# saiprasadbarke/robustmvd

Measured on AMD Instinct MI355X. Metric: depth-maps/sec at 768x1152x4srcx256planes; warp+aggregate HBM GB/s vs roofline, higher is better.
Workload: dtype f32; 1 GPU; mvsnet (Path B) forward 768x1152, 4 source views, 256 planes, batch 1 per step (BASELINE.json configs[2]); the regulariser's two layers with 32 input channels (conv0, conv4): every fp32 operand as two range-scaled fp16 terms on fp16 MFMA, fp32 accumulation (at least as close to a float64 convolution as the fp32 matrix instruction over 1e-42..1e30: tests/test_hip_f16.py), the other nine layers and ; parallelism=1 independent replica(s), frames round-robin, no collectives

## Files before the change

### include/mvd.h

```cpp
#ifndef MVD_H_
#define MVD_H_

#include <stddef.h>

#ifdef __cplusplus
extern "C" {
#endif

#define MVD_VERSION 100
#define MVD_MAX_VIEWS 32

typedef void* mvd_stream_t;

typedef enum {
    MVD_OK = 0,
    MVD_ERR_INVALID_ARG = 1,
    MVD_ERR_WORKSPACE = 2,
    MVD_ERR_LAUNCH = 3,
    MVD_ERR_NO_DEVICE = 4
} mvd_status;

#define MVD_LAYOUT_NCDHW 0
#define MVD_LAYOUT_NDHWC 1
#define MVD_GRID_EXACT 0x100
#define MVD_FEAT_NHWC_BORDER 0x200

#define MVD_LAYOUT_NCHW 0
#define MVD_LAYOUT_NHWC 1
#define MVD_LAYOUT_NHWC_BORDER 2

int mvd_version(void);
const char* mvd_last_error(void);


size_t mvd_sweep_corr_workspace_bytes(int N, int C, int h, int w, int hs, int ws, int V);
int mvd_sweep_corr_f32(const float* feat_key, const float* const* feat_src, const float* K_key,
                       const float* const* K_src, const float* const* T_src2key, const float* invdepths,
                       int invdepth_batched, int N, int C, int h, int w, int hs, int ws, int S, int V,
                       float* const* corr_out, float* const* mask_out, void* workspace, size_t workspace_bytes,
                       mvd_stream_t stream);

#define MVD_INVDEPTH_SHARED 0
#define MVD_INVDEPTH_BATCHED 1
#define MVD_INVDEPTH_PER_PIXEL 2
int mvd_sweep_corr_ex_f32(const float* feat_key, const float* const* feat_src, const float* K_key,
                          const float* const* K_src, const float* const* T_src2key, const float* invdepths,
                          int invdepth_mode, float corr_scale, int N, int C, int h, int w, int hs, int ws, int S, int V,
                          float* const* corr_out, float* const* mask_out, void* workspace, size_t workspace_bytes,
                          mvd_stream_t stream);
int mvd_sweep_corr_nhwc_f32(const float* feat_key, const float* const* feat_src, const float* K_key, const float* const* K_src,
                            const float* const* T_src2key, const float* invdepths, int invdepth_mode, float corr_scale, int N, int C,
                            int h, int w, int hs, int ws, int S, int V, float* const* corr_out, float* const* mask_out,
                            int out_pixel_stride, float* corr_absmax, mvd_stream_t stream);

int mvd_sweep_warp_f32(const float* const* feat_src, const float* K_key, const float* const* K_src,
                       const float* const* T_src2key, const float* invdepths, int invdepth_mode, int normalize_after, int N,
                       int C, int h, int w, int hs, int ws, int S, int V, float* const* warped_out, float* const* mask_out,
                       mvd_stream_t stream);

int mvd_fuse_views_f32(const float* const* corr, const float* const* mask, const float* const* score, int N, int S,
                       int h, int w, int V, float* fused, float* fused_mask, mvd_stream_t stream);
int mvd_fuse_views_nhwc_f32(const float* const* corr, const float* const* mask, const float* const* score, int N, int S, int h,
                            int w, int V, int in_pixel_stride, float* fused, float* fused_mask, int out_pixel_stride,
                            float* fused_absmax, mvd_stream_t stream);


size_t mvd_warp_variance_workspace_bytes(int B, int C, int h, int w, int V);
int mvd_warp_variance_f32(const float* key_feat, const float* const* src_feat, const float* const* src_proj,
                          const float* key_proj_inv, const float* depth_values, int B, int C, int D, int h, int w,
                          int V, float* var_out, int out_layout, void* workspace, size_t workspace_bytes,
                          mvd_stream_t stream);
int mvd_warp_variance_absmax_f32(const float* key_feat, const float* const* src_feat, const float* const* src_proj,
                                 const float* key_proj_inv, const float* depth_values, int B, int C, int D, int h, int w,
                                 int V, float* var_out, float* absmax_out, int out_layout, void* workspace,
                                 size_t workspace_bytes, mvd_stream_t stream);

size_t mvd_warp_variance_f16_workspace_bytes(int B);
int mvd_warp_variance_f16(const void* key_feat, const void* const* src_feat, const float* const* src_proj,
                          const float* key_proj_inv, const float* depth_values, int B, int D, int h, int w, int V,
                          void* var_out, void* workspace, size_t workspace_bytes, mvd_stream_t stream);
int mvd_convert_f32_to_f16(const float* src, void* dst, long long n, mvd_stream_t stream);
int mvd_convert_f16_to_f32(const void* src, float* dst, long long n, mvd_stream_t stream);

int mvd_homo_warp_f32(const float* src_feat, const float* src_proj, const float* key_proj_inv,
                      const float* depth_values, int B, int C, int D, int h, int w, float* warped_out,
                      void* workspace, size_t workspace_bytes, mvd_stream_t stream);

#define MVD_CONV3D_STRIDE1 0
#define MVD_CONV3D_STRIDE2 1
#define MVD_DECONV3D_STRIDE2 2
size_t mvd_conv3d_packed_weight_floats(int Cin, int Cout);
int mvd_pack_conv3d_weights_f32(const float* w, int Cin, int Cout, int mode, float* packed, mvd_stream_t stream);
int mvd_conv3d_bn_relu_f32(const float* x, const float* packed_w, const float* scale, const float* shift,
                           const float* skip, float* y, int B, int Di, int hi, int wi, int Cin, int Cout, int mode,
                           int relu, mvd_stream_t stream);
int mvd_conv3d_bn_relu_absmax_f32(const float* x, const float* packed_w, const float* scale, const float* shift,
                                  const float* skip, float* y, float* absmax_out, int B, int Di, int hi, int wi, int Cin,
                                  int Cout, int mode, int relu, mvd_stream_t stream);

size_t mvd_conv3d_weight_grad_workspace_bytes(int B, int Di, int hi, int wi, int Cin, int Cout, int mode);
int mvd_conv3d_weight_grad_f32(const float* x, const float* gy, float* gw, int B, int Di, int hi, int wi, int Cin, int Cout,
                               int mode, void* workspace, size_t workspace_bytes, mvd_stream_t stream);

size_t mvd_conv3d_f16_packed_weight_bytes(int Cin, int Cout);
int mvd_pack_conv3d_weights_f16(const float* w, int Cin, int Cout, void* packed, mvd_stream_t stream);
int mvd_conv3d_bn_relu_f16in(const void* x, const void* packed_w, const float* scale, const float* shift, float* y, int B,
                             int D, int h, int w, int Cin, int Cout, int relu, mvd_stream_t stream);

size_t mvd_conv3d_split_packed_weight_bytes(int Cin, int Cout);
int mvd_pack_conv3d_weights_split(const float* w, int Cin, int Cout, void* packed, mvd_stream_t stream);
int mvd_conv3d_bn_relu_f32_split(const float* x, const float* x_absmax, const void* packed_w, const float* scale, const float* shift,
                                 float* y, int B, int D, int h, int w, int Cin, int Cout, int relu, mvd_stream_t stream);
int mvd_conv3d_bn_relu_absmax_f32_split(const float* x, const float* x_absmax, const void* packed_w, const float* scale, const float* shift,
                                        float* y, float* y_absmax, int B, int D, int h, int w, int Cin, int Cout, int relu,
                                        mvd_stream_t stream);
size_t mvd_conv3d_igemm_packed_weight_bytes(int Cin, int Cout, int mode);
int mvd_pack_conv3d_weights_igemm(const float* w, int Cin, int Cout, int mode, void* packed, mvd_stream_t stream);
size_t mvd_conv3d_igemm_workspace_bytes(int B, int Di, int Hi, int Wi, int Cin, int Cout, int mode);
int mvd_conv3d_bn_relu_igemm_f32(const float* x, const float* x_absmax, const void* packed_w, const float* scale, const float* shift,
                                 const float* skip, float* y, float* y_absmax, int B, int Di, int Hi, int Wi, int Cin, int Cout, int mode,
                                 int relu, void* workspace, size_t workspace_bytes, mvd_stream_t stream);
size_t mvd_deconv3d_split_packed_weight_bytes(int Cin, int Cout);
int mvd_pack_deconv3d_weights_split(const float* w, int Cin, int Cout, void* packed, mvd_stream_t stream);
int mvd_deconv3d_bn_relu_f32_split(const float* x, const float* x_absmax, const void* packed_w, const float* scale, const float* shift,
                                   const float* skip, float* y, float* y_absmax, int B, int Di, int hi, int wi, int Cin, int Cout, int relu,
                                   mvd_stream_t stream);
#define MVD_CONV2D 0
#define MVD_DECONV2D 1
#define MVD_CONV2D_IMAGE 2
size_t mvd_conv2d_split_packed_weight_bytes(int Cin_pad, int Cout, int KH, int KW, int stride, int mode);
int mvd_pack_conv2d_weights_split(const float* w, int Cin, int Cin_pad, int Cout, int KH, int KW, int stride, int mode, void* packed,
                                  mvd_stream_t stream);
size_t mvd_conv2d_split_workspace_bytes(int B, int Hi, int Wi, int Cin_pad, int Cout, int KH, int KW, int stride, int mode);
int mvd_conv2d_split_f32(const float* x, const float* x_absmax, const void* packed_w, const float* bias, float* y, float* y_absmax, int B,
                         int Hi, int Wi, int Cin_pad, int x_pixel_stride, int Cout, int y_pixel_stride, long long y_row_stride,
                         long long y_image_stride, long long y_channel_stride, int KH, int KW, int stride, int mode, int act, float slope,
                         void* workspace, size_t workspace_bytes, mvd_stream_t stream);
int mvd_upsample2x_nhwc_f32(const float* x, float* y, float* y_absmax, int B, int C, int h, int w, int y_pixel_stride, mvd_stream_t stream);
int mvd_absmax_f32(const float* x, long long n, float* absmax, mvd_stream_t stream);

size_t mvd_conv2d_packed_weight_floats(int Cin, int Cout, int ksize);
int mvd_pack_conv2d_weights_f32(const float* w, int Cin, int Cout, int ksize, float* packed, mvd_stream_t stream);
int mvd_conv2d_bn_relu_f32(const float* x, int in_layout, const float* packed_w, const float* scale, const float* shift,
                           float* y, int out_layout, int B, int hi, int wi, int Cin, int Cout, int ksize, int stride,
                           int relu, mvd_stream_t stream);
int mvd_conv2d_bn_relu_absmax_f32(const float* x, int in_layout, const float* packed_w, const float* scale, const float* shift,
                                  float* y, float* y_absmax, int out_layout, int B, int hi, int wi, int Cin, int Cout, int ksize,
                                  int stride, int relu, mvd_stream_t stream);

size_t mvd_conv2d_head_tile_count(int B, int H, int W);
int mvd_conv2d_head_f32(const float* image, const float* w0, const float* scale0, const float* shift0, const float* w1,
                        const float* scale1, const float* shift1, float* y, float* tile_absmax, int B, int H, int W,
                        mvd_stream_t stream);
size_t mvd_conv2d_head_split_packed_bytes(void);
int mvd_pack_conv2d_head_split_weights(const float* w1, void* packed, mvd_stream_t stream);
int mvd_conv2d_head_split_f32(const float* image, const float* w0, const float* scale0, const float* shift0, const void* w1_packed,
                              const float* scale1, const float* shift1, float* y, float* tile_absmax, int B, int H, int W,
                              mvd_stream_t stream);

int mvd_softmax_regress_f32(const float* cost, const float* depth_values, int B, int D, int h, int w,
                            float* depth_out, float* conf_out, mvd_stream_t stream);

int mvd_softmax_regress_stats_f32(const float* cost, const float* depth_values, int B, int D, int h, int w,
                                  float* depth_out, float* conf_out, float* stats_out, mvd_stream_t stream);
int mvd_softmax_regress_backward_f32(const float* cost, const float* depth_values, const float* depth, const float* stats,
                                     const float* g_depth, int B, int D, int h, int w, float* g_cost, mvd_stream_t stream);

int mvd_stream_fill_f32(float* dst, long long n, float value, mvd_stream_t stream);

int mvd_arm_kernel_timing(void* start_event, void* stop_event);

int mvd_bias_leaky_relu_f32(float* x, const float* bias, int N, int C, long long HW, float slope, mvd_stream_t stream);

#define MVD_REDUCE_VARIANCE 0
#define MVD_REDUCE_VARIANCE_KEYSQ 1
#define MVD_REDUCE_GROUPCORR 2
size_t mvd_sweep_reduce_workspace_bytes(int B, int C, int h, int w, int V);
int mvd_sweep_reduce_f32(const float* key_feat, const float* const* src_feat, const float* const* M, const float* depth,
                         int depth_per_pixel, float pix_offset, float scale_x, float scale_y, float bias, int mode, int groups,
                         int B, int C, int D, int h, int w, int V, float* const* out, void* workspace, size_t workspace_bytes,
                         mvd_stream_t stream);

int mvd_sweep_reduce_nhwc_f32(const float* key_feat, const float* const* src_feat, const float* const* M, const float* depth,
                              int depth_per_pixel, float pix_offset, float scale_x, float scale_y, float bias, int mode, int B, int C,
                              int D, int h, int w, int V, float* out, mvd_stream_t stream);

int mvd_softmax_regress_pp_f32(const float* cost, const float* depth_hypos, int B, int D, int h, int w, float* depth_out,
                               float* conf_out, mvd_stream_t stream);

int mvd_sweep_groupcorr_nhwc_f32(const float* key_feat, const float* const* src_feat, const float* const* M, const float* depth,
                                 int depth_per_pixel, float pix_offset, float scale_x, float scale_y, float bias, float grid_clamp,
                                 int groups, int B, int C, int D, int h, int w, int V, float* const* out, mvd_stream_t stream);

int mvd_soft_argmin_f32(const float* score, const float* depth_start, int start_per_pixel, const float* depth_interval, float window,
                        int B, int D, int h, int w, float* depth_out, float* entropy_out, float* prob_map_out, mvd_stream_t stream);

int mvd_vis_fuse_f32(const float* const* x, const float* const* u, int B, int D, int h, int w, int C, int V, float* out,
                     mvd_stream_t stream);


size_t mvd_warp_variance_backward_workspace_bytes(int B);
int mvd_warp_variance_backward_f32(const float* key_feat, const float* const* src_feat, const float* const* src_proj,
                                   const float* key_proj_inv, const float* depth_values, const float* grad_var, int B, int C,
                                   int D, int h, int w, int V, float* grad_key, float* const* grad_src, void* workspace,
                                   size_t workspace_bytes, mvd_stream_t stream);

#define MVD_K3_GATHER_RADIUS 3
size_t mvd_warp_variance_backward_gather_workspace_bytes(int B, int C, int D, int h, int w, int V);
int mvd_warp_variance_backward_gather_f32(const float* key_feat, const float* const* src_feat, const float* const* src_proj,
                                          const float* key_proj_inv, const float* depth_values, const float* grad_var, int B, int C,
                                          int D, int h, int w, int V, float* grad_key, float* const* grad_src, int* fallback_count,
                                          void* workspace, size_t workspace_bytes, mvd_stream_t stream);

int mvd_sweep_corr_backward_f32(const float* feat_key, const float* const* feat_src, const float* K_key,
                                const float* const* K_src, const float* const* T_src2key, const float* invdepths,
                                int invdepth_mode, float corr_scale, const float* const* grad_corr, int N, int C, int h, int w,
                                int hs, int ws, int S, int V, float* grad_key, float* const* grad_src, mvd_stream_t stream);

int mvd_sweep_warp_backward_f32(const float* K_key, const float* const* K_src, const float* const* T_src2key, const float* invdepths,
                                int invdepth_mode, const float* const* grad_warped, int N, int C, int h, int w, int hs, int ws, int S,
                                int V, float* const* grad_src, mvd_stream_t stream);

size_t mvd_sweep_reduce_backward_workspace_bytes(int B, int C, int h, int w, int V);
int mvd_sweep_reduce_backward_f32(const float* key_feat, const float* const* src_feat, const float* const* M, const float* depth,
                                  int depth_per_pixel, float pix_offset, float scale_x, float scale_y, float bias, int mode,
                                  int groups, const float* const* grad_out, int B, int C, int D, int h, int w, int V, float* grad_key,
                                  float* const* grad_src, void* workspace, size_t workspace_bytes, mvd_stream_t stream);

int mvd_fuse_views_backward_f32(const float* const* corr, const float* const* mask, const float* const* score,
                                const float* grad_fused, int N, int S, int h, int w, int V, float* const* grad_corr,
                                float* const* grad_score, mvd_stream_t stream);

int mvd_resize_order1_f32(const float* src, float* dst, long long planes, int hi, int wi, int ho, int wo,
                          mvd_stream_t stream);

int mvd_dispnet_head_f32(const float* x, float* pred, float* ent, int N, long long HW, mvd_stream_t stream);

#define MVD_ALIGN_NONE 0
#define MVD_ALIGN_MEDIAN 1
#define MVD_ALIGN_LSQ 2
size_t mvd_depth_eval_workspace_bytes(int H, int W);

int mvd_depth_align_stats_f32(const float* gt, const float* pred, const float* uncertainty, const int* row, const int* col, int H,
                              int W, int h, int w, int mode, int sparse_pred, float* params, double* sums, void* workspace,
                              size_t workspace_bytes, mvd_stream_t stream);

int mvd_depth_score_f32(const float* gt, const float* pred, const float* uncertainty, const int* row, const int* col, int H, int W,
                        int h, int w, int mode, int sparse_pred, int clip, float clip_lo, float clip_hi, float thresh,
                        float thresh_plus_one, const float* params, void* result, float* pred_out, float* invdepth_out,
                        float* rel_ae_out, float* uncertainty_out, void* workspace, size_t workspace_bytes, mvd_stream_t stream);

int mvd_rank_keys_f32(const float* u, const float* u_min, const float* gt, const float* pred_aligned, int sparse_pred, long long n,
                      float* keys, mvd_stream_t stream);

int mvd_ranked_step_sums_f64(const float* ranked, long long n, const long long* count, double* step_sums, void* workspace,
                             size_t workspace_bytes, mvd_stream_t stream);

int mvd_geo_consistency_f32(const float* key_depth, const float* const* src_depth, const float* matrices, const float* uncertainty,
                            int V, int H, int W, float max_reproj_error, float max_rel_depth_diff, int min_consistent_views,
                            float max_uncertainty, unsigned* view_bits, float* fused, unsigned char* mask,
                            unsigned char* num_consistent, mvd_stream_t stream);

size_t mvd_compact_points_workspace_bytes(int H, int W);
int mvd_compact_points_f32(const unsigned char* mask, const float* depth, const float* image, const float* backproject, int H, int W,
                           float* xyz, float* rgb, long long* count, void* workspace, size_t workspace_bytes, mvd_stream_t stream);

int mvd_compact_points_attr_f32(const unsigned char* mask, const float* depth, const float* image, const float* attr,
                                const float* backproject, int H, int W, float* xyz, float* rgb, float* attr_out, long long* count,
// ... 104 lines not shown
```

### robustmvd_amd/_lib.py

```python
import ctypes
import os

import torch

_HERE = os.path.dirname(os.path.abspath(__file__))
LIB_PATH = os.path.join(_HERE, "lib", "libmvd_hip.so")
EXP_LIB_PATH = os.path.join(_HERE, "lib_exp", "libmvd_hip_exp.so")

MVD_MAX_VIEWS = 32
LAYOUT_NCDHW = 0
LAYOUT_NDHWC = 1
GRID_EXACT = 0x100
FEAT_NHWC_BORDER = 0x200
CONV3D_STRIDE1 = 0
CONV2D, DECONV2D, CONV2D_IMAGE = 0, 1, 2
CONV3D_STRIDE2 = 1
DECONV3D_STRIDE2 = 2
LAYOUT_NCHW = 0
LAYOUT_NHWC = 1
LAYOUT_NHWC_BORDER = 2
INVDEPTH_SHARED, INVDEPTH_BATCHED, INVDEPTH_PER_PIXEL = 0, 1, 2
REDUCE_VARIANCE = 0
REDUCE_VARIANCE_KEYSQ = 1
REDUCE_GROUPCORR = 2
ALIGN_NONE, ALIGN_MEDIAN, ALIGN_LSQ = 0, 1, 2
K3_GATHER_RADIUS = 3

_c_float_p = ctypes.c_void_p
_pp = ctypes.POINTER(ctypes.c_void_p)
_i = ctypes.c_int
_sz = ctypes.c_size_t

SIGNATURES = {
    "mvd_version": (_i, []),
    "mvd_last_error": (ctypes.c_char_p, []),
    "mvd_sweep_corr_workspace_bytes": (_sz, [_i] * 7),
    "mvd_sweep_corr_f32": (_i, [_c_float_p, _pp, _c_float_p, _pp, _pp, _c_float_p, _i] + [_i] * 8
                           + [_pp, _pp, ctypes.c_void_p, _sz, ctypes.c_void_p]),
    "mvd_sweep_corr_ex_f32": (_i, [_c_float_p, _pp, _c_float_p, _pp, _pp, _c_float_p, _i, ctypes.c_float] + [_i] * 8
                              + [_pp, _pp, ctypes.c_void_p, _sz, ctypes.c_void_p]),
    "mvd_sweep_corr_nhwc_f32": (_i, [_c_float_p, _pp, _c_float_p, _pp, _pp, _c_float_p, _i, ctypes.c_float] + [_i] * 8
                                + [_pp, _pp, _i, _c_float_p, ctypes.c_void_p]),
    "mvd_fuse_views_nhwc_f32": (_i, [_pp, _pp, _pp] + [_i] * 6 + [_c_float_p, _c_float_p, _i, _c_float_p, ctypes.c_void_p]),
    "mvd_upsample2x_nhwc_f32": (_i, [_c_float_p, _c_float_p, _c_float_p] + [_i] * 5 + [ctypes.c_void_p]),
    "mvd_sweep_warp_f32": (_i, [_pp, _c_float_p, _pp, _pp, _c_float_p] + [_i] * 10 + [_pp, _pp, ctypes.c_void_p]),
    "mvd_fuse_views_f32": (_i, [_pp, _pp, _pp, _i, _i, _i, _i, _i, _c_float_p, _c_float_p, ctypes.c_void_p]),
    "mvd_warp_variance_workspace_bytes": (_sz, [_i] * 5),
    "mvd_warp_variance_f32": (_i, [_c_float_p, _pp, _pp, _c_float_p, _c_float_p] + [_i] * 6
                              + [_c_float_p, _i, ctypes.c_void_p, _sz, ctypes.c_void_p]),
    "mvd_warp_variance_absmax_f32": (_i, [_c_float_p, _pp, _pp, _c_float_p, _c_float_p] + [_i] * 6
                                     + [_c_float_p, _c_float_p, _i, ctypes.c_void_p, _sz, ctypes.c_void_p]),
    "mvd_absmax_f32": (_i, [_c_float_p, ctypes.c_longlong, _c_float_p, ctypes.c_void_p]),
    "mvd_warp_variance_f16_workspace_bytes": (_sz, [_i]),
    "mvd_warp_variance_f16": (_i, [ctypes.c_void_p, _pp, _pp, _c_float_p, _c_float_p] + [_i] * 5
                              + [ctypes.c_void_p, ctypes.c_void_p, _sz, ctypes.c_void_p]),
    "mvd_convert_f32_to_f16": (_i, [_c_float_p, ctypes.c_void_p, ctypes.c_longlong, ctypes.c_void_p]),
    "mvd_convert_f16_to_f32": (_i, [ctypes.c_void_p, _c_float_p, ctypes.c_longlong, ctypes.c_void_p]),
    "mvd_homo_warp_f32": (_i, [_c_float_p] * 4 + [_i] * 5 + [_c_float_p, ctypes.c_void_p, _sz, ctypes.c_void_p]),
    "mvd_conv3d_packed_weight_floats": (_sz, [_i, _i]),
    "mvd_pack_conv3d_weights_f32": (_i, [_c_float_p, _i, _i, _i, _c_float_p, ctypes.c_void_p]),
    "mvd_conv3d_bn_relu_f32": (_i, [_c_float_p] * 6 + [_i] * 8 + [ctypes.c_void_p]),
    "mvd_conv3d_bn_relu_absmax_f32": (_i, [_c_float_p] * 7 + [_i] * 8 + [ctypes.c_void_p]),
    "mvd_conv3d_weight_grad_workspace_bytes": (_sz, [_i] * 7),
    "mvd_conv3d_weight_grad_f32": (_i, [_c_float_p] * 3 + [_i] * 7 + [ctypes.c_void_p, _sz, ctypes.c_void_p]),
    "mvd_conv3d_f16_packed_weight_bytes": (_sz, [_i, _i]),
    "mvd_pack_conv3d_weights_f16": (_i, [_c_float_p, _i, _i, ctypes.c_void_p, ctypes.c_void_p]),
    "mvd_conv3d_bn_relu_f16in": (_i, [ctypes.c_void_p, ctypes.c_void_p, _c_float_p, _c_float_p, _c_float_p] + [_i] * 7
                                 + [ctypes.c_void_p]),
    "mvd_conv3d_split_packed_weight_bytes": (_sz, [_i, _i]),
    "mvd_conv3d_bn_relu_absmax_f32_split": (_i, [_c_float_p, _c_float_p, ctypes.c_void_p, _c_float_p, _c_float_p, _c_float_p, _c_float_p]
                                            + [_i] * 7 + [ctypes.c_void_p]),
    "mvd_conv3d_igemm_packed_weight_bytes": (_sz, [_i] * 3),
    "mvd_pack_conv3d_weights_igemm": (_i, [_c_float_p, _i, _i, _i, ctypes.c_void_p, ctypes.c_void_p]),
    "mvd_conv3d_igemm_workspace_bytes": (_sz, [_i] * 7),
    "mvd_conv3d_bn_relu_igemm_f32": (_i, [_c_float_p, _c_float_p, ctypes.c_void_p] + [_c_float_p] * 5 + [_i] * 8
                                     + [ctypes.c_void_p, ctypes.c_size_t, ctypes.c_void_p]),
    "mvd_conv2d_split_packed_weight_bytes": (_sz, [_i] * 6),
    "mvd_pack_conv2d_weights_split": (_i, [_c_float_p] + [_i] * 7 + [ctypes.c_void_p, ctypes.c_void_p]),
    "mvd_conv2d_split_workspace_bytes": (_sz, [_i] * 9),
    "mvd_conv2d_split_f32": (_i, [_c_float_p, _c_float_p, ctypes.c_void_p, _c_float_p, _c_float_p, _c_float_p] + [_i] * 7
                             + [ctypes.c_longlong] * 3 + [_i] * 5 + [ctypes.c_float, ctypes.c_void_p, ctypes.c_size_t, ctypes.c_void_p]),
    "mvd_pack_conv3d_weights_split": (_i, [_c_float_p, _i, _i, ctypes.c_void_p, ctypes.c_void_p]),
    "mvd_conv3d_bn_relu_f32_split": (_i, [_c_float_p, _c_float_p, ctypes.c_void_p, _c_float_p, _c_float_p, _c_float_p] + [_i] * 7
                                     + [ctypes.c_void_p]),
    "mvd_deconv3d_split_packed_weight_bytes": (_sz, [_i, _i]),
    "mvd_pack_deconv3d_weights_split": (_i, [_c_float_p, _i, _i, ctypes.c_void_p, ctypes.c_void_p]),
    "mvd_deconv3d_bn_relu_f32_split": (_i, [_c_float_p, _c_float_p, ctypes.c_void_p] + [_c_float_p] * 5 + [_i] * 7 + [ctypes.c_void_p]),
    "mvd_conv2d_packed_weight_floats": (_sz, [_i, _i, _i]),
    "mvd_pack_conv2d_weights_f32": (_i, [_c_float_p, _i, _i, _i, _c_float_p, ctypes.c_void_p]),
    "mvd_conv2d_bn_relu_f32": (_i, [_c_float_p, _i, _c_float_p, _c_float_p, _c_float_p, _c_float_p, _i] + [_i] * 8
                               + [ctypes.c_void_p]),
    "mvd_conv2d_head_tile_count": (_sz, [_i] * 3),
    "mvd_conv2d_head_f32": (_i, [_c_float_p] * 9 + [_i] * 3 + [ctypes.c_void_p]),
    "mvd_conv2d_head_split_packed_bytes": (_sz, []),
    "mvd_pack_conv2d_head_split_weights": (_i, [_c_float_p, ctypes.c_void_p, ctypes.c_void_p]),
    "mvd_conv2d_head_split_f32": (_i, [_c_float_p] * 4 + [ctypes.c_void_p] + [_c_float_p] * 4 + [_i] * 3 + [ctypes.c_void_p]),
    "mvd_conv2d_bn_relu_absmax_f32": (_i, [_c_float_p, _i, _c_float_p, _c_float_p, _c_float_p, _c_float_p, _c_float_p, _i] + [_i] * 8
                                      + [ctypes.c_void_p]),
    "mvd_softmax_regress_f32": (_i, [_c_float_p, _c_float_p, _i, _i, _i, _i, _c_float_p, _c_float_p, ctypes.c_void_p]),
    "mvd_softmax_regress_stats_f32": (_i, [_c_float_p, _c_float_p, _i, _i, _i, _i, _c_float_p, _c_float_p, _c_float_p,
                                           ctypes.c_void_p]),
    "mvd_softmax_regress_backward_f32": (_i, [_c_float_p] * 5 + [_i] * 4 + [_c_float_p, ctypes.c_void_p]),
    "mvd_bias_leaky_relu_f32": (_i, [_c_float_p, _c_float_p, _i, _i, ctypes.c_longlong, ctypes.c_float, ctypes.c_void_p]),
    "mvd_dispnet_head_f32": (_i, [_c_float_p, _c_float_p, _c_float_p, _i, ctypes.c_longlong, ctypes.c_void_p]),
    "mvd_arm_kernel_timing": (_i, [ctypes.c_void_p, ctypes.c_void_p]),
    "mvd_stream_fill_f32": (_i, [_c_float_p, ctypes.c_longlong, ctypes.c_float, ctypes.c_void_p]),
    "mvd_warp_variance_backward_workspace_bytes": (_sz, [_i]),
    "mvd_warp_variance_backward_f32": (_i, [_c_float_p, _pp, _pp, _c_float_p, _c_float_p, _c_float_p] + [_i] * 6
                                       + [_c_float_p, _pp, ctypes.c_void_p, _sz, ctypes.c_void_p]),
    "mvd_warp_variance_backward_gather_workspace_bytes": (_sz, [_i] * 6),
    "mvd_warp_variance_backward_gather_f32": (_i, [_c_float_p, _pp, _pp, _c_float_p, _c_float_p, _c_float_p] + [_i] * 6
                                              + [_c_float_p, _pp, ctypes.c_void_p, ctypes.c_void_p, _sz, ctypes.c_void_p]),
    "mvd_sweep_corr_backward_f32": (_i, [_c_float_p, _pp, _c_float_p, _pp, _pp, _c_float_p, _i, ctypes.c_float, _pp] + [_i] * 8
                                    + [_c_float_p, _pp, ctypes.c_void_p]),
    "mvd_fuse_views_backward_f32": (_i, [_pp, _pp, _pp, _c_float_p] + [_i] * 5 + [_pp, _pp, ctypes.c_void_p]),
    "mvd_sweep_reduce_workspace_bytes": (_sz, [_i] * 5),
    "mvd_sweep_reduce_f32": (_i, [_c_float_p, _pp, _pp, _c_float_p, _i] + [ctypes.c_float] * 4 + [_i] * 8
                             + [_pp, ctypes.c_void_p, _sz, ctypes.c_void_p]),
    "mvd_sweep_reduce_nhwc_f32": (_i, [_c_float_p, _pp, _pp, _c_float_p, _i] + [ctypes.c_float] * 4 + [_i] * 7
                                  + [_c_float_p, ctypes.c_void_p]),
    "mvd_softmax_regress_pp_f32": (_i, [_c_float_p, _c_float_p, _i, _i, _i, _i, _c_float_p, _c_float_p, ctypes.c_void_p]),
    "mvd_sweep_groupcorr_nhwc_f32": (_i, [_c_float_p, _pp, _pp, _c_float_p, _i] + [ctypes.c_float] * 5 + [_i] * 7 + [_pp, ctypes.c_void_p]),
    "mvd_soft_argmin_f32": (_i, [_c_float_p, _c_float_p, _i, _c_float_p, ctypes.c_float] + [_i] * 4 + [_c_float_p] * 3 + [ctypes.c_void_p]),
    "mvd_vis_fuse_f32": (_i, [_pp, _pp] + [_i] * 6 + [_c_float_p, ctypes.c_void_p]),
    "mvd_sweep_reduce_backward_workspace_bytes": (_sz, [_i] * 5),
    "mvd_sweep_reduce_backward_f32": (_i, [_c_float_p, _pp, _pp, _c_float_p, _i] + [ctypes.c_float] * 4 + [_i, _i, _pp] + [_i] * 6
                                      + [_c_float_p, _pp, ctypes.c_void_p, _sz, ctypes.c_void_p]),
    "mvd_sweep_warp_backward_f32": (_i, [_c_float_p, _pp, _pp, _c_float_p, _i, _pp] + [_i] * 8 + [_pp, ctypes.c_void_p]),
    "mvd_resize_order1_f32": (_i, [_c_float_p, _c_float_p, ctypes.c_longlong, _i, _i, _i, _i, ctypes.c_void_p]),
    "mvd_nchw_to_nhwc_f32": (_i, [_c_float_p, _c_float_p, _i, _i, ctypes.c_longlong, ctypes.c_void_p]),
    "mvd_nhwc_to_nchw_f32": (_i, [_c_float_p, _c_float_p, _i, _i, ctypes.c_longlong, ctypes.c_void_p]),
    "mvd_zero_border_nhwc_f32": (_i, [_c_float_p, _i, _i, _i, _i, ctypes.c_void_p]),
    "mvd_depth_eval_workspace_bytes": (_sz, [_i, _i]),
    "mvd_depth_align_stats_f32": (_i, [_c_float_p] * 3 + [ctypes.c_void_p] * 2 + [_i] * 6 + [_c_float_p, ctypes.c_void_p,
                                                                                            ctypes.c_void_p, _sz, ctypes.c_void_p]),
    "mvd_depth_score_f32": (_i, [_c_float_p] * 3 + [ctypes.c_void_p] * 2 + [_i] * 7 + [ctypes.c_float] * 4
                            + [_c_float_p, ctypes.c_void_p] + [_c_float_p] * 4 + [ctypes.c_void_p, _sz, ctypes.c_void_p]),
    "mvd_rank_keys_f32": (_i, [_c_float_p] * 4 + [_i, ctypes.c_longlong, _c_float_p, ctypes.c_void_p]),
    "mvd_ranked_step_sums_f64": (_i, [_c_float_p, ctypes.c_longlong, ctypes.c_void_p, ctypes.c_void_p, ctypes.c_void_p, _sz,
                                      ctypes.c_void_p]),
    "mvd_geo_consistency_f32": (_i, [_c_float_p, _pp, _c_float_p, _c_float_p, _i, _i, _i, ctypes.c_float, ctypes.c_float, _i,
                                     ctypes.c_float] + [ctypes.c_void_p] * 5),
    "mvd_compact_points_workspace_bytes": (_sz, [_i, _i]),
    "mvd_compact_points_f32": (_i, [ctypes.c_void_p] + [_c_float_p] * 3 + [_i, _i, _c_float_p, _c_float_p, ctypes.c_void_p,
                                                                          ctypes.c_void_p, _sz, ctypes.c_void_p]),
    "mvd_compact_points_attr_f32": (_i, [ctypes.c_void_p] + [_c_float_p] * 4 + [_i, _i] + [_c_float_p] * 3
                                    + [ctypes.c_void_p, ctypes.c_void_p, _sz, ctypes.c_void_p]),
    "mvd_depth_normals_f32": (_i, [_c_float_p, _c_float_p, _i, _i, _c_float_p, ctypes.c_void_p]),
    "mvd_geo_merge_f32": (_i, [_c_float_p, _pp, _c_float_p, _c_float_p, _i, _i, _i, ctypes.c_float, ctypes.c_float, _i, ctypes.c_float,
                               ctypes.c_void_p, _pp, _c_float_p, _pp, _c_float_p, _pp] + [ctypes.c_void_p] * 7),
    "mvd_cloud_cell_keys_f32": (_i, [_c_float_p, ctypes.c_longlong] + [ctypes.c_double] * 4 + [ctypes.c_void_p] * 2),
    "mvd_cloud_grid_build_f32": (_i, [_c_float_p, ctypes.c_void_p, ctypes.c_longlong, _c_float_p, ctypes.c_void_p]),
    "mvd_cloud_nearest_f32": (_i, [_c_float_p, ctypes.c_longlong, _c_float_p, ctypes.c_void_p, ctypes.c_longlong]
                              + [ctypes.c_double] * 4 + [ctypes.c_float, _c_float_p, ctypes.c_void_p, ctypes.c_void_p]),
    "mvd_cloud_scores_workspace_bytes": (_sz, [ctypes.c_longlong]),
    "mvd_cloud_scores_f32": (_i, [_c_float_p, ctypes.c_void_p, _c_float_p, ctypes.c_longlong, _c_float_p, _i, ctypes.c_void_p,
                                  ctypes.c_void_p, _sz, ctypes.c_void_p]),
    "mvd_voxel_reduce_workspace_bytes": (_sz, [ctypes.c_longlong]),
    "mvd_voxel_reduce_f32": (_i, [ctypes.c_void_p] * 2 + [_c_float_p] * 2 + [ctypes.c_longlong, _c_float_p, _c_float_p]
                             + [ctypes.c_void_p] * 3 + [_sz, ctypes.c_void_p]),
    "mvd_cloud_transform_f32": (_i, [_c_float_p, _c_float_p, ctypes.c_longlong, ctypes.c_void_p, _c_float_p, _c_float_p, ctypes.c_void_p]),
    "mvd_cloud_transform_records_f32": (_i, [_c_float_p, ctypes.c_void_p, ctypes.c_longlong, ctypes.c_void_p, _c_float_p, ctypes.c_void_p]),
    "mvd_cloud_pair_sums_workspace_bytes": (_sz, [ctypes.c_longlong]),
    "mvd_cloud_pair_sums_f32": (_i, [_c_float_p, ctypes.c_longlong, ctypes.c_void_p, ctypes.c_void_p, _c_float_p, _c_float_p,
                                     ctypes.c_longlong] + [ctypes.c_double] * 3 + [ctypes.c_void_p, ctypes.c_void_p, _sz, ctypes.c_void_p]),
    "mvd_tsdf_integrate_f32": (_i, [_c_float_p] * 3 + [_i] * 3 + [_pp] * 3 + [_c_float_p, _i, _i, _i, ctypes.c_float, ctypes.c_float,
                                                                            ctypes.c_void_p]),
    "mvd_tsdf_extract_workspace_bytes": (_sz, [_i] * 3),
    "mvd_tsdf_extract_f32": (_i, [_c_float_p] * 3 + [_i] * 3 + [ctypes.c_float] * 5 + [_i, _c_float_p, _c_float_p, ctypes.c_void_p,
                                                                                      ctypes.c_longlong, ctypes.c_longlong,
                                                                                      ctypes.c_void_p, ctypes.c_void_p, _sz,
                                                                                      ctypes.c_void_p]),
    "mvd_mesh_render_workspace_bytes": (_sz, [ctypes.c_longlong, ctypes.c_longlong, _i, _i, _i]),
    "mvd_mesh_render_f32": (_i, [_c_float_p, ctypes.c_longlong, ctypes.c_void_p, ctypes.c_longlong, _c_float_p, _c_float_p, _i, _i, _i,
                                 ctypes.c_float, _i, _i, _i, _c_float_p, ctypes.c_void_p, _c_float_p, _c_float_p, _c_float_p,
                                 ctypes.c_void_p, _sz, ctypes.c_void_p]),
    "mvd_mesh_hook_round": (_i, [ctypes.c_void_p, ctypes.c_longlong, ctypes.c_longlong, _i] + [ctypes.c_void_p] * 4),
    "mvd_mesh_component_rank_workspace_bytes": (_sz, [ctypes.c_longlong]),
    "mvd_mesh_component_rank": (_i, [ctypes.c_void_p, ctypes.c_void_p, ctypes.c_longlong, ctypes.c_void_p, ctypes.c_void_p,
                                     ctypes.c_void_p, _sz, ctypes.c_void_p]),
    "mvd_mesh_component_table": (_i, [ctypes.c_void_p, ctypes.c_void_p] + [ctypes.c_longlong] * 3 + [ctypes.c_void_p] * 3),
    "mvd_mesh_component_sums_workspace_bytes": (_sz, [ctypes.c_longlong, ctypes.c_longlong]),
    "mvd_mesh_component_sums_f64": (_i, [_c_float_p, ctypes.c_longlong, ctypes.c_void_p, ctypes.c_longlong, ctypes.c_void_p,
                                         ctypes.c_void_p, ctypes.c_longlong, ctypes.c_void_p, ctypes.c_void_p, ctypes.c_void_p, _sz,
                                         ctypes.c_void_p]),
    "mvd_mesh_filter_workspace_bytes": (_sz, [ctypes.c_longlong, ctypes.c_longlong]),
    "mvd_mesh_filter": (_i, [ctypes.c_void_p, ctypes.c_longlong, ctypes.c_longlong, ctypes.c_void_p, ctypes.c_void_p,
                             ctypes.c_longlong, _i, _i] + [ctypes.c_void_p] * 3 + [ctypes.c_longlong, ctypes.c_void_p, ctypes.c_void_p,
                                                                                   _sz, ctypes.c_void_p]),
    "mvd_mesh_gather_rows_f32": (_i, [_c_float_p, ctypes.c_void_p, ctypes.c_longlong, _i, ctypes.c_longlong, _c_float_p,
                                      ctypes.c_void_p]),
    "mvd_mesh_vertex_normals_f32": (_i, [_c_float_p, ctypes.c_longlong, ctypes.c_void_p, ctypes.c_longlong, ctypes.c_void_p,
                                         ctypes.c_void_p, _c_float_p, ctypes.c_void_p]),
}
CULL_NONE, CULL_BACK, CULL_FRONT = 0, 1, 2
RENDER_LOAD_FIRST, RENDER_KEEP_PROJECT, RENDER_KEEP_KEYS, RENDER_NO_RESOLVE = 1, 16, 32, 64
MESH_RENDER_MAX_SMALL = 64
MESH_ROUND_FIRST, MESH_ROUND_NO_HOOK, MESH_ROUND_NO_SHORTCUT = 1, 2, 4
MVD_CLOUD_MAX_THRESHOLDS = 8
MVD_CLOUD_PAIR_SUMS_PER_WORKGROUP = 2048

PRODUCT_ONLY = ("mvd_sweep_reduce_backward_workspace_bytes", "mvd_sweep_reduce_backward_f32")

_lib = None
_override = None


def _bind(path, skip=()):
    lib = ctypes.CDLL(path)
    for name, (res, args) in SIGNATURES.items():
        if name in skip:
            continue
        fn = getattr(lib, name)
        fn.restype = res
        fn.argtypes = args
    return lib


def load():
    global _lib
    if _override is not None:
        return _override
    if _lib is not None:
        return _lib
    if not os.path.exists(LIB_PATH):
        raise RuntimeError(
            f"{LIB_PATH} not found: the HIP engine is not built. Run `python -c 'import __graft_entry__ as g; "
            "g.build()'` or `make -C robustmvd_amd/csrc`. There is no CPU fallback for this path.")
    _lib = _bind(LIB_PATH)
    return _lib


class use_experiments_library:

    def __init__(self, path=None):
        self.path = path or EXP_LIB_PATH

# ... 60 lines not shown
```

### robustmvd_amd/blocks.py

```python
from typing import NamedTuple

import numpy as np
import torch
import torch.nn as nn
import torch.nn.functional as F

from . import _lib as L
from . import ops
from .utils import to_torch

homo_warp = ops.homo_warp


def compute_sampling_invdepths(min_depth, max_depth, num_samples, sampling_type="linear_invdepth"):
    def col(v):
        if isinstance(v, (float, int, np.floating)):
            v = torch.tensor([float(v)])
        return to_torch(v).float()[..., None]

    lo, hi = col(min_depth), col(max_depth)
    steps = torch.arange(0, num_samples, dtype=lo.dtype, device=lo.device)[None]
    if sampling_type == "linear_invdepth":
        return 1 / hi + steps * (1 / lo - 1 / hi) / (num_samples - 1)
    if sampling_type == "linear_depth":
# ... 230 lines not shown
        self.split_layers = bool(split_layers)
        self.fused_head = True
        self.head_split = True
        for i, s in enumerate(self.SPEC):
            setattr(self, f"conv{i}", ConvBnReLU(*s))
        self.feature = nn.Conv2d(32, 32, 3, 1, 1)

    def _pack(self):
        pk = FeatureNetWeights()
        for i, (cin, cout, k, stride, _) in enumerate(self.SPEC):
            m = getattr(self, f"conv{i}")
            w, _, _, _ = ops.pack_conv2d_weights(m.conv.weight.detach())
            pk.layers.append(Conv2dLayer(w, cin, cout, k, stride, *fold_bn(m.bn), True))
        w, _, _, _ = ops.pack_conv2d_weights(self.feature.weight.detach())
        pk.layers.append(Conv2dLayer(w, 32, 32, 3, 1, torch.ones(32, device=w.device), self.feature.bias.detach().contiguous(), False))
        if self.split_layers:
            for i in range(2, 8):
                conv = getattr(self, f"conv{i}").conv if i < 7 else self.feature
                lay = pk.layers[i]
                pk.split.append((ops.pack_conv2d_weights_split(conv.weight.detach() * lay.scale.view(-1, 1, 1, 1), lay.shift,
                                                               stride=lay.stride), lay.relu))
            for conv, lay in ((self.conv0.conv, pk.layers[0]), (self.conv1.conv, pk.layers[1])):
                pk.head += (conv.weight.detach().permute(2, 3, 1, 0).contiguous(), lay.scale, lay.shift)
            pk.head_w1 = ops.pack_conv2d_head_weights_split(self.conv1.conv.weight.detach())
        return pk

    @ops.inference_only
    def forward_layout(self, x, out_layout, return_absmax=False, out=None):
        pk = self._prepare()
        if out is not None and not (self.split_layers and out_layout == L.LAYOUT_NHWC_BORDER):
            raise ValueError("out: only the split layers' LAYOUT_NHWC_BORDER output can be written into a caller's buffer")
        if not self.split_layers:
            for layer in pk.layers[:-1]:
                x = layer(x)
            x = pk.layers[-1](x, out_layout)
            return (x, ops.absmax(x)) if return_absmax else x
        slots = Slots(8, x.device)
        if self.fused_head:
            if self.head_split:
                x, a_in = ops.conv2d_head_split(x, *pk.head[:3], pk.head_w1, *pk.head[4:], return_absmax=True)
            else:
                x, a_in = ops.conv2d_head(x, *pk.head, return_absmax=True)
        else:
            x = pk.layers[1](pk.layers[0](x))
            a_in = ops.absmax(x)
        for wts, relu in pk.split[:-1]:
            a_out = slots.take()
            x = ops.conv2d_split(x, a_in, wts, act=2 if relu else 0, out_absmax=a_out)
            a_in = a_out
        wts, a_out = pk.split[-1][0], slots.take()
        if out_layout == L.LAYOUT_NCHW:
            x = ops.conv2d_split(x, a_in, wts, act=0, planar_out=True)
            if return_absmax:
                a_out.copy_(ops.absmax(x))
        elif out_layout == L.LAYOUT_NHWC_BORDER:
            B, h, w_, _ = x.shape
            if out is None:
                out = torch.empty((B, h + 3, w_ + 3, wts.cout), dtype=torch.float32, device=x.device)
            elif tuple(out.shape) != (B, h + 3, w_ + 3, wts.cout):
                raise ValueError(f"out: shape {tuple(out.shape)}, expected {(B, h + 3, w_ + 3, wts.cout)}")
            buf = ops.zero_border_nhwc(out)
            ops.conv2d_split(x, a_in, wts, act=0, out=buf[:, 1:h + 1, 1:w_ + 1, :], out_absmax=a_out)
            x = buf
        else:
            x = ops.conv2d_split(x, a_in, wts, act=0, out_absmax=a_out)
        return (x, a_out) if return_absmax else x

    def forward(self, x):
        return self.forward_layout(x, L.LAYOUT_NCHW)

    def forward_autograd(self, x):
        x = self.conv1(self.conv0(x))
        x = self.conv4(self.conv3(self.conv2(x)))
        return self.feature(self.conv6(self.conv5(x)))


class ConvBnReLU3D(nn.Module):
    def __init__(self, cin, cout, kernel_size=3, stride=1, pad=1):
        super().__init__()
        self.conv = nn.Conv3d(cin, cout, kernel_size, stride=stride, padding=pad, bias=False)
        self.bn = nn.BatchNorm3d(cout)

    def forward(self, x):
        return F.relu(self.bn(self.conv(x)), inplace=True)


def _deconv_block(cin, cout):
    return nn.Sequential(nn.ConvTranspose3d(cin, cout, kernel_size=3, padding=1, output_padding=1, stride=2, bias=False),
                         nn.BatchNorm3d(cout), nn.ReLU(inplace=True))


class CostRegWeights:

    def __init__(self):
        self.layers, self.igemm, self.dsplit = {}, {}, {}
        self.conv0_f16 = self.conv0_split = self.conv0_bound = None

    def get(self, key):
        name, _, form = key.rpartition("_")
        if form in ("igemm", "dsplit"):
            return getattr(self, form).get(name)
        return self.layers.get(key, getattr(self, key, None) if name == "conv0" else None)

    def __getitem__(self, key):
        found = self.get(key)
        if found is None:
            raise KeyError(key)
        return found

    def __contains__(self, key):
        return self.get(key) is not None


class CostRegNet(PackedWeights, nn.Module):

    FOLDS_BN = "CostRegNet"
    LAYERS = [("conv0", 32, 8, 1), ("conv1", 8, 16, 2), ("conv2", 16, 16, 1), ("conv3", 16, 32, 2), ("conv4", 32, 32, 1),
              ("conv5", 32, 64, 2), ("conv6", 64, 64, 1)]
    UPS = [("conv7", 64, 32), ("conv9", 32, 16), ("conv11", 16, 8)]

    def __init__(self, conv0_split=True):
        super().__init__()
        self.conv0_split = bool(conv0_split)
        for name, cin, cout, stride in self.LAYERS:
            setattr(self, name, ConvBnReLU3D(cin, cout, stride=stride))
        for name, cin, cout in self.UPS:
            setattr(self, name, _deconv_block(cin, cout))
        self.prob = nn.Conv3d(8, 1, 3, stride=1, padding=1)

    def _pack(self):
        pk = CostRegWeights()
        for name, _, _, stride in self.LAYERS:
            m = getattr(self, name)
            pk.layers[name] = Conv3dLayer.pack(m.conv.weight, L.CONV3D_STRIDE1 if stride == 1 else L.CONV3D_STRIDE2, bn=m.bn)
        for name, _, _ in self.UPS:
            m = getattr(self, name)
            pk.layers[name] = Conv3dLayer.pack(m[0].weight, L.DECONV3D_STRIDE2, bn=m[1])
        pk.layers["prob"] = Conv3dLayer.pack(self.prob.weight, L.CONV3D_STRIDE1, bias=self.prob.bias)
        pk.conv0_f16 = ops.pack_conv3d_weights_f16(self.conv0.conv.weight.detach())
        if self.conv0_split:
            w0, conv0 = self.conv0.conv.weight.detach(), pk.layers["conv0"]
            pk.conv0_split = ops.pack_conv3d_weights_split(w0)
            pk.conv0_bound = ((w0.abs().sum(dim=(1, 2, 3, 4)) * conv0.scale.abs()).contiguous(), conv0.shift.abs().contiguous())
            for name, _, _, _ in self.LAYERS[1:]:
                pk.igemm[name] = ops.pack_conv3d_weights_igemm(getattr(self, name).conv.weight.detach(), pk.layers[name].mode)
            for name, _, _ in self.UPS:
                pk.dsplit[name] = ops.pack_deconv3d_weights_split(getattr(self, name)[0].weight.detach())
        return pk

    @ops.inference_only
    def forward_channels_last(self, x, x_absmax=None):
        if x.shape[1] % 8 or x.shape[2] % 8 or x.shape[3] % 8:
            raise ValueError(f"CostRegNet needs D,h,w divisible by 8, got {tuple(x.shape[1:4])}")
        pk = self._prepare()
        first = pk["conv0"]
        split_decoder = self.conv0_split and x.dtype == torch.float32

        if x.dtype == torch.float16:
            conv0 = ops.conv3d_bn_relu_f16in(x, pk.conv0_f16, first.scale, first.shift, relu=True)
        elif self.conv0_split:
            if x_absmax is None:
                x_absmax = ops.absmax(x)
            conv0 = ops.conv3d_bn_relu_split(x, pk.conv0_split, first.scale, first.shift, relu=True, x_absmax=x_absmax)
            gain0, off0 = pk.conv0_bound
            a0 = (gain0 * x_absmax + off0).amax().reshape(1)
        else:
            conv0 = first(x)

        if self.conv0_split:
            slots = Slots(8, x.device)

            def igemm(name, t, a, leave_absmax=True):
                lay = pk[name]
                y = ops.conv3d_bn_relu_igemm(t, a, pk.igemm[name], lay.cin, lay.cout, lay.scale, lay.shift, lay.mode, relu=True,
                                             return_absmax=leave_absmax, out_absmax=slots.take() if leave_absmax else None)
                return y if leave_absmax else (y, None)

            if x.dtype == torch.float16:
                a0 = ops.absmax(conv0)
            t, a = igemm("conv1", conv0, a0)
            conv2, a = igemm("conv2", t, a)
            t, a = igemm("conv3", conv2, a)
            conv4, a = igemm("conv4", t, a)
            t, a = igemm("conv5", conv4, a)
            y, a = igemm("conv6", t, a, leave_absmax=split_decoder)
        else:
            conv2 = pk["conv2"](pk["conv1"](conv0))
            conv4 = pk["conv4"](pk["conv3"](conv2))
            y, a = pk["conv6"](pk["conv5"](conv4)), None

        def deconv(name, t, a, skip, leave_absmax=True):
            lay = pk[name]
            if not split_decoder:
                return lay(t, skip=skip), None
            y = ops.deconv3d_bn_relu_split(t, a, pk.dsplit[name], lay.cin, lay.cout, lay.scale, lay.shift, relu=True, skip=skip,
                                           return_absmax=leave_absmax, out_absmax=slots.take() if leave_absmax else None)
            return y if leave_absmax else (y, None)

        y, a = deconv("conv7", y, a, conv4)
        del conv4
        y, a = deconv("conv9", y, a, conv2)
        del conv2
        y, _ = deconv("conv11", y, a, conv0, leave_absmax=False)
        del conv0

        return pk["prob"](y, relu=False).squeeze(-1)

    @ops.inference_only
    def forward(self, x):
        return self.forward_channels_last(ops.to_channels_last_3d(x)).unsqueeze(1)

    def forward_autograd(self, x):
        conv0 = self.conv0(x)
        conv2 = self.conv2(self.conv1(conv0))
        conv4 = self.conv4(self.conv3(conv2))
        x = self.conv6(self.conv5(conv4))
        x = conv4 + self.conv7(x)
        x = conv2 + self.conv9(x)
        x = conv0 + self.conv11(x)
        return self.prob(x)

    def forward_autograd_engine(self, x):
        if x.dim() != 5 or x.shape[1] % 8 or x.shape[2] % 8 or x.shape[3] % 8:
            raise ValueError(f"CostRegNet needs (B,D,h,w,32) with D,h,w divisible by 8, got {tuple(x.shape)}")

        def layer(name, t):
            m = getattr(self, name)
            stride = m.conv.stride[0]
            y = ops.conv3d_autograd(t, m.conv.weight, L.CONV3D_STRIDE1 if stride == 1 else L.CONV3D_STRIDE2)
            return F.relu(_batch_norm_channels_last(m.bn, y), inplace=True)

        def up(name, t):
            m = getattr(self, name)
            y = ops.conv3d_autograd(t, m[0].weight, L.DECONV3D_STRIDE2)
            return F.relu(_batch_norm_channels_last(m[1], y), inplace=True)

        conv0 = layer("conv0", x)
        conv2 = layer("conv2", layer("conv1", conv0))
        conv4 = layer("conv4", layer("conv3", conv2))
        x = layer("conv6", layer("conv5", conv4))
        x = conv4 + up("conv7", x)
        x = conv2 + up("conv9", x)
        x = conv0 + up("conv11", x)
        return (ops.conv3d_autograd(x, self.prob.weight, L.CONV3D_STRIDE1) + self.prob.bias).squeeze(-1)


def _batch_norm_channels_last(bn, y):
    factor = 0.0 if bn.momentum is None else bn.momentum
    if bn.training and bn.track_running_stats and bn.num_batches_tracked is not None:
        bn.num_batches_tracked.add_(1)
        if bn.momentum is None:
            factor = 1.0 / float(bn.num_batches_tracked)
    batch_stats = bn.training or (bn.running_mean is None and bn.running_var is None)
    keep = not bn.training or bn.track_running_stats
    out = F.batch_norm(y.reshape(-1, y.shape[-1]), bn.running_mean if keep else None, bn.running_var if keep else None,
                       bn.weight, bn.bias, batch_stats, factor, bn.eps)
    return out.view(y.shape)


class _ConvLeaky(nn.Sequential):

    def forward(self, x):
        c = self[0]
        if torch.is_grad_enabled() or not x.is_cuda or c.bias is None:
            return super().forward(x)
        if isinstance(c, nn.ConvTranspose2d):
            y = F.conv_transpose2d(x, c.weight, None, c.stride, c.padding, c.output_padding, c.groups, c.dilation)
        else:
            y = F.conv2d(x, c.weight, None, c.stride, c.padding, c.dilation, c.groups)
        if y.dtype != torch.float32 or not y.is_contiguous() or y.shape[0] * y.shape[1] > 65535:
            return F.leaky_relu(y + c.bias.to(y.dtype).view(1, -1, 1, 1), self[1].negative_slope, inplace=True)
        return ops.bias_leaky_relu_(y, c.bias, self[1].negative_slope)


def conv(cin, cout, kernel_size=3, stride=1):
    return _ConvLeaky(nn.Conv2d(cin, cout, kernel_size=kernel_size, stride=stride, padding=(kernel_size - 1) // 2, bias=True),
                      nn.LeakyReLU(0.2, inplace=True))


class ReLUAndSigmoid(nn.Module):

    def __init__(self, inplace=False, min=0.0, max=1.0):
        super().__init__()
        self.min, self.max, self.range = min, max, max - min

    def forward(self, x):
        return torch.cat([F.relu(x[:, :1]), torch.sigmoid(x[:, 1:] * (4 / self.range)) * self.range + self.min], 1)


class DispnetEncoder(nn.Module):
    def __init__(self):
        super().__init__()
        self.conv1 = conv(3, 64, kernel_size=7, stride=2)
        self.conv2 = conv(64, 128, kernel_size=5, stride=2)
        self.conv3 = conv(128, 256, kernel_size=3, stride=2)

    def forward(self, image):
        c1 = self.conv1(image)
        c2 = self.conv2(c1)
        c3 = self.conv3(c2)
        return {"conv1": c1, "conv2": c2, "conv3a": c3}, c3


class DispnetContextEncoder(nn.Module):
    def __init__(self):
        super().__init__()
        self.conv_redir = conv(256, 32, kernel_size=1, stride=1)

    def forward(self, conv3):
        return self.conv_redir(conv3)


class DispnetCostvolumeEncoder(nn.Module):
    def __init__(self):
        super().__init__()
        self.conv3_1 = conv(256 + 32, 256)
        self.conv4 = conv(256, 512, stride=2)
        self.conv4_1 = conv(512, 512)
        self.conv5 = conv(512, 512, stride=2)
        self.conv5_1 = conv(512, 512)
        self.conv6 = conv(512, 1024, stride=2)
        self.conv6_1 = conv(1024, 1024)

    def forward(self, corr, ctx):
        out = {"merged": torch.cat([ctx, corr], 1)}
        x = out["merged"]
        for name in ("conv3_1", "conv4", "conv4_1", "conv5", "conv5_1", "conv6", "conv6_1"):
            x = getattr(self, name)(x)
            out[name] = x
        return out, x

# ... 61 lines not shown
```

### robustmvd_amd/csrc/conv3d_split.hip

```cpp
#include "mvd_common.h"
#include "split_operand.h"

#ifndef SPLIT_KO
#define SPLIT_KO 0
#endif
#ifndef SPLIT_DEPTH
#define SPLIT_DEPTH 4
#endif

namespace mvd {

typedef _Float16 h16x8 __attribute__((ext_vector_type(8)));
typedef float sf32x4 __attribute__((ext_vector_type(4)));
typedef unsigned int su32x4 __attribute__((ext_vector_type(4)));
typedef unsigned int su32x2 __attribute__((ext_vector_type(2)));
typedef _Float16 h16x2 __attribute__((ext_vector_type(2)));

constexpr int S_TH = 4, S_TW = 32, S_ROWS = S_TH + 2;
constexpr float S_LO_FACTOR = 2048.0f;
template <int CIN>
struct SplitGeom {
    static constexpr int CH8 = CIN / 8;
    static constexpr int VB = CIN * 2;
    static constexpr int KWG = CIN == 32 ? 3 : 2;
    static constexpr int NT = 9 * KWG;
    static constexpr int COLS = CIN == 32 ? S_TW + 2 : S_TW + 3;
    static constexpr int HALF_BYTES = S_ROWS * COLS * VB;
    static constexpr int PLANE_BYTES = 2 * HALF_BYTES;
    static constexpr int ITEMS = S_ROWS * COLS * CH8;
    static constexpr int NLOAD = (ITEMS + 255) / 256;
    static constexpr int NF = 4 * KWG * 2;
    static_assert(NF - 8 == 4 * NLOAD, "pass B interleaves 8 epilogue groups and 4 staging groups per item");
};

template <int CIN>
__global__ void pack_conv0_split_kernel(const float* __restrict__ w, const float* __restrict__ wscale, _Float16* __restrict__ packed, int ncb) {
    using G = SplitGeom<CIN>;
    const int e = blockIdx.x * 256 + threadIdx.x;
    if (e >= ncb * G::NT * 64 * 8) return;
    const int j = e & 7, lane = (e >> 3) & 63, t = (e >> 9) % G::NT, cb = (e >> 9) / G::NT;
    const int col = lane & 15, k = 8 * (lane >> 4) + j, cout = cb * 8 + (col & 7);
    int tap, cin;
    if constexpr (CIN == 32) { tap = t; cin = k; }
    else { const int kw = 2 * (t % 2) + k / 16; tap = kw < 3 ? (t / 2) * 3 + kw : -1; cin = k % 16; }
    const float v = tap >= 0 ? w[((size_t)cout * CIN + cin) * 27 + tap] / wscale[cout] : 0.0f;
    _Float16 hi, lo;
    split_weight(v, S_LO_FACTOR, hi, lo);
    packed[e] = col < 8 ? hi : lo;
}

struct SplitParams {
    const float* x;
    const char* wpk;
    const float* scale;
    const float* shift;
    const float* absmax;
    float* y;
    float* yamax;
    int B, D, h, w, relu;
    int cout, ncb;
    int tiles_x, tiles_y, dgroups, td, tiles_per_xcd;
};

__device__ __forceinline__ unsigned pack_h2(_Float16 a, _Float16 b) {
    const h16x2 v = {a, b};
    return __builtin_bit_cast(unsigned, v);
}

template <int CIN, bool YAMAX = false>
__global__ void __launch_bounds__(256, 2) conv0_split_kernel(SplitParams p) {
    using G = SplitGeom<CIN>;
    constexpr int S_COLS = G::COLS, S_HALF_BYTES = G::HALF_BYTES, S_PLANE_BYTES = G::PLANE_BYTES, S_ITEMS = G::ITEMS, S_NLOAD = G::NLOAD;
    constexpr int KWG = G::KWG, NT = G::NT;
    extern __shared__ __attribute__((aligned(16))) char ring[];
    const int tid = threadIdx.x, lane = tid & 63, wv = tid >> 6;
    const int D = p.D, h = p.h, w = p.w;

    const int xcd = blockIdx.x & 7;
    int j = blockIdx.x >> 3;
    const int cb = j % p.ncb; j /= p.ncb;
    const int t_in = j % p.tiles_per_xcd; j /= p.tiles_per_xcd;
    const int dg = j % p.dgroups;
    const int b = j / p.dgroups;
    const int tile = xcd * p.tiles_per_xcd + t_in;
    if (tile >= p.tiles_x * p.tiles_y) return;
    const int ty = tile / p.tiles_x, tx = tile - ty * p.tiles_x;
    const int x0 = tx * S_TW, y0 = ty * S_TH;
    const int dz0 = dg * p.td, dz1 = min(dz0 + p.td, D);

    h16x8 wf[NT];
#pragma unroll
    for (int t = 0; t < NT; ++t) wf[t] = *reinterpret_cast<const h16x8*>(p.wpk + (((size_t)cb * NT + t) * 64 + lane) * 16);

    constexpr unsigned OOB = 0x80000000u;
    unsigned gob[S_NLOAD];
    int loff[S_NLOAD];
#pragma unroll
    for (int k = 0; k < S_NLOAD; ++k) {
        const int e = tid + 256 * k;
        const int vox = e / G::CH8, ch = e % G::CH8;
        const int r = vox / S_COLS, c = vox - r * S_COLS;
        const int gy = y0 - 1 + r, gx = x0 - 1 + c;
        const bool in = e < S_ITEMS && c < S_TW + 2 && gy >= 0 && gy < h && gx >= 0 && gx < w;
        gob[k] = in ? (unsigned)(((gy * w + gx) * CIN + ch * 8) * 4) : OOB;
        if constexpr (CIN == 32) loff[k] = e < S_ITEMS ? (vox * 64 + ((ch ^ ((c >> 1) & 3)) * 16)) : -1;
        else loff[k] = e < S_ITEMS ? e * 16 : -1;
    }
    const size_t plane_f = (size_t)h * w * CIN;
    const float* xb = p.x + (size_t)b * D * plane_f;
    su32x4 pre[S_NLOAD][2];
    auto fetch = [&](int d) {
        const bool din = d >= 0 && d < D && d <= dz1;
        const __amdgpu_buffer_rsrc_t rs = __builtin_amdgcn_make_buffer_rsrc(
            const_cast<float*>(xb + (din ? (size_t)d * plane_f : 0)), 0, din ? (int)(plane_f * 4) : 0, 0x00020000);
#pragma unroll
        for (int k = 0; k < S_NLOAD; ++k) {
            pre[k][0] = __builtin_amdgcn_raw_buffer_load_b128(rs, gob[k], 0, 0);
            pre[k][1] = __builtin_amdgcn_raw_buffer_load_b128(rs, gob[k] + 16u, 0, 0);
        }
    };
    char* const dump = ring + 2 * S_PLANE_BYTES + tid * 16;
    float xs, xs_inv;
    split_xscale(p.absmax, xs, xs_inv);
    auto split2 = [xs](float a0, float a1, unsigned& hi, unsigned& lo) { mvd::split2(xs, a0, a1, hi, lo, S_LO_FACTOR); };
    auto stash = [&](int d) {
        char* slot = ring + (d & 1) * S_PLANE_BYTES;
#pragma unroll
        for (int k = 0; k < S_NLOAD; ++k) {
            su32x4 hv, lv;
#pragma unroll
            for (int q = 0; q < 4; ++q) {
                const sf32x4 v = __builtin_bit_cast(sf32x4, pre[k][q >> 1]);
                unsigned hi, lo;
                split2(v[(q & 1) * 2], v[(q & 1) * 2 + 1], hi, lo);
                hv[q] = hi; lv[q] = lo;
            }
            char* dst = loff[k] >= 0 ? slot + loff[k] : dump;
            *reinterpret_cast<su32x4*>(dst) = hv;
            *reinterpret_cast<su32x4*>(loff[k] >= 0 ? dst + S_HALF_BYTES : dst) = lv;
        }
    };

    const int col = lane & 15;
    float esc_ = p.scale[cb * 8 + (col & 7)], esh_ = p.shift[cb * 8 + (col & 7)];
    float eun_ = reinterpret_cast<const float*>(p.wpk + (size_t)p.ncb * NT * 64 * 16)[cb * 8 + (col & 7)] * xs_inv;
    const float floor_ = p.relu ? 0.f : -__builtin_inff();
    const int xh = wv & 1, rp = wv >> 1;

    int fragk[KWG];
#pragma unroll
    for (int kw = 0; kw < KWG; ++kw) {
        if constexpr (CIN == 32) {
            const int c = 16 * xh + (lane & 15) + kw;
            fragk[kw] = (2 * rp * S_COLS + c) * 64 + (((lane >> 4) ^ ((c >> 1) & 3)) * 16);
        } else {
            const int c = 16 * xh + (lane & 15) + 2 * kw;
            fragk[kw] = (2 * rp * S_COLS + c) * 32 + (lane >> 4) * 16;
        }
    }

    sf32x4 acc[3][2][2];
#pragma unroll
    for (int s = 0; s < 3; ++s)
#pragma unroll
        for (int r = 0; r < 2; ++r) { acc[s][r][0] = sf32x4{0, 0, 0, 0}; acc[s][r][1] = sf32x4{0, 0, 0, 0}; }

    unsigned yoff[2];
#pragma unroll
    for (int row = 0; row < 2; ++row) {
        const int oy = y0 + 2 * rp + row;
        yoff[row] = (col < 8 && oy < h) ? (unsigned)((((size_t)oy * w + x0 + 16 * xh + 4 * (lane >> 4)) * p.cout + cb * 8 + col) * 4) : OOB;
    }
    const int oxb = x0 + 16 * xh + 4 * (lane >> 4);
    const size_t yplane_f = (size_t)h * w * p.cout;
    const unsigned vox_b = (unsigned)p.cout * 4u;

    fetch(dz0 - 1);
    asm volatile("" : "+v"(esc_), "+v"(esh_), "+v"(eun_));
    stash(dz0 - 1);
    fetch(dz0);

    [[maybe_unused]] float amax_ = 0.f;
    for (int z = dz0 - 1; z <= dz1; ++z) {
        if (!(SPLIT_KO & 8)) __syncthreads();
        const char* slot = ring + (z & 1) * S_PLANE_BYTES;
        char* wslot = ring + ((z + 1) & 1) * S_PLANE_BYTES;
        const int din = z + 2, dout = z - 1;
        const bool in_ok = din >= 0 && din < D && din <= dz1, out_ok = dout >= dz0 && dout < dz1;
        const __amdgpu_buffer_rsrc_t rs_in = __builtin_amdgcn_make_buffer_rsrc(
            const_cast<float*>(xb + (in_ok ? (size_t)din * plane_f : 0)), 0, in_ok ? (int)(plane_f * 4) : 0, 0x00020000);
        const __amdgpu_buffer_rsrc_t rs_out = __builtin_amdgcn_make_buffer_rsrc(
            p.y + ((size_t)b * D + (out_ok ? dout : 0)) * yplane_f, 0, out_ok ? (int)(yplane_f * 4) : 0, 0x00020000);
        int ox = oxb;
        asm volatile("" : "+v"(ox));

        constexpr int NF = G::NF, NR = 2 * NF, DEPTH = SPLIT_DEPTH;
        h16x8 fr[DEPTH];
        auto rr_of = [](int ro) { return ro == 0 ? 1 : ro == 1 ? 2 : ro == 2 ? 0 : 3; };
        auto frag = [&](int i) {
            const int g = i % NF, term = g & 1, kw = (g >> 1) % KWG, rr = rr_of(g / (2 * KWG));
            if (SPLIT_KO & 32) return wf[i % NT];
            return *reinterpret_cast<const h16x8*>(slot + term * S_HALF_BYTES + fragk[kw] + rr * S_COLS * G::VB);
        };
#pragma unroll
        for (int i = 0; i < DEPTH; ++i) fr[i] = frag(i);
#pragma unroll
        for (int g = 0; g < NF; ++g) {
            const int term = g & 1, kw = (g >> 1) % KWG, rr = rr_of(g / (2 * KWG));
            const h16x8 f = fr[g % DEPTH];
#pragma unroll
            for (int row = 0; row < 2; ++row) {
                const int kh = rr - row;
                if (kh < 0 || kh > 2) continue;
                if (SPLIT_KO & 16) acc[0][row][term][0] += f[0] * wf[(6 + kh) * KWG + kw][0];
                else acc[0][row][term] = __builtin_amdgcn_mfma_f32_16x16x32_f16(f, wf[(6 + kh) * KWG + kw], acc[0][row][term], 0, 0, 0);
            }
            fr[g % DEPTH] = frag(g + DEPTH);
            __builtin_amdgcn_sched_barrier(0);
        }
        float hl = __shfl_down(acc[0][0][0][0], 8, 16);
        unsigned hq0 = 0, lq0 = 0;
#pragma unroll
        for (int g = 0; g < NF; ++g) {
            const int term = g & 1, kw = (g >> 1) % KWG, rr = rr_of(g / (2 * KWG));
            const h16x8 f = fr[(NF + g) % DEPTH];
#pragma unroll
            for (int row = 0; row < 2; ++row) {
                const int kh = rr - row;
                if (kh < 0 || kh > 2) continue;
#pragma unroll
                for (int s = 1; s < 3; ++s)
                    if (SPLIT_KO & 16) acc[s][row][term][0] += f[0] * wf[((2 - s) * 3 + kh) * KWG + kw][0];
                    else acc[s][row][term] = __builtin_amdgcn_mfma_f32_16x16x32_f16(f, wf[((2 - s) * 3 + kh) * KWG + kw], acc[s][row][term], 0, 0, 0);
            }
            if (NF + g + DEPTH < NR) fr[(NF + g) % DEPTH] = frag(NF + g + DEPTH);
            if (g < 8) {
                const int row = g >> 2, i = g & 3;
                const float cur = hl;
                if (g + 1 < 8) hl = __shfl_down(acc[0][(g + 1) >> 2][0][(g + 1) & 3], 8, 16);
                float r = __builtin_fmaf(cur + acc[0][row][1][i], 1.0f / 2048.0f, acc[0][row][0][i]);
                r = fmaxf(__builtin_fmaf(r * eun_, esc_, esh_), floor_);
                if constexpr (YAMAX)
                    if (out_ok && yoff[row] != OOB && ox + i < w) amax_ = fmaxf(amax_, finite_abs_or_zero(r));
                if (!(SPLIT_KO & 2) || r == 12345.678f)
                    __builtin_amdgcn_raw_buffer_store_b32(__float_as_uint(r), rs_out, ox + i < w ? yoff[row] + vox_b * i : OOB, 0, 0);
            } else if (!(SPLIT_KO & 4)) {
                const int k = (g - 8) >> 2, q = (g - 8) & 3;
                const sf32x4 v = __builtin_bit_cast(sf32x4, pre[k][q >> 1]);
                unsigned hq1, lq1;
                split2(v[(q & 1) * 2], v[(q & 1) * 2 + 1], hq1, lq1);
                if (q & 1) {
                    char* dst = (loff[k] >= 0 ? wslot + loff[k] : dump) + 8 * (q >> 1);
                    *reinterpret_cast<su32x2*>(dst) = su32x2{hq0, hq1};
                    *reinterpret_cast<su32x2*>(loff[k] >= 0 ? dst + S_HALF_BYTES : dst) = su32x2{lq0, lq1};
                } else {
                    hq0 = hq1; lq0 = lq1;
                }
                if (q == 3 && !(SPLIT_KO & 1)) {
                    pre[k][0] = __builtin_amdgcn_raw_buffer_load_b128(rs_in, gob[k], 0, 0);
                    pre[k][1] = __builtin_amdgcn_raw_buffer_load_b128(rs_in, gob[k] + 16u, 0, 0);
                }
            }
            __builtin_amdgcn_sched_barrier(0);
        }
#pragma unroll
        for (int r = 0; r < 2; ++r)
#pragma unroll
            for (int t = 0; t < 2; ++t) {
                acc[0][r][t] = acc[1][r][t];
                acc[1][r][t] = acc[2][r][t];
                acc[2][r][t] = sf32x4{0, 0, 0, 0};
            }
    }
    if constexpr (YAMAX) {
        for (int o = 32; o > 0; o >>= 1) amax_ = fmaxf(amax_, __shfl_xor(amax_, o));
        __syncthreads();
        float* wm = reinterpret_cast<float*>(ring);
        if (lane == 0) wm[wv] = amax_;
        __syncthreads();
        if (tid == 0) {
            amax_ = fmaxf(fmaxf(wm[0], wm[1]), fmaxf(wm[2], wm[3]));
            raise_absmax(p.yamax, amax_);
        }
    }
}

}

static bool split_shape_ok(int Cin, int Cout) { return (Cin == 32 || Cin == 16) && Cout >= 8 && Cout <= 64 && Cout % 8 == 0; }
static size_t split_frag_bytes(int Cin, int Cout) { return (size_t)(Cout / 8) * (Cin == 32 ? 27 : 18) * 64 * 16; }

template <int CIN, bool YAMAX>
static int launch_split_v(const mvd::SplitParams& p, long long nblk, hipStream_t st) {
    const size_t lds = 2 * (size_t)mvd::SplitGeom<CIN>::PLANE_BYTES + 256 * 16;
    (void)hipFuncSetAttribute((const void*)mvd::conv0_split_kernel<CIN, YAMAX>, hipFuncAttributeMaxDynamicSharedMemorySize, (int)lds);
    hipLaunchKernelGGL((mvd::conv0_split_kernel<CIN, YAMAX>), dim3((unsigned)nblk), dim3(256), lds, st, p);
    return mvd::launch_status("conv3d_split");
}
template <int CIN>
static int launch_split(const mvd::SplitParams& p, long long nblk, hipStream_t st) {
    return p.yamax ? launch_split_v<CIN, true>(p, nblk, st) : launch_split_v<CIN, false>(p, nblk, st);
}

extern "C" {

size_t mvd_conv3d_split_packed_weight_bytes(int Cin, int Cout) {
    return split_shape_ok(Cin, Cout) ? split_frag_bytes(Cin, Cout) + (size_t)Cout * sizeof(float) : 0;
}

int mvd_pack_conv3d_weights_split(const float* w, int Cin, int Cout, void* packed, mvd_stream_t stream) {
    MVD_REQUIRE(w && packed, "pack_conv3d_weights_split: NULL argument");
    MVD_REQUIRE(split_shape_ok(Cin, Cout), "pack_conv3d_weights_split: 16 or 32 input channels and 8, 16, ... 64 output channels are built (got %d -> %d)", Cin, Cout);
    const int ncb = Cout / 8;
    float* wscale = reinterpret_cast<float*>(static_cast<char*>(packed) + split_frag_bytes(Cin, Cout));
    mvd::split_wscale_launch(w, wscale, Cin, Cout, 27, false, Cout, Cout, (hipStream_t)stream);
    const unsigned nb = (unsigned)((split_frag_bytes(Cin, Cout) / 2 + 255) / 256);
    if (Cin == 32) hipLaunchKernelGGL(mvd::pack_conv0_split_kernel<32>, dim3(nb), dim3(256), 0, (hipStream_t)stream, w, wscale, (_Float16*)packed, ncb);
    else hipLaunchKernelGGL(mvd::pack_conv0_split_kernel<16>, dim3(nb), dim3(256), 0, (hipStream_t)stream, w, wscale, (_Float16*)packed, ncb);
    return mvd::launch_status("pack_conv3d_weights_split");
}

static int conv3d_split_entry(const float* x, const float* x_absmax, const void* packed_w, const float* scale, const float* shift, float* y,
                              float* y_absmax, int B, int D, int h, int w, int Cin, int Cout, int relu, mvd_stream_t stream);

int mvd_conv3d_bn_relu_f32_split(const float* x, const float* x_absmax, const void* packed_w, const float* scale, const float* shift,
                                 float* y, int B, int D, int h, int w, int Cin, int Cout, int relu, mvd_stream_t stream) {
    return conv3d_split_entry(x, x_absmax, packed_w, scale, shift, y, nullptr, B, D, h, w, Cin, Cout, relu, stream);
}

int mvd_conv3d_bn_relu_absmax_f32_split(const float* x, const float* x_absmax, const void* packed_w, const float* scale, const float* shift,
                                        float* y, float* y_absmax, int B, int D, int h, int w, int Cin, int Cout, int relu,
                                        mvd_stream_t stream) {
    MVD_REQUIRE(y_absmax, "conv3d_split_absmax: NULL argument");
    return conv3d_split_entry(x, x_absmax, packed_w, scale, shift, y, y_absmax, B, D, h, w, Cin, Cout, relu, stream);
}

static int conv3d_split_entry(const float* x, const float* x_absmax, const void* packed_w, const float* scale, const float* shift, float* y,
                              float* y_absmax, int B, int D, int h, int w, int Cin, int Cout, int relu, mvd_stream_t stream) {
    MVD_REQUIRE(x && x_absmax && packed_w && scale && shift && y, "conv3d_split: NULL argument");
    MVD_REQUIRE(split_shape_ok(Cin, Cout), "conv3d_split: 16 or 32 input channels and 8, 16, ... 64 output channels are built (got %d -> %d)", Cin, Cout);
    MVD_REQUIRE(B > 0 && D > 0 && h > 0 && w > 0, "conv3d_split: non-positive dimension");
    MVD_REQUIRE((long long)h * w * Cin * 4 < 0x7fffffffLL && (long long)h * w * Cout * 4 < 0x7fffffffLL,
                "conv3d_split: one plane exceeds the 31-bit byte-offset range");
    mvd::SplitParams p{};
    p.x = x; p.absmax = x_absmax; p.wpk = (const char*)packed_w; p.scale = scale; p.shift = shift; p.y = y; p.yamax = y_absmax;
    if (y_absmax && hipMemsetAsync(y_absmax, 0, sizeof(float), (hipStream_t)stream) != hipSuccess) return mvd::launch_status("conv3d_split: memset");
    p.B = B; p.D = D; p.h = h; p.w = w; p.relu = relu;
    p.cout = Cout; p.ncb = Cout / 8;
    p.tiles_x = (w + mvd::S_TW - 1) / mvd::S_TW;
    p.tiles_y = (h + mvd::S_TH - 1) / mvd::S_TH;
    const long long tiles = (long long)p.tiles_x * p.tiles_y;
    p.tiles_per_xcd = (int)((tiles + 7) / 8);
    int td = 32;
    while (td > 8 && tiles * B * p.ncb * ((D + td - 1) / td) < 2048) td /= 2;
    p.td = td;
    p.dgroups = (D + td - 1) / td;
    const long long nblk = 8LL * p.ncb * p.tiles_per_xcd * p.dgroups * B;
    MVD_REQUIRE(nblk <= 0x7fffffffLL, "conv3d_split: %lld workgroups exceed the grid limit", nblk);
    return Cin == 32 ? launch_split<32>(p, nblk, (hipStream_t)stream) : launch_split<16>(p, nblk, (hipStream_t)stream);
}
}
```

### robustmvd_amd/csrc/split_operand.h

```cpp
#pragma once
#include "mvd_common.h"

namespace mvd {

__device__ __forceinline__ void split_xscale_of(unsigned max_bits, float& xsc, float& xsc_inv) {
    const int ex = (int)((max_bits >> 23) & 0xffu) - 127;
    const int e = max(-125, min(125, ex - 14));
    xsc = __uint_as_float((unsigned)(127 - e) << 23);
    xsc_inv = __uint_as_float((unsigned)(127 + e) << 23);
}
__device__ __forceinline__ void split_xscale(const float* xamax, float& xsc, float& xsc_inv) {
    split_xscale_of(__builtin_amdgcn_readfirstlane((int)__float_as_uint(*xamax)), xsc, xsc_inv);
}
__device__ __forceinline__ void split2(float xsc, float a0, float a1, unsigned& hi, unsigned& lo, float lo_factor = 1.0f) {
    unsigned hp, lp;
    float t0, t1;
    asm("v_fma_mixlo_f16 %0, %1, %2, 0 op_sel:[0,0,0] op_sel_hi:[0,0,0]" : "=v"(hp) : "v"(a0), "s"(xsc));
    asm("v_fma_mixhi_f16 %0, %1, %2, 0 op_sel:[0,0,0] op_sel_hi:[0,0,0]" : "+v"(hp) : "v"(a1), "s"(xsc));
    asm("v_fma_mix_f32 %0, %1, %2, -%3 op_sel:[0,0,0] op_sel_hi:[0,0,1]" : "=v"(t0) : "v"(a0), "s"(xsc), "v"(hp));
    asm("v_fma_mix_f32 %0, %1, %2, -%3 op_sel:[0,0,1] op_sel_hi:[0,0,1]" : "=v"(t1) : "v"(a1), "s"(xsc), "v"(hp));
    asm("v_fma_mixlo_f16 %0, %1, %2, 0 op_sel:[0,0,0] op_sel_hi:[0,0,0]" : "=v"(lp) : "v"(t0), "s"(lo_factor));
    asm("v_fma_mixhi_f16 %0, %1, %2, 0 op_sel:[0,0,0] op_sel_hi:[0,0,0]" : "+v"(lp) : "v"(t1), "s"(lo_factor));
    hi = hp;
    lo = lp;
}

__device__ __forceinline__ void split_weight(float v, float lo_factor, _Float16& hi, _Float16& lo) {
    hi = (_Float16)v;
    lo = (_Float16)((v - (float)hi) * lo_factor);
}

static __global__ void split_wscale_kernel(const float* __restrict__ w, float* __restrict__ wscale, int Cin, int Cout, int taps, int transposed,
                                           int rows) {
    __shared__ float red[256];
    const int r = blockIdx.x, c = r % Cout;
    float m = 0.f;
    if (r < rows)
        for (int e = threadIdx.x; e < Cin * taps; e += 256) {
            const int ci = e / taps, t = e % taps;
            const float v = fabsf(transposed ? w[((size_t)ci * Cout + c) * taps + t] : w[((size_t)c * Cin + ci) * taps + t]);
            m = (finite_f32(v) && v > m) ? v : m;
        }
    red[threadIdx.x] = m;
    __syncthreads();
    for (int o = 128; o > 0; o >>= 1) {
        if (threadIdx.x < o) red[threadIdx.x] = fmaxf(red[threadIdx.x], red[threadIdx.x + o]);
        __syncthreads();
    }
    if (threadIdx.x == 0) {
        const int ex = (int)((__float_as_uint(red[0]) >> 23) & 0xffu) - 127;
        const int k = red[0] > 0.f ? max(-100, min(100, ex - 10)) : 0;
        wscale[r] = ldexpf(1.0f, k);
    }
}
static inline void split_wscale_launch(const float* w, float* wscale, int Cin, int Cout, int taps, bool transposed, int rows, int rows_padded,
                                       hipStream_t st) {
    hipLaunchKernelGGL(split_wscale_kernel, dim3(rows_padded), dim3(256), 0, st, w, wscale, Cin, Cout, taps, transposed ? 1 : 0, rows);
}

}
```

### robustmvd_amd/csrc/warp_variance.hip

```cpp
#include "mvd_common.h"
#include "warp_variance_common.h"

namespace mvd {


__global__ void compose_transforms_kernel(ViewPtrs proj, const float* __restrict__ key_proj_inv, int B, int V,
                                          float* __restrict__ M) {
    const int e = blockIdx.x * blockDim.x + threadIdx.x;
    if (e >= V * B * 12) return;
    const int j = e % 4, i = (e / 4) % 3, b = (e / 12) % B, v = e / (12 * B);
    const float* P = proj.p[v] + b * 16;
    const float* Q = key_proj_inv + b * 16;
    float acc = P[i * 4 + 0] * Q[0 * 4 + j];
    acc = fmaf(P[i * 4 + 1], Q[1 * 4 + j], acc);
    acc = fmaf(P[i * 4 + 2], Q[2 * 4 + j], acc);
    acc = fmaf(P[i * 4 + 3], Q[3 * 4 + j], acc);
    M[e] = acc;
}
void launch_compose_transforms(const ViewPtrs& proj, const float* key_proj_inv, int B, int V, float* M, hipStream_t st) {
    hipLaunchKernelGGL(compose_transforms_kernel, dim3((unsigned)((V * B * 12 + 255) / 256)), dim3(256), 0, st, proj, key_proj_inv,
                       B, V, M);
}

__global__ void __launch_bounds__(256) repack_padded_kernel(const float* __restrict__ src, float* __restrict__ dst, int C,
// ... 283 lines not shown
                }
        } else {
#pragma unroll
            for (int i = 0; i < DPB; ++i) {
                f[i][0] = __builtin_amdgcn_raw_buffer_load_b128(rsrc, off[i], 0, 0);
                f[i][1] = __builtin_amdgcn_raw_buffer_load_b128(rsrc, off[i] + PIX, 0, 0);
                f[i][2] = __builtin_amdgcn_raw_buffer_load_b128(rsrc, off[i] + rowb, 0, 0);
                f[i][3] = __builtin_amdgcn_raw_buffer_load_b128(rsrc, off[i] + rowb + PIX, 0, 0);
            }
        }
#pragma unroll
        for (int i = 0; i < DPB; ++i) {
            float4 acc = make_float4(0, 0, 0, 0);
#pragma unroll
            for (int k = 0; k < 4; ++k) {
                acc.x = fmaf(__uint_as_float(f[i][k].x), wt[i][k], acc.x);
                acc.y = fmaf(__uint_as_float(f[i][k].y), wt[i][k], acc.y);
                acc.z = fmaf(__uint_as_float(f[i][k].z), wt[i][k], acc.z);
                acc.w = fmaf(__uint_as_float(f[i][k].w), wt[i][k], acc.w);
            }
            s1[i].x += acc.x; s1[i].y += acc.y; s1[i].z += acc.z; s1[i].w += acc.w;
            s2[i].x = fmaf(acc.x, acc.x, s2[i].x); s2[i].y = fmaf(acc.y, acc.y, s2[i].y);
            s2[i].z = fmaf(acc.z, acc.z, s2[i].z); s2[i].w = fmaf(acc.w, acc.w, s2[i].w);
        }
    }

    const float inv_nv = 1.0f / (float)(p.V + 1);
    const size_t plane = (size_t)h * w;
#pragma unroll
    for (int i = 0; i < DPB; ++i) {
        const int d = d0 + i;
        if (d >= D) break;
        float4 r;
        if constexpr (WARP_ONLY) {
            r = s1[i];
        } else {
            const float mx = s1[i].x * inv_nv, my = s1[i].y * inv_nv, mz = s1[i].z * inv_nv, mw = s1[i].w * inv_nv;
            r = make_float4(fmaf(s2[i].x, inv_nv, -mx * mx), fmaf(s2[i].y, inv_nv, -my * my),
                            fmaf(s2[i].z, inv_nv, -mz * mz), fmaf(s2[i].w, inv_nv, -mw * mw));
        }
        if (p.layout == MVD_LAYOUT_NDHWC) {
            if (active)
                *reinterpret_cast<float4*>(p.out + ((((size_t)b * D + d) * h + y) * w + x) * C + q * 4) = r;
            continue;
        }
        __syncthreads();
        stage[(q * 4 + 0) * (PPB + 1) + px] = r.x;
        stage[(q * 4 + 1) * (PPB + 1) + px] = r.y;
        stage[(q * 4 + 2) * (PPB + 1) + px] = r.z;
        stage[(q * 4 + 3) * (PPB + 1) + px] = r.w;
        __syncthreads();
#pragma unroll
        for (int e0 = 0; e0 < C * PPB / 256; ++e0) {
            const int e = tid + e0 * 256;
            const int c = e / PPB, xx = e % PPB;
            if (x0 + xx < w)
                p.out[(((size_t)b * C + c) * D + d) * plane + (size_t)y * w + x0 + xx] = stage[c * (PPB + 1) + xx];
        }
    }
}

static size_t padded_image_floats(int C, int h, int w) { return (size_t)(h + 3) * (w + 3) * C; }
static size_t padded_slot_bytes(int B, int C, int h, int w) {
    return align_up((size_t)B * padded_image_floats(C, h, w) * sizeof(float), 256);
}

static int repack_padded(const float* src, float* dst, int B, int C, int h, int w, hipStream_t st) {
    if (hipMemsetAsync(dst, 0, padded_slot_bytes(B, C, h, w), st) != hipSuccess) return launch_status("repack: memset");
    const long long hw = (long long)h * w;
    dim3 grid((unsigned)((hw + 31) / 32), (unsigned)((C + 31) / 32), (unsigned)B);
    hipLaunchKernelGGL(repack_padded_kernel, grid, dim3(256), 0, st, src, dst, C, h, w);
    return launch_status("repack_padded");
}

int repack_padded_launch(const float* src, float* dst, int B, int C, int h, int w, hipStream_t st) {
    return repack_padded(src, dst, B, C, h, w, st);
}
size_t padded_slot_bytes_public(int B, int C, int h, int w) { return padded_slot_bytes(B, C, h, w); }

int launch_gather(const WarpParams& p0, int lpp, int dpb, WarpKernel kernel, hipStream_t st) {
    WarpParams p = p0;
    const int ppb = 256 / lpp;
    p.tiles_x = (p.w + ppb - 1) / ppb;
    const long long tiles = (long long)p.tiles_x * p.h;
    p.tiles_per_xcd = (int)((tiles + 7) / 8);
    const long long nblk = 8LL * p.tiles_per_xcd * ((p.D + dpb - 1) / dpb) * p.B;
    if (nblk > 0x7fffffffLL) {
        set_error("warp_variance: %lld workgroups exceed the grid limit", nblk);
        return MVD_ERR_INVALID_ARG;
    }
    timing_begin(st);
    hipLaunchKernelGGL(kernel, dim3((unsigned)nblk), dim3(256), 0, st, p);
    timing_end(st);
    return launch_status("warp_variance");
}

template <bool WARP_ONLY, bool EXACT>
static WarpKernel gather_kernel(int lpp) {
    switch (lpp) {
        case 1: return warp_variance_kernel<1, WARP_ONLY, 4, 3, 0, EXACT>;
        case 2: return warp_variance_kernel<2, WARP_ONLY, 4, 3, 0, EXACT>;
        case 4: return warp_variance_kernel<4, WARP_ONLY, 4, 3, 0, EXACT>;
        case 8: return warp_variance_kernel<8, WARP_ONLY, 4, 3, EXACT ? 0 : 2, EXACT>;
        default: return warp_variance_kernel<16, WARP_ONLY, 4, 3, 0, EXACT>;
    }
}

int launch_warp_gather(const WarpParams& p, int C, bool warp_only, hipStream_t st) {
    const int lpp = C / 4;
    const WarpKernel k = p.exact_grid ? (warp_only ? gather_kernel<true, true>(lpp) : gather_kernel<false, true>(lpp))
                                      : (warp_only ? gather_kernel<true, false>(lpp) : gather_kernel<false, false>(lpp));
    return launch_gather(p, lpp, 4, k, st);
}

__global__ void __launch_bounds__(256) absmax_kernel(const float* __restrict__ x, long long n, unsigned* __restrict__ out) {
    __shared__ float wmax[4];
    const long long n4 = n / 4;
    float m = 0.f;
    auto take = [&m](const float4 v) {
        m = fmaxf(fmaxf(m, fmaxf(finite_abs_or_zero(v.x), finite_abs_or_zero(v.y))), fmaxf(finite_abs_or_zero(v.z), finite_abs_or_zero(v.w)));
    };
    const long long per_blk = ((n4 + gridDim.x - 1) / gridDim.x + 255) / 256 * 256;
    const float4* __restrict__ x4 = reinterpret_cast<const float4*>(x);
    long long i = (long long)blockIdx.x * per_blk + threadIdx.x;
    const long long end = min(n4, ((long long)blockIdx.x + 1) * per_blk);
    for (; i + 7 * 256 < end; i += 8 * 256) {
        float4 v[8];
#pragma unroll
        for (int k = 0; k < 8; ++k) v[k] = x4[i + k * 256];
#pragma unroll
        for (int k = 0; k < 8; ++k) take(v[k]);
    }
    for (; i < end; i += 256) take(x4[i]);
    if (blockIdx.x == 0 && threadIdx.x < (int)(n - n4 * 4)) m = fmaxf(m, finite_abs_or_zero(x[n4 * 4 + threadIdx.x]));
    for (int o = 32; o > 0; o >>= 1) m = fmaxf(m, __shfl_xor(m, o));
    if ((threadIdx.x & 63) == 0) wmax[threadIdx.x >> 6] = m;
    __syncthreads();
    if (threadIdx.x == 0) {
        m = fmaxf(fmaxf(wmax[0], wmax[1]), fmaxf(wmax[2], wmax[3]));
        raise_absmax(reinterpret_cast<float*>(out), m);
    }
}

int absmax_launch(const float* x, long long n, float* absmax, hipStream_t st) {
    if (hipMemsetAsync(absmax, 0, sizeof(float), st) != hipSuccess) return launch_status("absmax: memset");
    if (n <= 0) return MVD_OK;
    const long long want = (n / 4 + 4095) / 4096;
    const unsigned nblk = (unsigned)(want < 1 ? 1 : (want > 2048 ? 2048 : want));
    hipLaunchKernelGGL(absmax_kernel, dim3(nblk), dim3(256), 0, st, x, n, reinterpret_cast<unsigned*>(absmax));
    return launch_status("absmax");
}

static int launch_k3(const WarpParams& p0, int C, bool warp_only, bool f16, hipStream_t st, float* absmax = nullptr,
                     bool* absmax_done = nullptr) {
    WarpParams p = p0;
#ifdef MVD_EXPERIMENTS
    if (const char* e = exp_env("MVD_K3_CFG")) {
#define MVD_G(R, DPB, MW) {R, DPB, MW, warp_only ? warp_variance_kernel<8, true, DPB, MW, R> : warp_variance_kernel<8, false, DPB, MW, R>}
        const GatherForm forms[] = {MVD_G(0, 1, 8), MVD_G(0, 2, 4), MVD_G(0, 2, 6), MVD_G(0, 2, 8), MVD_G(0, 4, 2), MVD_G(0, 4, 3),
                                    MVD_G(0, 4, 4), MVD_G(0, 8, 2), MVD_G(0, 8, 3), MVD_G(1, 2, 4), MVD_G(1, 2, 6), MVD_G(1, 4, 2),
                                    MVD_G(1, 4, 3), MVD_G(1, 4, 4), MVD_G(1, 8, 2), MVD_G(2, 4, 2), MVD_G(2, 4, 3), MVD_G(2, 4, 4),
                                    MVD_G(4, 4, 2), MVD_G(4, 4, 3), MVD_G(4, 4, 4)};
#undef MVD_G
        return warp_variance_experiment(e, p, C, warp_only, f16, st, forms, (int)(sizeof(forms) / sizeof(forms[0])));
    }
#endif
    if (f16) return launch_warp_tile(p, st, 8, 128, 8, 1, true, false);
    if (!warp_only && C == 32 && p.layout == MVD_LAYOUT_NDHWC && warp_tile_supported(p, false)) {
        if (absmax) {
            if (hipMemsetAsync(absmax, 0, sizeof(float), st) != hipSuccess) return launch_status("warp_variance: memset");
            p.absmax = absmax;
            *absmax_done = true;
        }
        return launch_warp_tile(p, st, 8, 104, 8, 1, false, p.exact_grid != 0);
    }
    return launch_warp_gather(p, C, warp_only, st);
}

static int run_warp(const float* key_feat, const float* const* src_feat, const float* const* src_proj,
                    const float* key_proj_inv, const float* depth_values, int B, int C, int D, int h, int w, int V,
                    float* out, int layout, void* workspace, size_t workspace_bytes, hipStream_t st, bool warp_only,
                    float* absmax = nullptr, bool* absmax_done = nullptr) {
    const char* who = warp_only ? "homo_warp" : "warp_variance";
    MVD_REQUIRE(B > 0 && D > 0 && h > 1 && w > 1, "%s: non-positive dimension (h, w must be >= 2)", who);
    MVD_REQUIRE(V >= 1 && V <= MVD_MAX_VIEWS, "%s: V=%d outside 1..%d", who, V, MVD_MAX_VIEWS);
    MVD_REQUIRE(C == 4 || C == 8 || C == 16 || C == 32 || C == 64, "%s: C=%d unsupported (need 4, 8, 16, 32 or 64)", who, C);
    MVD_REQUIRE((long long)(h + 3) * (w + 3) * C * 4 < 0x7fffffffLL && h < (1 << 23) && w < (1 << 23),
                "%s: one padded feature map of %dx%dx%d floats exceeds the 2 GiB buffer-offset range", who, h, w, C);
    const bool staged = (layout & MVD_FEAT_NHWC_BORDER) != 0;
    const size_t need = staged ? align_up((size_t)MVD_MAX_VIEWS * B * 12 * sizeof(float), 256)
                               : mvd_warp_variance_workspace_bytes(B, C, h, w, warp_only ? 0 : V);
    if (!workspace || workspace_bytes < need) {
        set_error("%s: workspace %zu B < required %zu B", who, workspace_bytes, need);
        return MVD_ERR_WORKSPACE;
    }
    const size_t slot = padded_slot_bytes(B, C, h, w);
    char* ws = (char*)workspace;
    WarpParams p{};
    p.M = (float*)ws;
    ws += align_up((size_t)MVD_MAX_VIEWS * B * 12 * sizeof(float), 256);
    int rc;
    if (!warp_only) {
        if (staged) {
            p.key = key_feat;
        } else {
            rc = repack_padded(key_feat, (float*)ws, B, C, h, w, st);
            if (rc) return rc;
            p.key = (float*)ws;
            ws += slot;
        }
    }
    for (int v = 0; v < V; ++v) {
        MVD_REQUIRE(src_feat[v] && src_proj[v], "%s: NULL view %d", who, v);
        if (staged) {
            p.src.p[v] = src_feat[v];
        } else {
            rc = repack_padded(src_feat[v], (float*)ws, B, C, h, w, st);
            if (rc) return rc;
            p.src.p[v] = (float*)ws;
            ws += slot;
        }
        p.proj.p[v] = src_proj[v];
    }
    launch_compose_transforms(p.proj, key_proj_inv, B, V, const_cast<float*>(p.M), st);
    rc = launch_status("compose_transforms");
    if (rc) return rc;
    p.key_proj_inv = key_proj_inv;
    p.depth = depth_values;
    p.out = out;
    p.B = B; p.D = D; p.h = h; p.w = w; p.V = V;
    p.layout = layout & 0xff;
    p.exact_grid = (layout & MVD_GRID_EXACT) ? 1 : 0;
    return launch_k3(p, C, warp_only, false, st, absmax, absmax_done);
}

static int run_warp_f16(const void* key_feat, const void* const* src_feat, const float* const* src_proj,
                        const float* key_proj_inv, const float* depth_values, int B, int D, int h, int w, int V, void* out,
                        void* workspace, size_t workspace_bytes, hipStream_t st) {
    const char* who = "warp_variance_f16";
    MVD_REQUIRE(B > 0 && D > 0 && h > 1 && w > 1, "%s: non-positive dimension (h, w must be >= 2)", who);
    MVD_REQUIRE(V >= 1 && V <= MVD_MAX_VIEWS, "%s: V=%d outside 1..%d", who, V, MVD_MAX_VIEWS);
    MVD_REQUIRE((long long)(h + 3) * (w + 3) * 64 < 0x7fffffffLL && h < (1 << 23) && w < (1 << 23),
                "%s: one padded feature map of %dx%dx32 halves exceeds the 2 GiB buffer-offset range", who, h, w);
    const size_t need = align_up((size_t)MVD_MAX_VIEWS * B * 12 * sizeof(float), 256);
    if (!workspace || workspace_bytes < need) {
        set_error("%s: workspace %zu B < required %zu B", who, workspace_bytes, need);
        return MVD_ERR_WORKSPACE;
    }
    WarpParams p{};
    p.M = (float*)workspace;
    p.key = (const float*)key_feat;
    for (int v = 0; v < V; ++v) {
        MVD_REQUIRE(src_feat[v] && src_proj[v], "%s: NULL view %d", who, v);
        p.src.p[v] = (const float*)src_feat[v];
        p.proj.p[v] = src_proj[v];
    }
    p.key_proj_inv = key_proj_inv;
    p.depth = depth_values;
    p.out = (float*)out;
    p.B = B; p.D = D; p.h = h; p.w = w; p.V = V;
    p.layout = MVD_LAYOUT_NDHWC;
    MVD_REQUIRE(warp_tile_supported(p, true), "%s: maps of %dx%d are outside the fp16 kernel's range (h, w <= 65532 and h*w*64 < 2^31)",
                who, h, w);
    launch_compose_transforms(p.proj, key_proj_inv, B, V, const_cast<float*>(p.M), st);
    const int rc = launch_status("compose_transforms");
    if (rc) return rc;
    return launch_k3(p, 32, false, true, st);
}

template <bool TO_HALF>
__global__ void __launch_bounds__(256) convert_kernel(const void* __restrict__ src, void* __restrict__ dst, long long n4) {
    const long long i = (long long)blockIdx.x * 256 + threadIdx.x;
    if (i >= n4) return;
    if constexpr (TO_HALF) {
        const float4 v = reinterpret_cast<const float4*>(src)[i];
        const f16x2 lo = {(_Float16)v.x, (_Float16)v.y}, hi = {(_Float16)v.z, (_Float16)v.w};
        reinterpret_cast<u32x2*>(dst)[i] = u32x2{as_u32(lo), as_u32(hi)};
    } else {
        const u32x2 v = reinterpret_cast<const u32x2*>(src)[i];
        const f16x2 lo = as_h2(v.x), hi = as_h2(v.y);
        reinterpret_cast<float4*>(dst)[i] = make_float4((float)lo.x, (float)lo.y, (float)hi.x, (float)hi.y);
    }
}

template <bool TO_HALF>
static int convert(const void* src, void* dst, long long n, hipStream_t st) {
    MVD_REQUIRE(src && dst && n > 0 && n % 4 == 0, "convert: NULL argument or element count not a positive multiple of 4");
    const long long n4 = n / 4, nblk = (n4 + 255) / 256;
    MVD_REQUIRE(nblk <= 0x7fffffffLL, "convert: too many elements");
    hipLaunchKernelGGL(convert_kernel<TO_HALF>, dim3((unsigned)nblk), dim3(256), 0, st, src, dst, n4);
    return launch_status("convert");
}

}

extern "C" {

size_t mvd_warp_variance_f16_workspace_bytes(int B) {
    return B > 0 ? mvd::align_up((size_t)MVD_MAX_VIEWS * B * 12 * sizeof(float), 256) : 0;
}

int mvd_warp_variance_f16(const void* key_feat, const void* const* src_feat, const float* const* src_proj,
                          const float* key_proj_inv, const float* depth_values, int B, int D, int h, int w, int V,
                          void* var_out, void* workspace, size_t workspace_bytes, mvd_stream_t stream) {
    MVD_REQUIRE(key_feat && src_feat && src_proj && key_proj_inv && depth_values && var_out, "warp_variance_f16: NULL argument");
    return mvd::run_warp_f16(key_feat, src_feat, src_proj, key_proj_inv, depth_values, B, D, h, w, V, var_out, workspace,
                             workspace_bytes, (hipStream_t)stream);
}

int mvd_convert_f32_to_f16(const float* src, void* dst, long long n, mvd_stream_t stream) {
    return mvd::convert<true>(src, dst, n, (hipStream_t)stream);
}
int mvd_convert_f16_to_f32(const void* src, float* dst, long long n, mvd_stream_t stream) {
    return mvd::convert<false>(src, dst, n, (hipStream_t)stream);
}

size_t mvd_warp_variance_workspace_bytes(int B, int C, int h, int w, int V) {
    if (B <= 0 || C <= 0 || h <= 0 || w <= 0 || V < 0) return 0;
    return mvd::align_up((size_t)MVD_MAX_VIEWS * B * 12 * sizeof(float), 256) +
           (size_t)(V + 1) * mvd::padded_slot_bytes(B, C, h, w);
}

int mvd_warp_variance_f32(const float* key_feat, const float* const* src_feat, const float* const* src_proj,
                          const float* key_proj_inv, const float* depth_values, int B, int C, int D, int h, int w,
                          int V, float* var_out, int out_layout, void* workspace, size_t workspace_bytes,
                          mvd_stream_t stream) {
    MVD_REQUIRE(key_feat && src_feat && src_proj && key_proj_inv && depth_values && var_out,
                "warp_variance: NULL argument");
    MVD_REQUIRE((out_layout & 0xff) == MVD_LAYOUT_NCDHW || (out_layout & 0xff) == MVD_LAYOUT_NDHWC, "warp_variance: bad layout");
    return mvd::run_warp(key_feat, src_feat, src_proj, key_proj_inv, depth_values, B, C, D, h, w, V, var_out, out_layout,
                         workspace, workspace_bytes, (hipStream_t)stream, false);
}

int mvd_warp_variance_absmax_f32(const float* key_feat, const float* const* src_feat, const float* const* src_proj,
                                 const float* key_proj_inv, const float* depth_values, int B, int C, int D, int h, int w,
                                 int V, float* var_out, float* absmax_out, int out_layout, void* workspace, size_t workspace_bytes,
                                 mvd_stream_t stream) {
    MVD_REQUIRE(key_feat && src_feat && src_proj && key_proj_inv && depth_values && var_out && absmax_out,
                "warp_variance_absmax: NULL argument");
    MVD_REQUIRE((out_layout & 0xff) == MVD_LAYOUT_NCDHW || (out_layout & 0xff) == MVD_LAYOUT_NDHWC, "warp_variance: bad layout");
    bool done = false;
    int rc = mvd::run_warp(key_feat, src_feat, src_proj, key_proj_inv, depth_values, B, C, D, h, w, V, var_out, out_layout,
                           workspace, workspace_bytes, (hipStream_t)stream, false, absmax_out, &done);
    if (rc == MVD_OK && !done) rc = mvd::absmax_launch(var_out, (long long)B * C * D * h * w, absmax_out, (hipStream_t)stream);
    return rc;
}

int mvd_absmax_f32(const float* x, long long n, float* absmax, mvd_stream_t stream) {
    MVD_REQUIRE(x && absmax && n >= 0, "absmax: NULL argument or negative count");
    return mvd::absmax_launch(x, n, absmax, (hipStream_t)stream);
}

int mvd_homo_warp_f32(const float* src_feat, const float* src_proj, const float* key_proj_inv,
                      const float* depth_values, int B, int C, int D, int h, int w, float* warped_out,
                      void* workspace, size_t workspace_bytes, mvd_stream_t stream) {
    MVD_REQUIRE(src_feat && src_proj && key_proj_inv && depth_values && warped_out, "homo_warp: NULL argument");
    const float* srcs[1] = {src_feat};
    const float* projs[1] = {src_proj};
    return mvd::run_warp(nullptr, srcs, projs, key_proj_inv, depth_values, B, C, D, h, w, 1, warped_out,
                         MVD_LAYOUT_NCDHW, workspace, workspace_bytes, (hipStream_t)stream, true);
}
}
```

### robustmvd_amd/csrc/warp_variance_common.h

```cpp
#pragma once
#include "mvd_common.h"

namespace mvd {

struct WarpParams {
    ViewPtrs src;
    ViewPtrs proj;
    const float* key;
    const float* M;
    const float* key_proj_inv;
    const float* depth;
    float* out;
    int B, D, h, w, V;
    int layout;
    int tiles_x, tiles_y, tiles_per_xcd;
    int exact_grid;
    float* absmax;
};

typedef unsigned int u32x4 __attribute__((ext_vector_type(4)));

__device__ __forceinline__ void accumulate_cell(float4& a1, float4& a2, const float (&w)[4], const u32x4 (&t)[4]) {
    float4 acc = make_float4(0, 0, 0, 0);
#pragma unroll
    for (int k = 0; k < 4; ++k) {
        acc.x = fmaf(__uint_as_float(t[k].x), w[k], acc.x);
        acc.y = fmaf(__uint_as_float(t[k].y), w[k], acc.y);
        acc.z = fmaf(__uint_as_float(t[k].z), w[k], acc.z);
        acc.w = fmaf(__uint_as_float(t[k].w), w[k], acc.w);
    }
    a1.x += acc.x; a1.y += acc.y; a1.z += acc.z; a1.w += acc.w;
    a2.x = fmaf(acc.x, acc.x, a2.x); a2.y = fmaf(acc.y, acc.y, a2.y);
    a2.z = fmaf(acc.z, acc.z, a2.z); a2.w = fmaf(acc.w, acc.w, a2.w);
}

typedef unsigned int u32x2 __attribute__((ext_vector_type(2)));
typedef _Float16 f16x2 __attribute__((ext_vector_type(2)));
__device__ __forceinline__ f16x2 as_h2(unsigned v) { return __builtin_bit_cast(f16x2, v); }
__device__ __forceinline__ unsigned as_u32(f16x2 v) { return __builtin_bit_cast(unsigned, v); }

__device__ __forceinline__ void accumulate_cell(float4& a1, float4& a2, const float (&w)[4], const u32x2 (&t)[4]) {
    float4 acc = make_float4(0, 0, 0, 0);
#pragma unroll
    for (int k = 0; k < 4; ++k) {
        const f16x2 lo = as_h2(t[k].x), hi = as_h2(t[k].y);
        acc.x = fmaf((float)lo.x, w[k], acc.x);
        acc.y = fmaf((float)lo.y, w[k], acc.y);
        acc.z = fmaf((float)hi.x, w[k], acc.z);
        acc.w = fmaf((float)hi.y, w[k], acc.w);
    }
    a1.x += acc.x; a1.y += acc.y; a1.z += acc.z; a1.w += acc.w;
    a2.x = fmaf(acc.x, acc.x, a2.x); a2.y = fmaf(acc.y, acc.y, a2.y);
    a2.z = fmaf(acc.z, acc.z, a2.z); a2.w = fmaf(acc.w, acc.w, a2.w);
}

typedef unsigned int u32x2n __attribute__((vector_size(8)));
__device__ __forceinline__ u32x2 load_b64(__amdgpu_buffer_rsrc_t rsrc, unsigned voff, unsigned soff) {
    const u32x2n r = __builtin_amdgcn_raw_buffer_load_b64(rsrc, voff, soff, 0);
    return u32x2{r[0], r[1]};
}
__device__ __forceinline__ void store_b64(u32x2 v, __amdgpu_buffer_rsrc_t rsrc, unsigned voff) {
    const u32x2n r = {v.x, v.y};
    __builtin_amdgcn_raw_buffer_store_b64(r, rsrc, voff, 0, 0);
}

bool warp_tile_supported(const WarpParams& p, bool f16);
int launch_warp_tile(const WarpParams& p0, hipStream_t st, int tw, int win, int nch, int sets, bool f16, bool exact);

typedef void (*WarpKernel)(WarpParams);
int launch_gather(const WarpParams& p0, int lpp, int dpb, WarpKernel kernel, hipStream_t st);
int launch_warp_gather(const WarpParams& p, int C, bool warp_only, hipStream_t st);

#ifdef MVD_EXPERIMENTS
struct GatherForm {
    int reuse, dpb, minw;
    WarpKernel kernel;
};
int warp_variance_experiment(const char* cfg, const WarpParams& p, int C, bool warp_only, bool f16, hipStream_t st,
                             const GatherForm* forms, int nforms);
#endif

}
```

### robustmvd_amd/csrc/warp_variance_tile.hip

```cpp
#include "mvd_common.h"
#include <type_traits>
#include "warp_variance_common.h"

namespace mvd {

typedef unsigned short u16x2 __attribute__((ext_vector_type(2)));

__device__ __forceinline__ unsigned pk_min_u16(unsigned a, unsigned b) {
    return __builtin_bit_cast(unsigned, __builtin_elementwise_min(__builtin_bit_cast(u16x2, a), __builtin_bit_cast(u16x2, b)));
}
__device__ __forceinline__ unsigned pk_max_u16(unsigned a, unsigned b) {
    return __builtin_bit_cast(unsigned, __builtin_elementwise_max(__builtin_bit_cast(u16x2, a), __builtin_bit_cast(u16x2, b)));
}
template <int K>
__device__ __forceinline__ unsigned row_shr(unsigned v) {
    return (unsigned)__builtin_amdgcn_update_dpp((int)v, (int)v, 0x110 + K, 0xf, 0xf, false);
}

typedef float f32x2 __attribute__((ext_vector_type(2)));
struct Sums { f32x2 a1[2], a2[2]; };
__device__ __forceinline__ void tap_pairs(const u32x4& t, f32x2& lo, f32x2& hi) {
    lo = f32x2{__uint_as_float(t.x), __uint_as_float(t.y)};
    hi = f32x2{__uint_as_float(t.z), __uint_as_float(t.w)};
}
__device__ __forceinline__ void tap_pairs(const u32x2& t, f32x2& lo, f32x2& hi) {
    const f16x2 l = as_h2(t.x), h = as_h2(t.y);
    lo = f32x2{(float)l.x, (float)l.y};
    hi = f32x2{(float)h.x, (float)h.y};
}
template <class TAP>
__device__ __forceinline__ void accumulate_cell_pk(Sums& s, const float4 w, const TAP (&t)[4]) {
    const float wk[4] = {w.x, w.y, w.z, w.w};
    f32x2 lo = {0.0f, 0.0f}, hi = {0.0f, 0.0f};
#pragma unroll
    for (int k = 0; k < 4; ++k) {
        f32x2 tl, th;
        tap_pairs(t[k], tl, th);
        const f32x2 ws = {wk[k], wk[k]};
        lo = __builtin_elementwise_fma(tl, ws, lo);
        hi = __builtin_elementwise_fma(th, ws, hi);
    }
    s.a1[0] += lo; s.a1[1] += hi;
    s.a2[0] = __builtin_elementwise_fma(lo, lo, s.a2[0]);
    s.a2[1] = __builtin_elementwise_fma(hi, hi, s.a2[1]);
}

__device__ __forceinline__ void lds_dma_b128(u32x4 rsrc, unsigned voff, unsigned lds_dst) {
    asm volatile("s_mov_b32 m0, %2\n\ts_nop 0\n\tbuffer_load_dwordx4 %0, %1, 0 offen lds" : : "v"(voff), "s"(rsrc), "s"(lds_dst) : "memory");
}

#ifndef MVD_K3T_KO
#define MVD_K3T_KO 0
#endif

struct UnitRec {
    unsigned boxmin;
    unsigned extent;
    unsigned pitch;
    unsigned npix;
    unsigned base;
    unsigned skip;
    float inv_nc;
    unsigned pad;
};
struct ViewRec {
    float M[12];
    unsigned base_lo, base_hi;
    unsigned pad[2];
};

template <int TW, int WINPIX, bool F16, bool EXACT, int MINW, int SETS>
__global__ void __launch_bounds__(256, MINW) warp_variance_tile_kernel(WarpParams p, int nch) {
    constexpr int P = 8, NPX = 32;
    constexpr unsigned PIXB = F16 ? 64 : 128;
    constexpr unsigned QB = F16 ? 8 : 16;
    constexpr unsigned WINB = WINPIX * PIXB;
    constexpr int PPP = 1024 / PIXB;
    constexpr int LPX = PIXB / 16;
    constexpr int NPIECE = WINPIX / PPP;
    constexpr unsigned TABW0 = 2 * WINB, TABO0 = TABW0 + 2 * 4096, PROBE0 = TABO0 + 2 * 1024, FAIL0 = PROBE0 + 512, VIEW0 = FAIL0 + 128;
    using TAP = typename std::conditional<F16, u32x2, u32x4>::type;
    extern __shared__ __attribute__((aligned(16))) char lds[];

    const int tid = threadIdx.x;
    const int wv = __builtin_amdgcn_readfirstlane(tid >> 6);
    const int h = p.h, w = p.w, D = p.D, V = p.V;
    const unsigned DEP0 = VIEW0 + (unsigned)V * sizeof(ViewRec), UNIT0 = DEP0 + (unsigned)nch * 32;

    const int xcd = blockIdx.x & 7;
    int j = blockIdx.x >> 3;
    const int dchunks = (D + P - 1) / P;
    const int dgroups = (dchunks + nch - 1) / nch;
    const int dg = j % dgroups; j /= dgroups;
    const int tile_in = j % p.tiles_per_xcd;
    const int b = j / p.tiles_per_xcd;
    const int tile = xcd * p.tiles_per_xcd + tile_in;
    if (tile >= p.tiles_x * p.tiles_y) return;
    const int tyi = tile / p.tiles_x;
    const int x0 = (tile - tyi * p.tiles_x) * TW, y0 = tyi * (NPX / TW);
    const int nchunks = (dchunks - dg + dgroups - 1) / dgroups;
    auto chunk_of = [&](int jc) { return dg + jc * dgroups; };

    const int W2 = w + 3;
    const unsigned rowb = (unsigned)W2 * PIXB;
    const unsigned img_bytes = (unsigned)(h + 3) * rowb;

    auto opaque_tid = [&]() { int t = tid; asm volatile("" : "+v"(t)); return t; };
    auto blend_pixel = [&](int t, int& bx, int& by) {
        const int px = t >> 3;
        bx = min(x0 + px % TW, w - 1);
        by = min(y0 + px / TW, h - 1);
    };

    float4 key;
    {
        int bx, by;
        blend_pixel(tid, bx, by);
        const char* kp = reinterpret_cast<const char*>(p.key) + (size_t)b * img_bytes + (unsigned)(by + 1) * rowb +
                         (unsigned)(bx + 1) * PIXB + (unsigned)(tid & 7) * QB;
        if constexpr (F16) {
            const u32x2 kh = *reinterpret_cast<const u32x2*>(kp);
            const f16x2 lo = as_h2(kh.x), hi = as_h2(kh.y);
            key = make_float4((float)lo.x, (float)lo.y, (float)hi.x, (float)hi.y);
        } else {
            key = *reinterpret_cast<const float4*>(kp);
        }
    }
    const float inv_nv = 1.0f / (float)(V + 1);
    const size_t plane_bytes = (size_t)h * w * PIXB;

    auto src_rsrc = [&](int v) {
        return __builtin_amdgcn_make_buffer_rsrc(const_cast<char*>(reinterpret_cast<const char*>(p.src.p[v]) + (size_t)b * img_bytes),
                                                 0, (int)img_bytes, 0x00020000);
    };

    const float sx = __int_as_float(__builtin_amdgcn_readfirstlane(__float_as_int((float)w / (float)(w - 1))));
    const float sy = __int_as_float(__builtin_amdgcn_readfirstlane(__float_as_int((float)h / (float)(h - 1))));
    auto position = [&](const float (&M)[12], float fx, float fy, float depth, float& ix, float& iy) -> float {
        float Z;
        if constexpr (EXACT) {
            const float half_w = (float)(w - 1) / 2.0f, half_h = (float)(h - 1) / 2.0f;
            const float gx = fx * depth, gy = fy * depth;
            const float X = ((M[0] * gx + M[1] * gy) + M[2] * depth) + M[3];
            const float Y = ((M[4] * gx + M[5] * gy) + M[6] * depth) + M[7];
            Z = ((M[8] * gx + M[9] * gy) + M[10] * depth) + M[11];
            ix = unnormalize_coord((X / Z) / half_w - 1.0f, (float)w);
            iy = unnormalize_coord((Y / Z) / half_h - 1.0f, (float)h);
        } else {
            const float ax = fmaf(M[0], fx, fmaf(M[1], fy, M[2]));
            const float ay = fmaf(M[4], fx, fmaf(M[5], fy, M[6]));
            const float az = fmaf(M[8], fx, fmaf(M[9], fy, M[10]));
            const float X = fmaf(ax, depth, M[3]), Y = fmaf(ay, depth, M[7]);
            Z = fmaf(az, depth, M[11]);
            const float rz = __builtin_amdgcn_rcpf(Z);
            ix = fmaf(X * rz, sx, -0.5f);
            iy = fmaf(Y * rz, sy, -0.5f);
        }
        ix = __builtin_amdgcn_fmed3f(ix, -1.0f, (float)w);
        iy = __builtin_amdgcn_fmed3f(iy, -1.0f, (float)h);
        return Z;
    };

    unsigned lds_chunks;
    {
        const int pv = tid >> 3, co = tid & 7;
        const float cfx = (float)((co & 1) ? min(x0 + TW - 1, w - 1) : x0);
        const float cfy = (float)((co & 2) ? min(y0 + NPX / TW - 1, h - 1) : y0);
        float M[12];
        {
            const float* Mg = p.M + ((size_t)min(pv, V - 1) * p.B + b) * 12;
#pragma unroll
            for (int k = 0; k < 12; ++k) M[k] = Mg[k];
        }
        if (co == 0 && pv < V) {
            ViewRec* vr = reinterpret_cast<ViewRec*>(lds + VIEW0) + pv;
#pragma unroll
            for (int k = 0; k < 12; ++k) vr->M[k] = M[k];
            const unsigned long long sb = (unsigned long long)(reinterpret_cast<const char*>(p.src.p[pv]) + (size_t)b * img_bytes);
            vr->base_lo = (unsigned)sb; vr->base_hi = (unsigned)(sb >> 32);
        }
        if (tid < 32) *reinterpret_cast<unsigned*>(lds + FAIL0 + tid * 4) = 0u;
        const float* dg_ = p.depth + (size_t)b * D;
        for (int e = tid; e < nchunks * P; e += 256) *reinterpret_cast<float*>(lds + DEP0 + e * 4) = dg_[min(chunk_of(e / P) * P + e % P, D - 1)];
        __syncthreads();
        for (int jc = 0; jc < nchunks; ++jc) {
            const float depth = *reinterpret_cast<const float*>(lds + DEP0 + (jc * P + ((co & 4) ? P - 1 : 0)) * 4);
            float ix, iy;
            const float Z = position(M, cfx, cfy, depth, ix, iy);
            const unsigned cell = ((unsigned)((int)floorf(iy) + 1) << 16) | (unsigned)((int)floorf(ix) + 1);
            const bool ok = Z > 0.0f;
            unsigned mn = ok ? cell : 0u, mx = ok ? cell : 0xffffffffu;
            mn = pk_min_u16(mn, row_shr<1>(mn)); mx = pk_max_u16(mx, row_shr<1>(mx));
            mn = pk_min_u16(mn, row_shr<2>(mn)); mx = pk_max_u16(mx, row_shr<2>(mx));
            mn = pk_min_u16(mn, row_shr<4>(mn)); mx = pk_max_u16(mx, row_shr<4>(mx));
            const int xmin = max((int)(mn & 0xffffu) - 1, 0), ymin = max((int)(mn >> 16) - 1, 0);
            const int xmax = min((int)(mx & 0xffffu) + 1, w + 1), ymax = min((int)(mx >> 16) + 1, h + 1);
            const int nc = xmax - xmin + 2, nr = ymax - ymin + 2;
            const bool mine = (co == 7) && (pv < V);
            if (mine) {
                UnitRec r;
                r.boxmin = (unsigned)xmin | ((unsigned)ymin << 16);
                r.extent = (unsigned)(xmax - xmin) | ((unsigned)(ymax - ymin) << 16);
                r.pitch = (unsigned)nc * PIXB;
                r.npix = (unsigned)(nc * nr);
                r.base = (unsigned)(ymin * W2 + xmin) * PIXB;
                r.skip = rowb - (unsigned)nc * PIXB;
                r.inv_nc = 1.0f / (float)nc;
                r.pad = 0;
                *(reinterpret_cast<UnitRec*>(lds + UNIT0) + jc * V + pv) = r;
            }
            const bool any_bad = __builtin_amdgcn_ballot_w64(mine && nc * nr > WINPIX) != 0;
            if ((tid & 63) == 0) *reinterpret_cast<unsigned*>(lds + PROBE0 + (jc * 4 + wv) * 4) = any_bad ? 1u : 0u;
        }
        __syncthreads();
        unsigned m = 0;
        for (int jc = 0; jc < nchunks; ++jc) {
            const u32x4 f = *reinterpret_cast<const u32x4*>(lds + PROBE0 + jc * 16);
            if ((f.x | f.y | f.z | f.w) == 0) m |= 1u << jc;
        }
        lds_chunks = (unsigned)__builtin_amdgcn_readfirstlane((int)m);
        if constexpr ((MVD_K3T_KO & 16) != 0) lds_chunks = 0;
    }

    auto locate = [&](int jc, int v, int slot, int wb) {
        if constexpr ((MVD_K3T_KO & 8) != 0) return;
        const int t = opaque_tid(), lpx = t & 31, li = t >> 5;
        const float lfx = (float)min(x0 + lpx % TW, w - 1), lfy = (float)min(y0 + lpx / TW, h - 1);
        const float depth = *reinterpret_cast<const float*>(lds + DEP0 + (jc * P + li) * 4);
        const ViewRec* vr = reinterpret_cast<const ViewRec*>(lds + VIEW0) + v;
        const float4 m0 = *reinterpret_cast<const float4*>(vr->M), m1 = *reinterpret_cast<const float4*>(vr->M + 4),
                     m2 = *reinterpret_cast<const float4*>(vr->M + 8);
        const float M[12] = {m0.x, m0.y, m0.z, m0.w, m1.x, m1.y, m1.z, m1.w, m2.x, m2.y, m2.z, m2.w};
        float ix, iy;
        position(M, lfx, lfy, depth, ix, iy);
        const float xf = floorf(ix), yf = floorf(iy);
        const float wx = ix - xf, wy = iy - yf;
        const float ux = 1.0f - wx, uy = 1.0f - wy;
        *reinterpret_cast<float4*>(lds + TABW0 + slot * 4096 + t * 16) = make_float4(ux * uy, wx * uy, ux * wy, wx * wy);
        unsigned* const ent = reinterpret_cast<unsigned*>(lds + TABO0 + slot * 1024 + (lpx * P + li) * 4);
        const int cx = (int)xf + 1, cy = (int)yf + 1;
        if (wb < 0) {
            *ent = (unsigned)(cy * W2 + cx) * PIXB;
        } else {
            const u32x4 rec = *reinterpret_cast<const u32x4*>(lds + UNIT0 + (jc * V + v) * sizeof(UnitRec));
            const unsigned dx = (unsigned)cx - (rec.x & 0xffffu), dy = (unsigned)cy - (rec.x >> 16);
            *ent = (unsigned)wb * WINB + dy * rec.z + dx * PIXB;
            const bool outside = dx > (rec.y & 0xffffu) || dy > (rec.y >> 16);
            if (__builtin_amdgcn_ballot_w64(outside) != 0) {
                if ((t & 63) == 0) *reinterpret_cast<unsigned*>(lds + FAIL0 + jc * 4) = 1u;
            }
        }
    };

    auto copy_window = [&](int jc, int v, int wb) {
        if constexpr ((MVD_K3T_KO & 1) != 0) return;
        const char* rp = lds + UNIT0 + (jc * V + v) * sizeof(UnitRec);
        const u32x4 ra = *reinterpret_cast<const u32x4*>(rp), rb = *reinterpret_cast<const u32x4*>(rp + 16);
        const u32x2 sb = *reinterpret_cast<const u32x2*>(lds + VIEW0 + v * sizeof(ViewRec) + 48);
        const u32x4 rsrc = {(unsigned)__builtin_amdgcn_readfirstlane((int)sb.x), (unsigned)__builtin_amdgcn_readfirstlane((int)sb.y) & 0xffffu,
                            img_bytes, 0x00020000u};
        const int npix = __builtin_amdgcn_readfirstlane((int)ra.w);
        const int ln = opaque_tid() & 63;
        const float inv_nc = __uint_as_float(rb.z);
        const unsigned base = rb.x + (unsigned)(ln % LPX) * 16u + (unsigned)(ln / LPX) * PIXB;
        const float nf0 = (float)(ln / LPX) + 0.5f;
#pragma unroll
        for (int k = 0; k < (NPIECE + 3) / 4; ++k) {
            const int piece = wv + 4 * k;
            if (piece * PPP < npix) {
                const int r = (int)((nf0 + (float)(piece * PPP)) * inv_nc);
                lds_dma_b128(rsrc, base + (unsigned)(piece * 1024) + (unsigned)r * rb.y, (unsigned)(wb * WINB + piece * 1024));
            }
        }
    };

    auto blend = [&](Sums (&sm)[P], int jc, int v, int slot, auto lds_tag) {
        constexpr bool LDSTAPS = decltype(lds_tag)::value;
        const int t = opaque_tid();
        const unsigned q_b = (unsigned)(t & 7) * QB;
        const char* tw = lds + TABW0 + slot * 4096 + (t >> 3) * 16;
        const char* to = lds + TABO0 + slot * 1024 + (t >> 3) * 32;
        const u32x4 oa = *reinterpret_cast<const u32x4*>(to), ob = *reinterpret_cast<const u32x4*>(to + 16);
        const unsigned ofs[P] = {oa.x, oa.y, oa.z, oa.w, ob.x, ob.y, ob.z, ob.w};
        unsigned pitch = 0;
        __amdgpu_buffer_rsrc_t rsrc;
        if constexpr (LDSTAPS) pitch = *reinterpret_cast<const unsigned*>(lds + UNIT0 + (jc * V + v) * sizeof(UnitRec) + 8);
        else rsrc = src_rsrc(v);
        auto weights = [&](int i) { return *reinterpret_cast<const float4*>(tw + i * (NPX * 16)); };
        auto taps = [&](int i, TAP (&f)[4]) {
            const unsigned o = ofs[i] + q_b;
            if constexpr ((MVD_K3T_KO & 2) != 0) {
                if constexpr (F16) { f[0] = u32x2{o, o + 1}; f[1] = u32x2{o + 2, o + 3}; f[2] = u32x2{o + pitch, o + 5}; f[3] = u32x2{o + 6, o + 7}; }
                else { f[0] = u32x4{o, o + 1, o + 2, o + 3}; f[1] = u32x4{o + 4, o + 5, o + 6, o + 7};
                       f[2] = u32x4{o + pitch, o + 9, o + 10, o + 11}; f[3] = u32x4{o + 12, o + 13, o + 14, o + 15}; }
            } else if constexpr (LDSTAPS) {
                f[0] = *reinterpret_cast<const TAP*>(lds + o);
                f[1] = *reinterpret_cast<const TAP*>(lds + o + PIXB);
                f[2] = *reinterpret_cast<const TAP*>(lds + o + pitch);
                f[3] = *reinterpret_cast<const TAP*>(lds + o + pitch + PIXB);
            } else if constexpr (F16) {
                f[0] = load_b64(rsrc, o, 0); f[1] = load_b64(rsrc, o + PIXB, 0);
                f[2] = load_b64(rsrc, o, rowb); f[3] = load_b64(rsrc, o + PIXB, rowb);
            } else {
                f[0] = __builtin_amdgcn_raw_buffer_load_b128(rsrc, o, 0, 0);
                f[1] = __builtin_amdgcn_raw_buffer_load_b128(rsrc, o + PIXB, 0, 0);
                f[2] = __builtin_amdgcn_raw_buffer_load_b128(rsrc, o, rowb, 0);
                f[3] = __builtin_amdgcn_raw_buffer_load_b128(rsrc, o + PIXB, rowb, 0);
            }
        };
        auto next = [&](int i, float4& wq, TAP (&f)[4], Sums& done) {
            wq = weights(i);
            unsigned oi = ofs[i];
            asm volatile("" : "+v"(done.a1[0]), "+v"(done.a1[1]), "+v"(done.a2[0]), "+v"(done.a2[1]), "+v"(oi));
            if (__builtin_amdgcn_ballot_w64(oi != ofs[i - SETS]) != 0) {
                const unsigned o = oi + q_b;
                if constexpr ((MVD_K3T_KO & 2) != 0) { taps(i, f); }
                else if constexpr (LDSTAPS) {
                    f[0] = *reinterpret_cast<const TAP*>(lds + o);
                    f[1] = *reinterpret_cast<const TAP*>(lds + o + PIXB);
                    f[2] = *reinterpret_cast<const TAP*>(lds + o + pitch);
                    f[3] = *reinterpret_cast<const TAP*>(lds + o + pitch + PIXB);
                } else if constexpr (F16) {
                    f[0] = load_b64(rsrc, o, 0); f[1] = load_b64(rsrc, o + PIXB, 0);
                    f[2] = load_b64(rsrc, o, rowb); f[3] = load_b64(rsrc, o + PIXB, rowb);
                } else {
                    f[0] = __builtin_amdgcn_raw_buffer_load_b128(rsrc, o, 0, 0);
                    f[1] = __builtin_amdgcn_raw_buffer_load_b128(rsrc, o + PIXB, 0, 0);
                    f[2] = __builtin_amdgcn_raw_buffer_load_b128(rsrc, o, rowb, 0);
                    f[3] = __builtin_amdgcn_raw_buffer_load_b128(rsrc, o + PIXB, rowb, 0);
                }
            }
        };
        if constexpr (SETS == 2) {
            float4 wA = weights(0), wB = weights(1);
            TAP fA[4], fB[4];
            taps(0, fA);
            taps(1, fB);
            __builtin_amdgcn_sched_barrier(0);
#pragma unroll
            for (int i = 0; i < P; i += 2) {
                accumulate_cell_pk(sm[i], wA, fA);
                __builtin_amdgcn_sched_barrier(0);
                if (i + 2 < P) next(i + 2, wA, fA, sm[i]);
                __builtin_amdgcn_sched_barrier(0);
                accumulate_cell_pk(sm[i + 1], wB, fB);
                __builtin_amdgcn_sched_barrier(0);
                if (i + 3 < P) next(i + 3, wB, fB, sm[i + 1]);
                __builtin_amdgcn_sched_barrier(0);
            }
        } else {
            float4 wA = weights(0);
            TAP fA[4];
            taps(0, fA);
            __builtin_amdgcn_sched_barrier(0);
#pragma unroll
            for (int i = 0; i < P; ++i) {
                accumulate_cell_pk(sm[i], wA, fA);
                __builtin_amdgcn_sched_barrier(0);
                if (i + 1 < P) next(i + 1, wA, fA, sm[i]);
                __builtin_amdgcn_sched_barrier(0);
            }
        }
    };

    auto reset_sums = [&](Sums (&sm)[P]) {
        const f32x2 klo = {key.x, key.y}, khi = {key.z, key.w};
#pragma unroll
        for (int i = 0; i < P; ++i) { sm[i].a1[0] = klo; sm[i].a1[1] = khi; sm[i].a2[0] = klo * klo; sm[i].a2[1] = khi * khi; }
    };

    float amax = 0.f;
    const bool want_absmax = p.absmax != nullptr;
    auto store_chunk = [&](const Sums (&sm)[P], int c, bool drop) {
        int bx, by;
        const int t = opaque_tid();
        blend_pixel(t, bx, by);
        const unsigned out_off = ((unsigned)by * (unsigned)w + (unsigned)bx) * PIXB + (unsigned)(t & 7) * QB;
        const unsigned long long plane0 = (unsigned long long)(reinterpret_cast<char*>(p.out) + ((size_t)b * D + (size_t)c * P) * plane_bytes);
        const int nvalid = drop ? 0 : min(P, D - c * P);
#pragma unroll
        for (int i = 0; i < P; ++i) {
            const float mx = sm[i].a1[0].x * inv_nv, my = sm[i].a1[0].y * inv_nv, mz = sm[i].a1[1].x * inv_nv, mw = sm[i].a1[1].y * inv_nv;
            const float4 r = make_float4(fmaf(sm[i].a2[0].x, inv_nv, -mx * mx), fmaf(sm[i].a2[0].y, inv_nv, -my * my),
                                         fmaf(sm[i].a2[1].x, inv_nv, -mz * mz), fmaf(sm[i].a2[1].y, inv_nv, -mw * mw));
            const unsigned long long pb = plane0 + (i < nvalid ? (unsigned long long)i * plane_bytes : 0ull);
            const __amdgpu_buffer_rsrc_t orsrc = __builtin_amdgcn_make_buffer_rsrc(reinterpret_cast<char*>(pb), 0, i < nvalid ? (int)plane_bytes : 0, 0x00020000);
            if constexpr ((MVD_K3T_KO & 4) != 0) { if (r.x != 123.456f) continue; }
            if (want_absmax && i < nvalid) {
                const float qm = fmaxf(fmaxf(fabsf(r.x), fabsf(r.y)), fmaxf(fabsf(r.z), fabsf(r.w)));
                const bool fin = fabsf(r.x) + fabsf(r.y) + fabsf(r.z) + fabsf(r.w) <= 3.402823466e38f;
                amax = fin ? fmaxf(amax, qm) : amax;
            }
            if constexpr (F16) {
                const f16x2 lo = {(_Float16)r.x, (_Float16)r.y}, hi = {(_Float16)r.z, (_Float16)r.w};
                store_b64(u32x2{as_u32(lo), as_u32(hi)}, orsrc, out_off);
            } else {
                __builtin_amdgcn_raw_buffer_store_b128(u32x4{__float_as_uint(r.x), __float_as_uint(r.y), __float_as_uint(r.z), __float_as_uint(r.w)},
                                                       orsrc, out_off, 0, 0);
            }
        }
    };

#define MVD_UNIT_BARRIER(NST) asm volatile("s_waitcnt vmcnt(" #NST ") lgkmcnt(0)\n\ts_barrier" ::: "memory")
    auto first_chunk = [](unsigned mask) { return mask ? (int)__builtin_ctz(mask) : -1; };
    auto advance = [&](unsigned mask, int& jc, int& v) {
        if (++v < V) return;
        v = 0;
        const unsigned rest = jc >= 31 ? 0u : (mask >> (jc + 1));
        jc = rest ? jc + 1 + (int)__builtin_ctz(rest) : -1;
    };
    std::integral_constant<bool, true> yes;
    std::integral_constant<bool, false> no;

    if (lds_chunks) {
        const unsigned mask = lds_chunks;
        int jb = first_chunk(mask);
        copy_window(jb, 0, 0);
        locate(jb, 0, 0, 0);
        MVD_UNIT_BARRIER(0);
        int slot = 0;
        while (jb >= 0) {
            const unsigned rest = jb >= 31 ? 0u : (mask >> (jb + 1));
            const int jn = rest ? jb + 1 + (int)__builtin_ctz(rest) : -1;
            Sums sm[P];
            reset_sums(sm);
            for (int v = 0; v + 1 < V; ++v) {
                copy_window(jb, v + 1, slot ^ 1);
                blend(sm, jb, v, slot, yes);
                locate(jb, v + 1, slot ^ 1, slot ^ 1);
                MVD_UNIT_BARRIER(0);
                slot ^= 1;
            }
            if (jn >= 0) copy_window(jn, 0, slot ^ 1);
            blend(sm, jb, V - 1, slot, yes);
            {
                const bool drop = __builtin_amdgcn_readfirstlane((int)*reinterpret_cast<const unsigned*>(lds + FAIL0 + jb * 4)) != 0;
                store_chunk(sm, chunk_of(jb), drop);
            }
            if (jn >= 0) locate(jn, 0, slot ^ 1, slot ^ 1);
            MVD_UNIT_BARRIER(8);
            slot ^= 1;
            jb = jn;
        }
    }

    unsigned failed = 0;
    for (int jc = 0; jc < nchunks; ++jc)
        if (*reinterpret_cast<const unsigned*>(lds + FAIL0 + jc * 4) != 0) failed |= 1u << jc;
    failed = (unsigned)__builtin_amdgcn_readfirstlane((int)failed);
    const unsigned all = nchunks >= 32 ? 0xffffffffu : ((1u << nchunks) - 1u);
    const unsigned gmask = (all & ~lds_chunks) | failed;
    if (gmask) {
        int jl = first_chunk(gmask), vl = 0;
        locate(jl, vl, 0, -1); advance(gmask, jl, vl);
        int jb = first_chunk(gmask), vb = 0, slot = 0;
        Sums sm[P];
        reset_sums(sm);
        while (jb >= 0) {
            MVD_UNIT_BARRIER(8);
            if (jl >= 0) { locate(jl, vl, slot ^ 1, -1); advance(gmask, jl, vl); }
            blend(sm, jb, vb, slot, no);
            if (vb + 1 == V) {
                store_chunk(sm, chunk_of(jb), false);
                reset_sums(sm);
            }
            slot ^= 1;
            advance(gmask, jb, vb);
        }
    }
#undef MVD_UNIT_BARRIER
    if (want_absmax) {
        unsigned m = __float_as_uint(amax);
        m = max(m, row_shr<1>(m)); m = max(m, row_shr<2>(m)); m = max(m, row_shr<4>(m)); m = max(m, row_shr<8>(m));
        m = max(m, (unsigned)__builtin_amdgcn_update_dpp((int)m, (int)m, 0x142, 0xa, 0xf, false));
        m = max(m, (unsigned)__builtin_amdgcn_update_dpp((int)m, (int)m, 0x143, 0xc, 0xf, false));
        unsigned* wm = reinterpret_cast<unsigned*>(lds + PROBE0);
        __syncthreads();
        if ((tid & 63) == 63) wm[wv] = m;
        __syncthreads();
        if (tid == 0) raise_absmax(p.absmax, __uint_as_float(max(max(wm[0], wm[1]), max(wm[2], wm[3]))));
    }
}

static size_t tile_lds_bytes(int win, bool f16, int V, int nch) {
    return 2 * (size_t)win * (f16 ? 64 : 128) + 2 * 4096 + 2 * 1024 + 512 + 128 + (size_t)V * sizeof(ViewRec) + (size_t)nch * 32 +
           (size_t)nch * V * sizeof(UnitRec);
}

template <int TW, int WINPIX, bool F16, bool EXACT, int MINW, int SETS>
static int launch_tile_variant(const WarpParams& p, const dim3& grid, hipStream_t st, int nch) {
    const size_t lds = tile_lds_bytes(WINPIX, F16, p.V, nch);
    auto* fn = warp_variance_tile_kernel<TW, WINPIX, F16, EXACT, MINW, SETS>;
    if (lds > 48 * 1024) {
        if (hipFuncSetAttribute(reinterpret_cast<const void*>(fn), hipFuncAttributeMaxDynamicSharedMemorySize, (int)lds) != hipSuccess)
            return launch_status("warp_variance_tile: hipFuncSetAttribute");
    }
    hipLaunchKernelGGL(fn, grid, dim3(256), lds, st, p, nch);
    return MVD_OK;
}

bool warp_tile_supported(const WarpParams& p, bool f16) {
    return p.h + 3 < 65536 && p.w + 3 < 65536 && (long long)p.h * p.w * (f16 ? 64 : 128) < 0x7fffffffLL && p.V <= 32;
}

int launch_warp_tile(const WarpParams& p0, hipStream_t st, int tw, int win, int nch, int sets, bool f16, bool exact) {
    WarpParams p = p0;
    const int th = 32 / tw;
    p.tiles_x = (p.w + tw - 1) / tw;
    p.tiles_y = (p.h + th - 1) / th;
    const long long tiles = (long long)p.tiles_x * p.tiles_y;
    p.tiles_per_xcd = (int)((tiles + 7) / 8);
    const int dchunks = (p.D + 7) / 8;
    nch = nch < 1 ? 1 : (nch > 32 ? 32 : nch);
    const size_t budget = (size_t)160 * 1024 / (sets == 1 ? 4 : 3);
    while (nch > 1 && tile_lds_bytes(win, f16, p.V, nch) > budget) --nch;
    const int dgroups = (dchunks + nch - 1) / nch;
    const long long nblk = 8LL * p.tiles_per_xcd * dgroups * p.B;
    if (nblk > 0x7fffffffLL) {
        set_error("warp_variance: %lld workgroups exceed the grid limit", nblk);
        return MVD_ERR_INVALID_ARG;
    }
    const dim3 grid((unsigned)nblk);
    int rc = MVD_ERR_INVALID_ARG;
    timing_begin(st);
#define MVD_T(TW_, WIN_, MW_, SETS_)                                                                                   \
    if (tw == TW_ && win == WIN_ && sets == SETS_) {                                                                  \
        rc = f16 ? (exact ? launch_tile_variant<TW_, WIN_, true, true, MW_, SETS_>(p, grid, st, nch)                  \
                          : launch_tile_variant<TW_, WIN_, true, false, MW_, SETS_>(p, grid, st, nch))                \
                 : (exact ? launch_tile_variant<TW_, WIN_, false, true, MW_, SETS_>(p, grid, st, nch)                 \
                          : launch_tile_variant<TW_, WIN_, false, false, MW_, SETS_>(p, grid, st, nch));              \
    }
    MVD_T(8, 104, 4, 1) MVD_T(8, 128, 4, 1)
#ifdef MVD_EXPERIMENTS
    MVD_T(8, 128, 3, 2) MVD_T(8, 96, 4, 1) MVD_T(16, 128, 3, 2) MVD_T(16, 104, 4, 1) MVD_T(16, 96, 4, 1) MVD_T(32, 128, 3, 2) MVD_T(32, 104, 4, 1)
#endif
#undef MVD_T
    timing_end(st);
    if (rc == MVD_ERR_INVALID_ARG) {
        set_error("warp_variance: tile variant tw=%d win=%d sets=%d is not compiled", tw, win, sets);
        return rc;
    }
    if (rc) return rc;
    return launch_status("warp_variance_tile");
}

}
```

### robustmvd_amd/models.py

```python
import math

import numpy as np
import torch
import torch.nn as nn

from . import _lib as L
from . import ops
from .blocks import (CostRegNet, DispnetContextEncoder, DispnetCostvolumeEncoder, DispnetDecoder, DispnetEncoder,
                     FeatureNet, LearnedFusion, PlanesweepCorrelation)
from .registry import build_model_with_cfg, register_model
from .utils import exclude_index, get_torch_model_device, select_by_index, to_numpy, to_torch


def _key_positions(keyview_idx, n):
    if isinstance(keyview_idx, torch.Tensor):
        keyview_idx = keyview_idx.detach().cpu().numpy()
    k = np.asarray(keyview_idx).reshape(-1)
    if k.size == 1:
        return [int(k[0])] * n
    if k.size != n:
        raise ValueError(f"keyview_idx has {k.size} entries for a batch of {n}")
    return [int(v) for v in k]


def _upscale_to_multiple(images, intrinsics, m, device):
    orig_ht, orig_wd = images[0].shape[-2:]
    ht, wd = int(math.ceil(orig_ht / m) * m), int(math.ceil(orig_wd / m) * m)
    images = [im.float() for im in to_torch(list(images), device=device)]
    if ht != orig_ht or wd != orig_wd:
        if any(tuple(im.shape[-2:]) != (orig_ht, orig_wd) for im in images):
            raise ValueError("all views must have the size of the first one to be resized together (transforms.py:56-66)")
        images = [ops.resize_order1(im, ht, wd) for im in images]
        if intrinsics is not None:
            scale = np.array([[wd / orig_wd] * 3, [ht / orig_ht] * 3, [1.0] * 3], dtype=np.float32)
            intrinsics = [(k.detach().cpu().numpy() if isinstance(k, torch.Tensor) else np.asarray(k)) * scale
                          for k in intrinsics]
    return images, intrinsics, ht, wd


def _stack_views(images, fn):
    if len(images) < 2 or any(im.shape != images[0].shape for im in images):
        return [fn(im).float() for im in images]
    buf = torch.empty((len(images),) + tuple(images[0].shape), dtype=torch.float32, device=images[0].device)
    for i, im in enumerate(images):
        buf[i].copy_(fn(im))
    return [buf[i] for i in range(len(images))]


def _as_batch(views):
    v0 = views[0]
    if len(views) == 1:
        return v0
    step = v0.numel() * v0.element_size()
    if all(v.shape == v0.shape and v.dtype == v0.dtype and v.is_contiguous() and v.untyped_storage().data_ptr() == v0.untyped_storage().data_ptr()
           and v.data_ptr() == v0.data_ptr() + i * step for i, v in enumerate(views)):
        return torch.as_strided(v0, (len(views) * v0.shape[0],) + tuple(v0.shape[1:]), v0.stride())
    return torch.cat(list(views), 0)


class RobustMVD(nn.Module):
    def __init__(self, half_dispnet=False, engine_dispnet=True):
        super().__init__()
        self.half_dispnet = bool(half_dispnet)
        self.engine_dispnet = bool(engine_dispnet)
        self._engine = None
        self.encoder = DispnetEncoder()
        self.context_encoder = DispnetContextEncoder()
        self.corr_block = PlanesweepCorrelation()
        self.fusion_block = LearnedFusion()
        self.fusion_enc_block = DispnetCostvolumeEncoder()
        self.decoder = DispnetDecoder()
        for m in self.modules():
            if isinstance(m, (nn.Conv2d, nn.ConvTranspose2d)):
                nn.init.kaiming_normal_(m.weight, a=0.2, nonlinearity="leaky_relu")
                if m.bias is not None:
                    nn.init.zeros_(m.bias)

    SWEEP = dict(num_sampling_points=256, min_depth=0.4, max_depth=1000.0)

    def _prepare(self):
        dev = next(self.parameters()).device
        if dev.type == "cuda":
            self.corr_block.warm(sampling_type="linear_invdepth", device=dev, **self.SWEEP)

    def forward(self, images, poses, intrinsics, keyview_idx, **_):
        half = self.half_dispnet and images[0].is_cuda and not torch.is_grad_enabled()
        with torch.autocast("cuda", dtype=torch.float16, enabled=half):
            pred, aux = self._forward(images, poses, intrinsics, keyview_idx)
        if half:
            f32 = lambda v: [x.float() for x in v] if isinstance(v, list) else v.float()
            pred = {k: f32(v) for k, v in pred.items()}
            aux = {k: f32(v) for k, v in aux.items()}
        return pred, aux

    def _forward(self, images, poses, intrinsics, keyview_idx):
        key_pos = _key_positions(keyview_idx, images[0].shape[0])
        keyview_idx = key_pos[0] if all(k == key_pos[0] for k in key_pos) else key_pos
        image_key = select_by_index(images, keyview_idx)
        images_source = exclude_index(images, keyview_idx)
        intrinsics_key = select_by_index(intrinsics, keyview_idx)
        intrinsics_source = exclude_index(intrinsics, keyview_idx)
        source_to_key = exclude_index(poses, keyview_idx)

        n = image_key.shape[0]
        same = all(im.shape == image_key.shape for im in images_source)
        if (self.engine_dispnet and same and image_key.is_cuda and image_key.dtype == torch.float32 and not torch.is_grad_enabled()
                and not torch.is_autocast_enabled() and image_key.shape[-2] % 64 == 0 and image_key.shape[-1] % 64 == 0):
            if self._engine is None:
                from .dispnet_engine import DispnetEngine
                self._engine = DispnetEngine(self)
            dec = self._engine.forward(image_key, images_source, intrinsics_key, intrinsics_source, source_to_key)
            return self._outputs(dec)
        if same:
            feats = self.encoder.conv3(self.encoder.conv2(self.encoder.conv1(_as_batch(images_source))))
            enc_sources = list(torch.split(feats, n, 0))
        else:
            enc_sources = [self.encoder(im)[1] for im in images_source]
        all_enc_key, enc_key = self.encoder(image_key)
        ctx = self.context_encoder(enc_key)

        corrs, masks, _ = self.corr_block(
            feat_key=enc_key, intrinsics_key=intrinsics_key, feat_sources=enc_sources,
            source_to_key_transforms=source_to_key, intrinsics_sources=intrinsics_source,
            **self.SWEEP)
        fused_corr, _ = self.fusion_block(corrs=corrs, masks=masks)
        all_enc_fused, enc_fused = self.fusion_enc_block(corr=fused_corr, ctx=ctx)
        dec = self.decoder(enc_fused=enc_fused, all_enc={**all_enc_key, **all_enc_fused})
        return self._outputs(dec)

    @staticmethod
    def _outputs(dec):
        inv, log_b = dec["invdepth"].float(), dec["invdepth_log_b"].float()
        pred = {"depth": 1 / (inv + 1e-9), "depth_uncertainty": torch.exp(log_b) / (inv + 1e-9)}
        aux = dec
        aux["depth"], aux["depth_uncertainty"] = pred["depth"], pred["depth_uncertainty"]
        return pred, aux

    def input_adapter(self, images, keyview_idx, poses, intrinsics, **_):
        device = get_torch_model_device(self)
        images, intrinsics, ht, wd = _upscale_to_multiple(images, intrinsics, 64, device)
        scale = np.array([[wd] * 3, [ht] * 3, [1.0] * 3], dtype=np.float32)
        intrinsics = [k / scale for k in intrinsics]
        poses, intrinsics = to_torch((poses, intrinsics), device=device)
        keyview_idx = to_torch(keyview_idx)
        c255 = torch.full((1,), 255.0, dtype=torch.float32, device=device)
        images = _stack_views(images, lambda im: im / c255 - 0.4)
        poses = [p.float() for p in poses]
        intrinsics = [k.float() for k in intrinsics]
        return {"images": images, "keyview_idx": keyview_idx, "poses": poses, "intrinsics": intrinsics}

    def output_adapter(self, model_output):
        pred, aux = model_output
        return to_numpy(pred), to_numpy(aux)


class MVSNet(nn.Module):
    def __init__(self, sample_in_inv_depth_space=False, num_sampling_steps=192, half_features=False, conv0_split=True,
                 exact_grid=False, train_regulariser="vendor", sweep_backward="atomic"):
        super().__init__()
        if train_regulariser not in ("vendor", "engine"):
            raise ValueError(f"train_regulariser must be 'vendor' or 'engine', got {train_regulariser!r}")
        self.train_regulariser = train_regulariser
        if sweep_backward not in ops.K3_BACKWARDS:
            raise ValueError(f"sweep_backward must be 'atomic' or 'gather', got {sweep_backward!r}")
        self.sweep_backward = sweep_backward
        if sweep_backward == "gather":
            self.register_buffer("sweep_backward_fallbacks", torch.zeros(1, dtype=torch.int32), persistent=False)
        self.half_features = bool(half_features)
        if sample_in_inv_depth_space:
            raise NotImplementedError("sample_in_inv_depth_space=True is a dead branch in the reference "
                                      "(tensor[::-1] raises, mvsnet.py:50,56-63)")
        self.feature = FeatureNet(split_layers=conv0_split)
        self.cost_regularization = CostRegNet(conv0_split=conv0_split)
        self.exact_grid = bool(exact_grid)
        self.num_sampling_steps = num_sampling_steps
        self.sample_in_inv_depth_space = False
        self._intrinsics_scale_host = torch.tensor([[0.25] * 3, [0.25] * 3, [1.0] * 3])
        self.register_buffer("intrinsics_scale", self._intrinsics_scale_host.clone(), persistent=False)

    def depth_samples(self, depth_range, n, device):
        D = self.num_sampling_steps
        if depth_range is None:
            return torch.linspace(0.2, 100.0, D, dtype=torch.float32, device=device).expand(n, D).contiguous()
        lo, hi = depth_range[0], depth_range[1]
        if not (isinstance(lo, torch.Tensor) and lo.is_cuda) and not (isinstance(hi, torch.Tensor) and hi.is_cuda):
            lo = float(torch.as_tensor(lo, dtype=torch.float32).reshape(-1)[0])
            hi = float(torch.as_tensor(hi, dtype=torch.float32).reshape(-1)[0])
            d = torch.linspace(lo, hi, D, dtype=torch.float32)
            return d.expand(n, D).contiguous().to(device, non_blocking=True)
        lo = torch.as_tensor(lo, dtype=torch.float32, device=device).reshape(-1)[0]
        hi = torch.as_tensor(hi, dtype=torch.float32, device=device).reshape(-1)[0]
        i = torch.arange(D, dtype=torch.float32, device=device)
        step = (hi - lo) / (D - 1)
        d = torch.where(i < D // 2, lo + step * i, hi - step * (D - 1 - i))
        return d.expand(n, D).contiguous()

    def projection_matrices(self, intrinsics, poses, key_pos, device):
        on_host = not intrinsics[0].is_cuda and not poses[0].is_cuda
        scale = self._intrinsics_scale_host if on_host else self.intrinsics_scale
        out = []
        for v, (K, T) in enumerate(zip(intrinsics, poses)):
            P = T.float().clone()
            P[:, :3, :4] = torch.matmul(K.float() * scale, P[:, :3, :4])
            if any(k == v for k in key_pos):
                inv = torch.linalg.inv(P) if on_host else torch.linalg.inv_ex(P, check_errors=False).inverse
                if all(k == v for k in key_pos):
                    P = inv
                else:
                    sel = torch.tensor([k == v for k in key_pos], device=P.device).view(-1, 1, 1)
                    P = torch.where(sel, inv, P)
            out.append(P)
        if on_host:
            packed = torch.stack(out, 0).to(device, non_blocking=True)
            out = list(packed.unbind(0))
        return out

    def _records_graph(self):
        return self.training or (torch.is_grad_enabled() and any(p.requires_grad for p in self.parameters()))

    def forward(self, images, poses, intrinsics, keyview_idx, depth_range=None, **_):
        n = images[0].shape[0]
        device = images[0].device
        key_pos = _key_positions(keyview_idx, n)
        kidx = key_pos[0] if all(k == key_pos[0] for k in key_pos) else key_pos
        depth_samples = self.depth_samples(depth_range, n, device)
        proj = self.projection_matrices(intrinsics, poses, key_pos, device)
        views = [select_by_index(images, kidx)] + exclude_index(images, kidx)
        projs = [select_by_index(proj, kidx)] + exclude_index(proj, kidx)
        if self._records_graph():
            return self._forward_autograd(views, projs, depth_samples, n)

        split = self.cost_regularization.conv0_split and not self.half_features
        feats = self.feature.forward_layout(_as_batch(views), L.LAYOUT_NHWC_BORDER, return_absmax=split)
        if split:
            feats, a_feat = feats
        if self.half_features:
            feats = ops.to_f16(feats)
        feats = list(torch.split(feats, n, 0))
        amax = None
        if self.half_features:
            var = ops.warp_variance_f16(feats[0], feats[1:], projs[1:], projs[0], depth_samples)
        else:
            var = ops.warp_variance(feats[0], feats[1:], projs[1:], projs[0], depth_samples, channels_last=True, staged=True,
                                    exact_grid=self.exact_grid)
            if split:
                amax = a_feat * a_feat
        cost = self.cost_regularization.forward_channels_last(var, x_absmax=amax)
        del var
        depth, conf = ops.softmax_regress(cost, depth_samples)
        pred = {"depth": depth.unsqueeze(1), "depth_uncertainty": (1 - conf).unsqueeze(1)}
        return pred, {}

    def _forward_autograd(self, views, projs, depth_samples, n):
        if self.half_features:
            raise ValueError("MVSNet(half_features=True) is inference-only: call .eval() and run under torch.no_grad()")
        feats = list(torch.split(self.feature.forward_autograd(_as_batch(views)), n, 0))
        if self.sweep_backward == "gather":
            var = ops.warp_variance_autograd(feats[0], feats[1:], projs[1:], projs[0], depth_samples, backward="gather",
                                             fallback_count=self.sweep_backward_fallbacks)
        else:
            var = ops.warp_variance_autograd(feats[0], feats[1:], projs[1:], projs[0], depth_samples)
        if self.train_regulariser == "engine":
            cost = self.cost_regularization.forward_autograd_engine(var.permute(0, 2, 3, 4, 1).contiguous())
        else:
            cost = self.cost_regularization.forward_autograd(var).squeeze(1)
        depth, conf = ops.softmax_regress_autograd(cost, depth_samples)
        pred = {"depth": depth.unsqueeze(1), "depth_uncertainty": (1 - conf).unsqueeze(1)}
        return pred, {}

    def input_adapter(self, images, keyview_idx, poses=None, intrinsics=None, depth_range=None, masks=None):
        device = get_torch_model_device(self)
        images, intrinsics, _, _ = _upscale_to_multiple(images, intrinsics, 32, device)
        masks = to_torch(masks, device=device)
        mean = torch.tensor([0.485, 0.456, 0.406], dtype=torch.float64, device=device).view(-1, 1, 1)
        std = torch.tensor([0.229, 0.224, 0.225], dtype=torch.float64, device=device).view(-1, 1, 1)
        c255 = torch.full((1,), 255.0, dtype=torch.float32, device=device)
        images = _stack_views(images, lambda im: ((im.float() / c255).double() - mean) / std)
        keyview_idx, depth_range, intrinsics, poses = to_torch((keyview_idx, depth_range, intrinsics, poses))
        return {"images": images, "poses": poses, "intrinsics": intrinsics,
                "keyview_idx": keyview_idx, "depth_range": depth_range, "masks": masks}

    def output_adapter(self, model_output):
        pred, aux = model_output
        return to_numpy(pred), to_numpy(aux)


@register_model
def robust_mvd(pretrained=True, weights=None, train=False, num_gpus=1, **kwargs):
    if pretrained and weights is None:
        raise RuntimeError("robust_mvd: the pretrained weights are URL-only (robust_mvd.py:153) and there is no network; "
                           "pass weights=<path to robustmvd_600k.pt> or pretrained=False")
    return build_model_with_cfg(model_cls=RobustMVD, weights=weights, train=train, num_gpus=num_gpus, **kwargs)


@register_model(trainable=False)
def robust_mvd_5M(pretrained=True, weights=None, train=False, num_gpus=1, **kwargs):
    if pretrained and weights is None:
        raise RuntimeError("robust_mvd_5M: the pretrained weights are URL-only (robust_mvd.py:142); pass weights=<path>")
    return build_model_with_cfg(model_cls=RobustMVD, weights=weights, train=train, num_gpus=num_gpus)


@register_model(trainable=False)
def mvsnet_train(pretrained=True, weights=None, train=False, num_gpus=1, **kwargs):
    assert not (pretrained and weights is None), "Pretrained weights are not available for this model."
    cfg = {"sample_in_inv_depth_space": False, "num_sampling_steps": 256}
    return build_model_with_cfg(model_cls=MVSNet, cfg=cfg, weights=weights, train=train, num_gpus=num_gpus, **kwargs)
```

### robustmvd_amd/ops.py

```python
import ctypes
import functools
import itertools

import torch

from . import _lib as L


def _tensors(obj):
    if isinstance(obj, torch.Tensor):
        yield obj
    elif isinstance(obj, (list, tuple)):
        for o in obj:
            yield from _tensors(o)
    elif isinstance(obj, dict):
        for o in obj.values():
            yield from _tensors(o)


def inference_only(fn):
    @functools.wraps(fn)
    def wrapper(*args, **kwargs):
        if torch.is_grad_enabled():
            if any(t.requires_grad for t in _tensors((args, kwargs))):
                raise RuntimeError(f"{fn.__qualname__}: an input requires grad, but this HIP path is inference-only (no "
                                   "backward is implemented); call it under torch.no_grad() or detach the inputs")
            owner = args[0] if args and isinstance(args[0], torch.nn.Module) else None
            if owner is not None and owner.training and any(p.requires_grad for p in owner.parameters()):
                raise RuntimeError(f"{fn.__qualname__}: the module is in training mode with trainable parameters and autograd is "
                                   "recording, but this HIP path is inference-only; call .eval() and run it under torch.no_grad()")
        with torch.no_grad():
            return fn(*args, **kwargs)
    return wrapper


def call(name, dev, *args):
    argv, keep = list(args), []
    for i, a in enumerate(args):
        t = type(a)
        if t is int or t is float or a is None:
            continue
        if t is list or t is tuple:
            argv[i], arr = L.ptr_array(a)
            keep.append(arr)
        elif isinstance(a, torch.Tensor):
            argv[i] = a.data_ptr()
    with torch.cuda.device(dev):
        rc = getattr(L.load(), name)(*argv, L.raw_stream(dev))
    L.check(rc, name)


def views(ts, name, V=None):
    ts = list(ts)
    if len(ts) == 0 or len(ts) > L.MVD_MAX_VIEWS:
        raise ValueError(f"{name}: {len(ts)} views, supported 1..{L.MVD_MAX_VIEWS}")
    if V is not None and len(ts) != V:
        raise ValueError(f"{name}: {len(ts)} entries for {V} views")
    return ts


def workspace(nbytes, device):
    return torch.empty(max(int(nbytes), 16), dtype=torch.uint8, device=device)


def _invdepth_mode(inv, N, h, w):
    if inv.dim() == 2 and inv.shape[0] in (1, N):
        return L.INVDEPTH_BATCHED if (inv.shape[0] == N and N > 1) else L.INVDEPTH_SHARED
    if inv.dim() == 4 and tuple(inv.shape[0:1] + inv.shape[2:]) == (N, h, w):
        return L.INVDEPTH_PER_PIXEL
    raise ValueError(f"sampling_invdepths must be (1 or N, S) or (N, S, h, w), got {tuple(inv.shape)}")


def _k1_calibration(K_key, K_sources, T_src2key, invdepths, V, N, h, w, dev):
    Kk = L.as_f32(K_key, "intrinsics_key", (N, 3, 3), dev)
    Ks = [L.as_f32(k, f"intrinsics_sources[{i}]", (N, 3, 3), dev) for i, k in enumerate(views(K_sources, "intrinsics_sources", V))]
    Ts = [L.as_f32(t, f"source_to_key_transforms[{i}]", (N, 4, 4), dev) for i, t in enumerate(views(T_src2key, "source_to_key_transforms", V))]
    inv = L.as_f32(invdepths, "sampling_invdepths", device=dev)
    return Kk, Ks, Ts, inv, _invdepth_mode(inv, N, h, w)


def _corr_scale(corr_scale, C):
    return float(corr_scale) if corr_scale is not None else 1.0 / float(C) ** 0.5


def _k3_depths(depth_values, B, C, dev):
    dv = L.as_f32(depth_values, "depth_values", device=dev)
    if dv.dim() != 2 or dv.shape[0] != B:
        raise ValueError(f"depth_values must be (B,D), got {tuple(dv.shape)}")
    if C not in (4, 8, 16, 32, 64):
        raise ValueError(f"feature channels C={C} unsupported (4, 8, 16, 32, 64)")
    return dv


def _k3_calibration(src_projs, key_proj_inv, depth_values, V, B, C, dev):
    projs = [L.as_f32(p, f"src_projs[{i}]", (B, 4, 4), dev) for i, p in enumerate(views(src_projs, "src_projs", V))]
    kpi = L.as_f32(key_proj_inv, "key_proj_inv", (B, 4, 4), dev)
    return projs, kpi, _k3_depths(depth_values, B, C, dev)


@inference_only
def sweep_corr(feat_key, feat_sources, K_key, K_sources, T_src2key, invdepths, corr_scale=None):
    fk = L.as_f32(feat_key, "feat_key")
    if fk.dim() != 4:
        raise ValueError("feat_key must be (N,C,h,w)")
    N, C, h, w = fk.shape
    dev = fk.device
    srcs = views(feat_sources, "feat_sources")
    V = len(srcs)
    hs, ws = srcs[0].shape[-2:]
    srcs = [L.as_f32(s, f"feat_sources[{i}]", (N, C, hs, ws), dev) for i, s in enumerate(srcs)]
    Kk, Ks, Ts, inv, mode = _k1_calibration(K_key, K_sources, T_src2key, invdepths, V, N, h, w, dev)
    S = inv.shape[1]
    scale = _corr_scale(corr_scale, C)
    if C % 64 != 0:
        raise ValueError(f"feature channels C={C} must be a multiple of 64")
    corrs = [torch.empty((N, S, h, w), dtype=torch.float32, device=dev) for _ in range(V)]
    masks = [torch.empty((N, S, h, w), dtype=torch.float32, device=dev) for _ in range(V)]
    wsb = L.load().mvd_sweep_corr_workspace_bytes(N, C, h, w, hs, ws, V)
    call("mvd_sweep_corr_ex_f32", dev, fk, srcs, Kk, Ks, Ts, inv, mode, scale, N, C, h, w, hs, ws, S, V, corrs, masks,
          workspace(wsb, dev), wsb)
    return corrs, masks


@inference_only
def sweep_warp(feat_sources, K_key, K_sources, T_src2key, invdepths, key_size, normalize_after=False):
    srcs = views(feat_sources, "feat_sources")
    V = len(srcs)
    s0 = L.as_f32(srcs[0], "feat_sources[0]")
    if s0.dim() != 4:
        raise ValueError("feat_sources must be (N,C,hs,ws)")
    N, C, hs, ws = s0.shape
    dev = s0.device
    h, w = int(key_size[0]), int(key_size[1])
    srcs = [L.as_f32(s, f"feat_sources[{i}]", (N, C, hs, ws), dev) for i, s in enumerate(srcs)]
    Kk, Ks, Ts, inv, mode = _k1_calibration(K_key, K_sources, T_src2key, invdepths, V, N, h, w, dev)
    S = inv.shape[1]
    outs = [torch.empty((N, S, C, h, w), dtype=torch.float32, device=dev) for _ in range(V)]
    masks = [torch.empty((N, S, h, w), dtype=torch.float32, device=dev) for _ in range(V)]
    call("mvd_sweep_warp_f32", dev, srcs, Kk, Ks, Ts, inv, mode, 1 if normalize_after else 0, N, C, h, w, hs, ws, S, V, outs, masks)
    return outs, masks


@inference_only
def fuse_views(corrs, masks, scores):
    corrs = views(corrs, "corrs")
    V = len(corrs)
    c0 = L.as_f32(corrs[0], "corrs[0]")
    N, S, h, w = c0.shape
    dev = c0.device
    corrs = [L.as_f32(c, f"corrs[{i}]", (N, S, h, w), dev) for i, c in enumerate(corrs)]
    masks = [L.as_f32(m, f"masks[{i}]", (N, S, h, w), dev) for i, m in enumerate(views(masks, "masks", V))]
    scores = [L.as_f32(s, f"scores[{i}]", (N, 1, h, w), dev) for i, s in enumerate(views(scores, "scores", V))]
    fused = torch.empty_like(c0)
    fmask = torch.empty_like(c0)
    call("mvd_fuse_views_f32", dev, corrs, masks, scores, N, S, h, w, V, fused, fmask)
    return fused, fmask


@inference_only
def warp_variance(key_feat, src_feats, src_projs, key_proj_inv, depth_values, channels_last=False, exact_grid=False,
                  staged=False, return_absmax=False):
    kf = L.as_f32(key_feat, "key_feat")
    if kf.dim() != 4:
        raise ValueError("key_feat must be (B,C,h,w)" + (" / (B,h+3,w+3,C) when staged" if staged else ""))
    if staged:
        B, h, w, C = kf.shape[0], kf.shape[1] - 3, kf.shape[2] - 3, kf.shape[3]
    else:
        B, C, h, w = kf.shape
    dev = kf.device
    srcs = [L.as_f32(s, f"src_feats[{i}]", tuple(kf.shape), dev) for i, s in enumerate(views(src_feats, "src_feats"))]
    V = len(srcs)
    projs, kpi, dv = _k3_calibration(src_projs, key_proj_inv, depth_values, V, B, C, dev)
    D = dv.shape[1]
    out = torch.empty((B, D, h, w, C) if channels_last else (B, C, D, h, w), dtype=torch.float32, device=dev)
    wsb = L.load().mvd_warp_variance_workspace_bytes(B, C, h, w, 0 if staged else V)
    flags = (L.LAYOUT_NDHWC if channels_last else L.LAYOUT_NCDHW) | (L.GRID_EXACT if exact_grid else 0) | \
        (L.FEAT_NHWC_BORDER if staged else 0)
    name, amax = "mvd_warp_variance_f32", []
    if return_absmax:
        name, amax = "mvd_warp_variance_absmax_f32", [torch.empty(1, dtype=torch.float32, device=dev)]
    call(name, dev, kf, srcs, projs, kpi, dv, B, C, D, h, w, V, out, *amax, flags, workspace(wsb, dev), wsb)
    return (out, amax[0]) if return_absmax else out


@inference_only
def absmax(x):
    x = L.as_f32(x, "x")
    out = torch.empty(1, dtype=torch.float32, device=x.device)
    call("mvd_absmax_f32", x.device, x, x.numel(), out)
    return out


@inference_only
def to_f16(x):
    x = L.as_f32(x, "x")
    y = torch.empty(x.shape, dtype=torch.float16, device=x.device)
    call("mvd_convert_f32_to_f16", x.device, x, y, x.numel())
    return y


@inference_only
def warp_variance_f16(key_feat, src_feats, src_projs, key_proj_inv, depth_values):
    kf = L.as_f16(key_feat, "key_feat")
    if kf.dim() != 4 or kf.shape[3] != 32:
        raise ValueError("key_feat must be the fp16 zero-bordered channel-last map (B,h+3,w+3,32)")
    B, h, w = kf.shape[0], kf.shape[1] - 3, kf.shape[2] - 3
    dev = kf.device
    srcs = [L.as_f16(s, f"src_feats[{i}]", tuple(kf.shape), dev) for i, s in enumerate(views(src_feats, "src_feats"))]
    V = len(srcs)
    projs, kpi, dv = _k3_calibration(src_projs, key_proj_inv, depth_values, V, B, 32, dev)
    D = dv.shape[1]
    out = torch.empty((B, D, h, w, 32), dtype=torch.float16, device=dev)
    wsb = L.load().mvd_warp_variance_f16_workspace_bytes(B)
    call("mvd_warp_variance_f16", dev, kf, srcs, projs, kpi, dv, B, D, h, w, V, out, workspace(wsb, dev), wsb)
    return out


@inference_only
def homo_warp(src_feat, src_proj, ref_proj_inv, depth_values):
    sf = L.as_f32(src_feat, "src_feat")
    if sf.dim() != 4:
        raise ValueError("src_feat must be (B,C,H,W)")
    B, C, h, w = sf.shape
    dev = sf.device
    sp = L.as_f32(src_proj, "src_proj", (B, 4, 4), dev)
    kpi = L.as_f32(ref_proj_inv, "ref_proj_inv", (B, 4, 4), dev)
    dv = _k3_depths(depth_values, B, C, dev)
    D = dv.shape[1]
    out = torch.empty((B, C, D, h, w), dtype=torch.float32, device=dev)
    wsb = L.load().mvd_warp_variance_workspace_bytes(B, C, h, w, 0)
    call("mvd_homo_warp_f32", dev, sf, sp, kpi, dv, B, C, D, h, w, out, workspace(wsb, dev), wsb)
    return out


def _conv3d_channels(weight, mode):
    if weight.dim() != 5 or tuple(weight.shape[2:]) != (3, 3, 3):
        raise ValueError(f"weight must be (*,*,3,3,3), got {tuple(weight.shape)}")
    return (weight.shape[0], weight.shape[1]) if mode == L.DECONV3D_STRIDE2 else (weight.shape[1], weight.shape[0])


def _conv3d_out_size(mode, Di, hi, wi):
    if mode == L.CONV3D_STRIDE1:
        return Di, hi, wi
    if mode == L.CONV3D_STRIDE2:
        if Di % 2 or hi % 2 or wi % 2:
            raise ValueError(f"stride-2 conv needs even D,h,w, got {Di},{hi},{wi}")
        return Di // 2, hi // 2, wi // 2
    if mode == L.DECONV3D_STRIDE2:
        return Di * 2, hi * 2, wi * 2
    raise ValueError(f"mode {mode}")


@inference_only
def pack_conv3d_weights(weight, mode):
    wt = L.as_f32(weight, "weight")
    Cin, Cout = _conv3d_channels(wt, mode)
    n = L.load().mvd_conv3d_packed_weight_floats(Cin, Cout)
    if n == 0:
        raise ValueError(f"conv3d: Cin={Cin}, Cout={Cout} unsupported (Cin in 8/16/32/64, Cout in 1/8/16/32/64; Cin 1 with Cout 4, 8 .. 64)")
    packed = torch.empty(n, dtype=torch.float32, device=wt.device)
    call("mvd_pack_conv3d_weights_f32", wt.device, wt, Cin, Cout, mode, packed)
    return packed, Cin, Cout


@inference_only
def conv3d_bn_relu(x, packed, Cin, Cout, scale, shift, mode, relu=True, skip=None, return_absmax=False):
    x = L.as_f32(x, "x")
    if x.dim() != 5 or x.shape[-1] != Cin:
        raise ValueError(f"x must be (B,D,h,w,{Cin}) channel-last, got {tuple(x.shape)}")
    B, Di, hi, wi, _ = x.shape
    dev = x.device
    oshape = (B, *_conv3d_out_size(mode, Di, hi, wi), Cout)
    scale = L.as_f32(scale, "scale", (Cout,), dev)
    shift = L.as_f32(shift, "shift", (Cout,), dev)
    if skip is not None:
        skip = L.as_f32(skip, "skip", oshape, dev)
    y = torch.empty(oshape, dtype=torch.float32, device=dev)
    name, amax = "mvd_conv3d_bn_relu_f32", []
    if return_absmax:
        name, amax = "mvd_conv3d_bn_relu_absmax_f32", [torch.empty(1, dtype=torch.float32, device=dev)]
    call(name, dev, x, packed, scale, shift, skip, y, *amax, B, Di, hi, wi, Cin, Cout, mode, int(bool(relu)))
    return (y, amax[0]) if return_absmax else y


@inference_only
def pack_conv3d_weights_f16(weight):
    wt = L.as_f32(weight, "weight")
    if tuple(wt.shape) != (8, 32, 3, 3, 3):
        raise ValueError(f"conv3d f16: only the 32 -> 8 first layer is built, got weight {tuple(wt.shape)}")
    packed = torch.empty(L.load().mvd_conv3d_f16_packed_weight_bytes(32, 8), dtype=torch.uint8, device=wt.device)
    call("mvd_pack_conv3d_weights_f16", wt.device, wt, 32, 8, packed)
    return packed


@inference_only
def conv3d_bn_relu_f16in(x, packed, scale, shift, relu=True):
    x = L.as_f16(x, "x")
    if x.dim() != 5 or x.shape[-1] != 32:
        raise ValueError(f"x must be (B,D,h,w,32) fp16 channel-last, got {tuple(x.shape)}")
    B, D, h, w, _ = x.shape
    dev = x.device
    scale = L.as_f32(scale, "scale", (8,), dev)
    shift = L.as_f32(shift, "shift", (8,), dev)
    y = torch.empty((B, D, h, w, 8), dtype=torch.float32, device=dev)
    call("mvd_conv3d_bn_relu_f16in", dev, x, packed, scale, shift, y, B, D, h, w, 32, 8, int(bool(relu)))
    return y


def _split3d_inputs(x, cin, cout, out_size, scale, shift, skip, x_absmax):
    x = L.as_f32(x, "x")
    if x.dim() != 5 or x.shape[-1] != cin:
        raise ValueError(f"x must be (B,D,h,w,{cin}) channel-last, got {tuple(x.shape)}")
    dev = x.device
    oshape = (x.shape[0], *out_size(*x.shape[1:4]), cout)
    scale = L.as_f32(scale, "scale", (cout,), dev)
    shift = L.as_f32(shift, "shift", (cout,), dev)
    if skip is not None:
        skip = L.as_f32(skip, "skip", oshape, dev)
    return x, scale, shift, skip, L.as_f32(x_absmax, "x_absmax", (1,), dev), oshape


def _absmax_slot(return_absmax, out_absmax, dev):
    if not return_absmax:
        return None
    if out_absmax is not None:
        return L.as_f32(out_absmax, "out_absmax", (1,), dev)
    return torch.zeros(1, dtype=torch.float32, device=dev)


@inference_only
def pack_conv3d_weights_split(weight):
    wt = L.as_f32(weight, "weight")
    cout, cin = (wt.shape[0], wt.shape[1]) if wt.dim() == 5 else (0, 0)
    if wt.dim() != 5 or tuple(wt.shape[2:]) != (3, 3, 3) or cin not in (16, 32) or cout % 8 or not 8 <= cout <= 64:
        raise ValueError(f"conv3d split: 16 or 32 input channels and 8..64 output channels (a multiple of 8) are built, got weight {tuple(wt.shape)}")
    packed = torch.empty(L.load().mvd_conv3d_split_packed_weight_bytes(cin, cout), dtype=torch.uint8, device=wt.device)
    call("mvd_pack_conv3d_weights_split", wt.device, wt, cin, cout, packed)
    return packed


@inference_only
def conv3d_bn_relu_split(x, packed, scale, shift, relu=True, x_absmax=None, return_absmax=False):
    x = L.as_f32(x, "x")
    if x.dim() != 5 or x.shape[-1] not in (16, 32):
        raise ValueError(f"x must be (B,D,h,w,16 or 32) channel-last, got {tuple(x.shape)}")
    B, D, h, w, cin = x.shape
    dev = x.device
    scale = L.as_f32(scale, "scale", device=dev)
    cout = scale.numel()
    if packed.numel() != L.load().mvd_conv3d_split_packed_weight_bytes(cin, cout):
        raise ValueError(f"packed weights of {packed.numel()} bytes do not belong to a {cin} -> {cout} layer")
    shift = L.as_f32(shift, "shift", (cout,), dev)
    y = torch.empty((B, D, h, w, cout), dtype=torch.float32, device=dev)
    if x_absmax is None:
        x_absmax = absmax(x)
    x_absmax = L.as_f32(x_absmax, "x_absmax", (1,), dev)
    name, yam = "mvd_conv3d_bn_relu_f32_split", []
    if return_absmax:
        name, yam = "mvd_conv3d_bn_relu_absmax_f32_split", [torch.empty(1, dtype=torch.float32, device=dev)]
    call(name, dev, x, x_absmax, packed, scale, shift, y, *yam, B, D, h, w, cin, cout, int(bool(relu)))
    return (y, yam[0]) if return_absmax else y


@inference_only
def pack_conv3d_weights_igemm(weight, mode):
    wt = L.as_f32(weight, "weight")
    cin, cout = _conv3d_channels(wt, mode)
    n = L.load().mvd_conv3d_igemm_packed_weight_bytes(cin, cout, mode)
    if n == 0:
        raise ValueError(f"conv3d igemm: {cin} -> {cout} channels, mode {mode} is not built (Cin a multiple of 8 (16 transposed), Cout of 4)")
    packed = torch.empty(n, dtype=torch.uint8, device=wt.device)
    call("mvd_pack_conv3d_weights_igemm", wt.device, wt, cin, cout, mode, packed)
    return packed


@inference_only
def conv3d_bn_relu_igemm(x, x_absmax, packed, Cin, Cout, scale, shift, mode, relu=True, skip=None, return_absmax=False, out_absmax=None):
    lib = L.load()
    x, scale, shift, skip, xam, oshape = _split3d_inputs(x, Cin, Cout, lambda d, h, w: _conv3d_out_size(mode, d, h, w), scale, shift, skip,
                                                         x_absmax)
    B, Di, hi, wi, _ = x.shape
    dev = x.device
    if packed.numel() != lib.mvd_conv3d_igemm_packed_weight_bytes(Cin, Cout, mode):
        raise ValueError(f"packed weights of {packed.numel()} bytes do not belong to a {Cin} -> {Cout} layer of mode {mode}")
    y = torch.empty(oshape, dtype=torch.float32, device=dev)
    yam = _absmax_slot(return_absmax, out_absmax, dev)
    wsb = lib.mvd_conv3d_igemm_workspace_bytes(B, Di, hi, wi, Cin, Cout, mode)
    call("mvd_conv3d_bn_relu_igemm_f32", dev, x, xam, packed, scale, shift, skip, y, yam, B, Di, hi, wi, Cin, Cout, mode,
          int(bool(relu)), workspace(wsb, dev) if wsb else None, wsb)
    return (y, yam) if return_absmax else y


@inference_only
def pack_deconv3d_weights_split(weight):
    wt = L.as_f32(weight, "weight")
    cin, cout = _conv3d_channels(wt, L.DECONV3D_STRIDE2)
    n = L.load().mvd_deconv3d_split_packed_weight_bytes(cin, cout)
    if n == 0:
        raise ValueError(f"deconv3d split: {cin} -> {cout} channels is not built (32 or 64 -> 16, 32, 48 or 64; 16 -> 8)")
    packed = torch.empty(n, dtype=torch.uint8, device=wt.device)
    call("mvd_pack_deconv3d_weights_split", wt.device, wt, cin, cout, packed)
    return packed


@inference_only
def deconv3d_bn_relu_split(x, x_absmax, packed, Cin, Cout, scale, shift, relu=True, skip=None, return_absmax=False, out_absmax=None):
    x, scale, shift, skip, xam, oshape = _split3d_inputs(x, Cin, Cout, lambda d, h, w: (2 * d, 2 * h, 2 * w), scale, shift, skip, x_absmax)
    B, Di, hi, wi, _ = x.shape
    dev = x.device
    n = L.load().mvd_deconv3d_split_packed_weight_bytes(Cin, Cout)
    if n == 0 or packed.numel() != n:
        raise ValueError(f"packed weights of {packed.numel()} bytes do not belong to a transposed {Cin} -> {Cout} layer")
    y = torch.empty(oshape, dtype=torch.float32, device=dev)
    yam = _absmax_slot(return_absmax, out_absmax, dev)
    call("mvd_deconv3d_bn_relu_f32_split", dev, x, xam, packed, scale, shift, skip, y, yam, B, Di, hi, wi, Cin, Cout, int(bool(relu)))
    return (y, yam) if return_absmax else y


@inference_only
def pack_conv2d_weights(weight):
    wt = L.as_f32(weight, "weight")
    if wt.dim() != 4 or wt.shape[2] != wt.shape[3]:
        raise ValueError(f"weight must be (Cout,Cin,k,k), got {tuple(wt.shape)}")
    Cout, Cin, k = wt.shape[0], wt.shape[1], wt.shape[2]
    n = L.load().mvd_conv2d_packed_weight_floats(Cin, Cout, k)
    if n == 0:
        raise ValueError(f"conv2d: Cin={Cin}, Cout={Cout}, k={k} unsupported (Cin in 3/8/16/32, Cout in 8/16/32, k in 3/5)")
    packed = torch.empty(n, dtype=torch.float32, device=wt.device)
    call("mvd_pack_conv2d_weights_f32", wt.device, wt, Cin, Cout, k, packed)
    return packed, Cin, Cout, k


@inference_only
def conv2d_head(image, w0, scale0, shift0, w1, scale1, shift1, return_absmax=False):
    x = L.as_f32(image, "image")
    if x.dim() != 4 or x.shape[1] != 3:
        raise ValueError(f"image must be (B,3,H,W), got {tuple(x.shape)}")
    B, _, H, W = x.shape
    dev = x.device
    w0 = L.as_f32(w0, "w0", (3, 3, 3, 8), dev)
    w1 = L.as_f32(w1, "w1", (3, 3, 8, 8), dev)
    vs = [L.as_f32(v, n, (8,), dev) for v, n in ((scale0, "scale0"), (shift0, "shift0"), (scale1, "scale1"), (shift1, "shift1"))]
    y = torch.empty((B, H, W, 8), dtype=torch.float32, device=dev)
    tiles = torch.empty(L.load().mvd_conv2d_head_tile_count(B, H, W), dtype=torch.float32, device=dev) if return_absmax else None
    call("mvd_conv2d_head_f32", dev, x, w0, vs[0], vs[1], w1, vs[2], vs[3], y, tiles, B, H, W)
    return (y, absmax(tiles)) if return_absmax else y


@inference_only
def pack_conv2d_head_weights_split(weight1):
    wt = L.as_f32(weight1, "weight1")
    if tuple(wt.shape) != (8, 8, 3, 3):
        raise ValueError(f"conv2d_head split: conv1's weight is (8,8,3,3), got {tuple(wt.shape)}")
    packed = torch.empty(L.load().mvd_conv2d_head_split_packed_bytes(), dtype=torch.uint8, device=wt.device)
    call("mvd_pack_conv2d_head_split_weights", wt.device, wt, packed)
    return packed


@inference_only
def conv2d_head_split(image, w0, scale0, shift0, w1_packed, scale1, shift1, return_absmax=False):
    x = L.as_f32(image, "image")
    if x.dim() != 4 or x.shape[1] != 3:
        raise ValueError(f"image must be (B,3,H,W), got {tuple(x.shape)}")
    B, _, H, W = x.shape
    dev = x.device
    w0 = L.as_f32(w0, "w0", (3, 3, 3, 8), dev)
    n = L.load().mvd_conv2d_head_split_packed_bytes()
    if w1_packed.dtype != torch.uint8 or w1_packed.numel() != n or w1_packed.device != dev or not w1_packed.is_contiguous():
        raise ValueError(f"w1_packed: pack_conv2d_head_weights_split's {n} bytes on {dev} expected")
    vs = [L.as_f32(v, n_, (8,), dev) for v, n_ in ((scale0, "scale0"), (shift0, "shift0"), (scale1, "scale1"), (shift1, "shift1"))]
    y = torch.empty((B, H, W, 8), dtype=torch.float32, device=dev)
    tiles = torch.empty(L.load().mvd_conv2d_head_tile_count(B, H, W), dtype=torch.float32, device=dev) if return_absmax else None
    call("mvd_conv2d_head_split_f32", dev, x, w0, vs[0], vs[1], w1_packed, vs[2], vs[3], y, tiles, B, H, W)
    return (y, absmax(tiles)) if return_absmax else y


def conv2d_bn_relu(x, packed, Cin, Cout, ksize, stride, scale, shift, relu=True, out_layout=L.LAYOUT_NHWC, out=None, out_absmax=None):
    x = L.as_f32(x, "x")
    if Cin == 3:
        if x.dim() != 4 or x.shape[1] != 3:
            raise ValueError(f"x must be (B,3,H,W), got {tuple(x.shape)}")
        B, _, hi, wi = x.shape
        in_layout = L.LAYOUT_NCHW
    else:
        if x.dim() != 4 or x.shape[-1] != Cin:
            raise ValueError(f"x must be (B,h,w,{Cin}) channel-last, got {tuple(x.shape)}")
        B, hi, wi, _ = x.shape
        in_layout = L.LAYOUT_NHWC
    if (ksize, stride) not in ((3, 1), (5, 2)):
        raise ValueError(f"conv2d: kernel {ksize} stride {stride} unsupported (3/1 or 5/2)")
    dev = x.device
    ho, wo = (hi - 1) // stride + 1, (wi - 1) // stride + 1
    oshape = {L.LAYOUT_NHWC: (B, ho, wo, Cout), L.LAYOUT_NCHW: (B, Cout, ho, wo),
              L.LAYOUT_NHWC_BORDER: (B, ho + 3, wo + 3, Cout)}.get(out_layout)
    if oshape is None:
        raise ValueError(f"out_layout {out_layout}")
    scale = L.as_f32(scale, "scale", (Cout,), dev)
    shift = L.as_f32(shift, "shift", (Cout,), dev)
    if out is not None:
        y = L.as_f32(out, "out", oshape, dev)
        if y.data_ptr() != out.data_ptr():
            raise ValueError("out must be a contiguous fp32 tensor")
    elif out_layout == L.LAYOUT_NHWC_BORDER:
        y = torch.zeros(oshape, dtype=torch.float32, device=dev)
    else:
        y = torch.empty(oshape, dtype=torch.float32, device=dev)
    name, yam = "mvd_conv2d_bn_relu_f32", []
    if out_absmax is not None:
        name, yam = "mvd_conv2d_bn_relu_absmax_f32", [L.as_f32(out_absmax, "out_absmax", (1,), dev)]
    call(name, dev, x, in_layout, packed, scale, shift, y, *yam, out_layout, B, hi, wi, Cin, Cout, ksize, stride, int(bool(relu)))
    return y


# ... 1271 lines not shown
```

Measured before the change: 346.7 depth-maps/sec.

## Emit pre-split fp16 hi/lo volume from warp-variance for conv0

The warp-variance tile kernel gains a split store mode. Using a bound on the volume's absmax computed before the kernel runs, it writes each variance value already split into two fp16 terms (hi and lo words) instead of an fp32 value. Conv0 reads these words directly and skips its in-kernel range scaling and fp32 split. This is meant to take splitting work out of conv0's inner loop, at the cost of a new kernel variant and a scale that comes from a prior bound rather than the measured absmax.

```diff
diff --git a/include/mvd.h b/include/mvd.h
--- a/include/mvd.h
+++ b/include/mvd.h
@@ -74,6 +74,11 @@
                                  const float* key_proj_inv, const float* depth_values, int B, int C, int D, int h, int w,
                                  int V, float* var_out, float* absmax_out, int out_layout, void* workspace,
                                  size_t workspace_bytes, mvd_stream_t stream);
+int mvd_warp_variance_split_supported(int C, int h, int w, int V, int out_layout);
+int mvd_warp_variance_split_f32(const float* key_feat, const float* const* src_feat, const float* const* src_proj,
+                                const float* key_proj_inv, const float* depth_values, int B, int C, int D, int h, int w, int V,
+                                const float* split_absmax, void* split_out, int out_layout, void* workspace, size_t workspace_bytes,
+                                mvd_stream_t stream);
 
 size_t mvd_warp_variance_f16_workspace_bytes(int B);
 int mvd_warp_variance_f16(const void* key_feat, const void* const* src_feat, const float* const* src_proj,
@@ -114,6 +119,11 @@
 int mvd_conv3d_bn_relu_absmax_f32_split(const float* x, const float* x_absmax, const void* packed_w, const float* scale, const float* shift,
                                         float* y, float* y_absmax, int B, int D, int h, int w, int Cin, int Cout, int relu,
                                         mvd_stream_t stream);
+int mvd_conv3d_bn_relu_presplit(const void* x_split, const float* x_absmax, const void* packed_w, const float* scale, const float* shift,
+                                float* y, int B, int D, int h, int w, int Cin, int Cout, int relu, mvd_stream_t stream);
+int mvd_conv3d_bn_relu_absmax_presplit(const void* x_split, const float* x_absmax, const void* packed_w, const float* scale,
+                                       const float* shift, float* y, float* y_absmax, int B, int D, int h, int w, int Cin, int Cout,
+                                       int relu, mvd_stream_t stream);
 size_t mvd_conv3d_igemm_packed_weight_bytes(int Cin, int Cout, int mode);
 int mvd_pack_conv3d_weights_igemm(const float* w, int Cin, int Cout, int mode, void* packed, mvd_stream_t stream);
 size_t mvd_conv3d_igemm_workspace_bytes(int B, int Di, int Hi, int Wi, int Cin, int Cout, int mode);
diff --git a/robustmvd_amd/_lib.py b/robustmvd_amd/_lib.py
--- a/robustmvd_amd/_lib.py
+++ b/robustmvd_amd/_lib.py
@@ -50,6 +50,9 @@
                               + [_c_float_p, _i, ctypes.c_void_p, _sz, ctypes.c_void_p]),
     "mvd_warp_variance_absmax_f32": (_i, [_c_float_p, _pp, _pp, _c_float_p, _c_float_p] + [_i] * 6
                                      + [_c_float_p, _c_float_p, _i, ctypes.c_void_p, _sz, ctypes.c_void_p]),
+    "mvd_warp_variance_split_supported": (_i, [_i] * 5),
+    "mvd_warp_variance_split_f32": (_i, [_c_float_p, _pp, _pp, _c_float_p, _c_float_p] + [_i] * 6
+                                    + [_c_float_p, ctypes.c_void_p, _i, ctypes.c_void_p, _sz, ctypes.c_void_p]),
     "mvd_absmax_f32": (_i, [_c_float_p, ctypes.c_longlong, _c_float_p, ctypes.c_void_p]),
     "mvd_warp_variance_f16_workspace_bytes": (_sz, [_i]),
     "mvd_warp_variance_f16": (_i, [ctypes.c_void_p, _pp, _pp, _c_float_p, _c_float_p] + [_i] * 5
@@ -83,6 +86,10 @@
     "mvd_pack_conv3d_weights_split": (_i, [_c_float_p, _i, _i, ctypes.c_void_p, ctypes.c_void_p]),
     "mvd_conv3d_bn_relu_f32_split": (_i, [_c_float_p, _c_float_p, ctypes.c_void_p, _c_float_p, _c_float_p, _c_float_p] + [_i] * 7
                                      + [ctypes.c_void_p]),
+    "mvd_conv3d_bn_relu_presplit": (_i, [ctypes.c_void_p, _c_float_p, ctypes.c_void_p, _c_float_p, _c_float_p, _c_float_p] + [_i] * 7
+                                    + [ctypes.c_void_p]),
+    "mvd_conv3d_bn_relu_absmax_presplit": (_i, [ctypes.c_void_p, _c_float_p, ctypes.c_void_p, _c_float_p, _c_float_p, _c_float_p,
+                                                _c_float_p] + [_i] * 7 + [ctypes.c_void_p]),
     "mvd_deconv3d_split_packed_weight_bytes": (_sz, [_i, _i]),
     "mvd_pack_deconv3d_weights_split": (_i, [_c_float_p, _i, _i, ctypes.c_void_p, ctypes.c_void_p]),
     "mvd_deconv3d_bn_relu_f32_split": (_i, [_c_float_p, _c_float_p, ctypes.c_void_p] + [_c_float_p] * 5 + [_i] * 7 + [ctypes.c_void_p]),
diff --git a/robustmvd_amd/blocks.py b/robustmvd_amd/blocks.py
--- a/robustmvd_amd/blocks.py
+++ b/robustmvd_amd/blocks.py
@@ -406,12 +406,21 @@
     def forward_channels_last(self, x, x_absmax=None):
         if x.shape[1] % 8 or x.shape[2] % 8 or x.shape[3] % 8:
             raise ValueError(f"CostRegNet needs D,h,w divisible by 8, got {tuple(x.shape[1:4])}")
+        presplit = isinstance(x, ops.SplitVolume)
+        if presplit and not self.conv0_split:
+            raise ValueError("CostRegNet(conv0_split=False) cannot read an ops.SplitVolume")
+        half_volume = not presplit and x.dtype == torch.float16
         pk = self._prepare()
         first = pk["conv0"]
-        split_decoder = self.conv0_split and x.dtype == torch.float32
-
-        if x.dtype == torch.float16:
+        split_decoder = self.conv0_split and not half_volume
+
+        if half_volume:
             conv0 = ops.conv3d_bn_relu_f16in(x, pk.conv0_f16, first.scale, first.shift, relu=True)
+        elif presplit:
+            x_absmax = x.absmax
+            conv0 = ops.conv3d_bn_relu_presplit(x, pk.conv0_split, first.scale, first.shift, relu=True)
+            gain0, off0 = pk.conv0_bound
+            a0 = (gain0 * x_absmax + off0).amax().reshape(1)
         elif self.conv0_split:
             if x_absmax is None:
                 x_absmax = ops.absmax(x)
@@ -430,7 +439,7 @@
                                              return_absmax=leave_absmax, out_absmax=slots.take() if leave_absmax else None)
                 return y if leave_absmax else (y, None)
 
-            if x.dtype == torch.float16:
+            if half_volume:
                 a0 = ops.absmax(conv0)
             t, a = igemm("conv1", conv0, a0)
             conv2, a = igemm("conv2", t, a)
diff --git a/robustmvd_amd/csrc/conv3d_split.hip b/robustmvd_amd/csrc/conv3d_split.hip
--- a/robustmvd_amd/csrc/conv3d_split.hip
+++ b/robustmvd_amd/csrc/conv3d_split.hip
@@ -17,7 +17,7 @@
 typedef _Float16 h16x2 __attribute__((ext_vector_type(2)));
 
 constexpr int S_TH = 4, S_TW = 32, S_ROWS = S_TH + 2;
-constexpr float S_LO_FACTOR = 2048.0f;
+constexpr float S_LO_FACTOR = CONV0_LO_FACTOR;
 template <int CIN>
 struct SplitGeom {
     static constexpr int CH8 = CIN / 8;
@@ -67,8 +67,9 @@
     return __builtin_bit_cast(unsigned, v);
 }
 
-template <int CIN, bool YAMAX = false>
+template <int CIN, bool YAMAX = false, bool PRESPLIT = false>
 __global__ void __launch_bounds__(256, 2) conv0_split_kernel(SplitParams p) {
+    static_assert(!PRESPLIT || CIN == 32, "the SPLIT32 volume has 32 channels");
     using G = SplitGeom<CIN>;
     constexpr int S_COLS = G::COLS, S_HALF_BYTES = G::HALF_BYTES, S_PLANE_BYTES = G::PLANE_BYTES, S_ITEMS = G::ITEMS, S_NLOAD = G::NLOAD;
     constexpr int KWG = G::KWG, NT = G::NT;
@@ -122,7 +123,15 @@
     char* const dump = ring + 2 * S_PLANE_BYTES + tid * 16;
     float xs, xs_inv;
     split_xscale(p.absmax, xs, xs_inv);
-    auto split2 = [xs](float a0, float a1, unsigned& hi, unsigned& lo) { mvd::split2(xs, a0, a1, hi, lo, S_LO_FACTOR); };
+    auto split_pair = [&](int k, int q, unsigned& hi, unsigned& lo) {
+        if constexpr (PRESPLIT) {
+            hi = pre[k][q >> 1][q & 1];
+            lo = pre[k][q >> 1][2 + (q & 1)];
+        } else {
+            const sf32x4 v = __builtin_bit_cast(sf32x4, pre[k][q >> 1]);
+            mvd::split2(xs, v[(q & 1) * 2], v[(q & 1) * 2 + 1], hi, lo, S_LO_FACTOR);
+        }
+    };
     auto stash = [&](int d) {
         char* slot = ring + (d & 1) * S_PLANE_BYTES;
 #pragma unroll
@@ -130,9 +139,8 @@
             su32x4 hv, lv;
 #pragma unroll
             for (int q = 0; q < 4; ++q) {
-                const sf32x4 v = __builtin_bit_cast(sf32x4, pre[k][q >> 1]);
                 unsigned hi, lo;
-                split2(v[(q & 1) * 2], v[(q & 1) * 2 + 1], hi, lo);
+                split_pair(k, q, hi, lo);
                 hv[q] = hi; lv[q] = lo;
             }
             char* dst = loff[k] >= 0 ? slot + loff[k] : dump;
@@ -246,9 +254,8 @@
                     __builtin_amdgcn_raw_buffer_store_b32(__float_as_uint(r), rs_out, ox + i < w ? yoff[row] + vox_b * i : OOB, 0, 0);
             } else if (!(SPLIT_KO & 4)) {
                 const int k = (g - 8) >> 2, q = (g - 8) & 3;
-                const sf32x4 v = __builtin_bit_cast(sf32x4, pre[k][q >> 1]);
                 unsigned hq1, lq1;
-                split2(v[(q & 1) * 2], v[(q & 1) * 2 + 1], hq1, lq1);
+                split_pair(k, q, hq1, lq1);
                 if (q & 1) {
                     char* dst = (loff[k] >= 0 ? wslot + loff[k] : dump) + 8 * (q >> 1);
                     *reinterpret_cast<su32x2*>(dst) = su32x2{hq0, hq1};
@@ -290,16 +297,16 @@
 static bool split_shape_ok(int Cin, int Cout) { return (Cin == 32 || Cin == 16) && Cout >= 8 && Cout <= 64 && Cout % 8 == 0; }
 static size_t split_frag_bytes(int Cin, int Cout) { return (size_t)(Cout / 8) * (Cin == 32 ? 27 : 18) * 64 * 16; }
 
-template <int CIN, bool YAMAX>
+template <int CIN, bool YAMAX, bool PRESPLIT>
 static int launch_split_v(const mvd::SplitParams& p, long long nblk, hipStream_t st) {
     const size_t lds = 2 * (size_t)mvd::SplitGeom<CIN>::PLANE_BYTES + 256 * 16;
-    (void)hipFuncSetAttribute((const void*)mvd::conv0_split_kernel<CIN, YAMAX>, hipFuncAttributeMaxDynamicSharedMemorySize, (int)lds);
-    hipLaunchKernelGGL((mvd::conv0_split_kernel<CIN, YAMAX>), dim3((unsigned)nblk), dim3(256), lds, st, p);
+    (void)hipFuncSetAttribute((const void*)mvd::conv0_split_kernel<CIN, YAMAX, PRESPLIT>, hipFuncAttributeMaxDynamicSharedMemorySize, (int)lds);
+    hipLaunchKernelGGL((mvd::conv0_split_kernel<CIN, YAMAX, PRESPLIT>), dim3((unsigned)nblk), dim3(256), lds, st, p);
     return mvd::launch_status("conv3d_split");
 }
-template <int CIN>
+template <int CIN, bool PRESPLIT = false>
 static int launch_split(const mvd::SplitParams& p, long long nblk, hipStream_t st) {
-    return p.yamax ? launch_split_v<CIN, true>(p, nblk, st) : launch_split_v<CIN, false>(p, nblk, st);
+    return p.yamax ? launch_split_v<CIN, true, PRESPLIT>(p, nblk, st) : launch_split_v<CIN, false, PRESPLIT>(p, nblk, st);
 }
 
 extern "C" {
@@ -321,7 +328,8 @@
 }
 
 static int conv3d_split_entry(const float* x, const float* x_absmax, const void* packed_w, const float* scale, const float* shift, float* y,
-                              float* y_absmax, int B, int D, int h, int w, int Cin, int Cout, int relu, mvd_stream_t stream);
+                              float* y_absmax, int B, int D, int h, int w, int Cin, int Cout, int relu, mvd_stream_t stream,
+                              bool presplit = false);
 
 int mvd_conv3d_bn_relu_f32_split(const float* x, const float* x_absmax, const void* packed_w, const float* scale, const float* shift,
                                  float* y, int B, int D, int h, int w, int Cin, int Cout, int relu, mvd_stream_t stream) {
@@ -335,10 +343,25 @@
     return conv3d_split_entry(x, x_absmax, packed_w, scale, shift, y, y_absmax, B, D, h, w, Cin, Cout, relu, stream);
 }
 
+int mvd_conv3d_bn_relu_presplit(const void* x_split, const float* x_absmax, const void* packed_w, const float* scale, const float* shift,
+                                float* y, int B, int D, int h, int w, int Cin, int Cout, int relu, mvd_stream_t stream) {
+    return conv3d_split_entry(static_cast<const float*>(x_split), x_absmax, packed_w, scale, shift, y, nullptr, B, D, h, w, Cin, Cout, relu,
+                              stream, true);
+}
+
+int mvd_conv3d_bn_relu_absmax_presplit(const void* x_split, const float* x_absmax, const void* packed_w, const float* scale,
+                                       const float* shift, float* y, float* y_absmax, int B, int D, int h, int w, int Cin, int Cout,
+                                       int relu, mvd_stream_t stream) {
+    MVD_REQUIRE(y_absmax, "conv3d_presplit_absmax: NULL argument");
+    return conv3d_split_entry(static_cast<const float*>(x_split), x_absmax, packed_w, scale, shift, y, y_absmax, B, D, h, w, Cin, Cout,
+                              relu, stream, true);
+}
+
 static int conv3d_split_entry(const float* x, const float* x_absmax, const void* packed_w, const float* scale, const float* shift, float* y,
-                              float* y_absmax, int B, int D, int h, int w, int Cin, int Cout, int relu, mvd_stream_t stream) {
+                              float* y_absmax, int B, int D, int h, int w, int Cin, int Cout, int relu, mvd_stream_t stream, bool presplit) {
     MVD_REQUIRE(x && x_absmax && packed_w && scale && shift && y, "conv3d_split: NULL argument");
     MVD_REQUIRE(split_shape_ok(Cin, Cout), "conv3d_split: 16 or 32 input channels and 8, 16, ... 64 output channels are built (got %d -> %d)", Cin, Cout);
+    MVD_REQUIRE(!presplit || Cin == 32, "conv3d_presplit: the split volume has 32 channels (got Cin = %d)", Cin);
     MVD_REQUIRE(B > 0 && D > 0 && h > 0 && w > 0, "conv3d_split: non-positive dimension");
     MVD_REQUIRE((long long)h * w * Cin * 4 < 0x7fffffffLL && (long long)h * w * Cout * 4 < 0x7fffffffLL,
                 "conv3d_split: one plane exceeds the 31-bit byte-offset range");
@@ -357,6 +380,7 @@
     p.dgroups = (D + td - 1) / td;
     const long long nblk = 8LL * p.ncb * p.tiles_per_xcd * p.dgroups * B;
     MVD_REQUIRE(nblk <= 0x7fffffffLL, "conv3d_split: %lld workgroups exceed the grid limit", nblk);
+    if (presplit) return launch_split<32, true>(p, nblk, (hipStream_t)stream);
     return Cin == 32 ? launch_split<32>(p, nblk, (hipStream_t)stream) : launch_split<16>(p, nblk, (hipStream_t)stream);
 }
 }
diff --git a/robustmvd_amd/csrc/split_operand.h b/robustmvd_amd/csrc/split_operand.h
--- a/robustmvd_amd/csrc/split_operand.h
+++ b/robustmvd_amd/csrc/split_operand.h
@@ -2,6 +2,8 @@
 #include "mvd_common.h"
 
 namespace mvd {
+
+constexpr float CONV0_LO_FACTOR = 2048.0f;
 
 __device__ __forceinline__ void split_xscale_of(unsigned max_bits, float& xsc, float& xsc_inv) {
     const int ex = (int)((max_bits >> 23) & 0xffu) - 127;
diff --git a/robustmvd_amd/csrc/warp_variance.hip b/robustmvd_amd/csrc/warp_variance.hip
--- a/robustmvd_amd/csrc/warp_variance.hip
+++ b/robustmvd_amd/csrc/warp_variance.hip
@@ -459,8 +459,9 @@
 }
 
 static int launch_k3(const WarpParams& p0, int C, bool warp_only, bool f16, hipStream_t st, float* absmax = nullptr,
-                     bool* absmax_done = nullptr) {
+                     bool* absmax_done = nullptr, const float* split_absmax = nullptr) {
     WarpParams p = p0;
+    if (split_absmax) return launch_warp_tile(p, st, 8, 104, 8, 1, false, p.exact_grid != 0, split_absmax);
 #ifdef MVD_EXPERIMENTS
     if (const char* e = exp_env("MVD_K3_CFG")) {
 #define MVD_G(R, DPB, MW) {R, DPB, MW, warp_only ? warp_variance_kernel<8, true, DPB, MW, R> : warp_variance_kernel<8, false, DPB, MW, R>}
@@ -487,7 +488,7 @@
 static int run_warp(const float* key_feat, const float* const* src_feat, const float* const* src_proj,
                     const float* key_proj_inv, const float* depth_values, int B, int C, int D, int h, int w, int V,
                     float* out, int layout, void* workspace, size_t workspace_bytes, hipStream_t st, bool warp_only,
-                    float* absmax = nullptr, bool* absmax_done = nullptr) {
+                    float* absmax = nullptr, bool* absmax_done = nullptr, const float* split_absmax = nullptr) {
     const char* who = warp_only ? "homo_warp" : "warp_variance";
     MVD_REQUIRE(B > 0 && D > 0 && h > 1 && w > 1, "%s: non-positive dimension (h, w must be >= 2)", who);
     MVD_REQUIRE(V >= 1 && V <= MVD_MAX_VIEWS, "%s: V=%d outside 1..%d", who, V, MVD_MAX_VIEWS);
@@ -538,7 +539,14 @@
     p.B = B; p.D = D; p.h = h; p.w = w; p.V = V;
     p.layout = layout & 0xff;
     p.exact_grid = (layout & MVD_GRID_EXACT) ? 1 : 0;
-    return launch_k3(p, C, warp_only, false, st, absmax, absmax_done);
+    return launch_k3(p, C, warp_only, false, st, absmax, absmax_done, split_absmax);
+}
+
+static bool split_volume_supported(int C, int h, int w, int V, int layout) {
+    WarpParams p{};
+    p.h = h; p.w = w; p.V = V;
+    return C == 32 && (layout & 0xff) == MVD_LAYOUT_NDHWC && (layout & MVD_FEAT_NHWC_BORDER) != 0 && h > 1 && w > 1 && V >= 1 &&
+           warp_tile_supported(p, false);
 }
 
 static int run_warp_f16(const void* key_feat, const void* const* src_feat, const float* const* src_proj,
@@ -653,6 +661,23 @@
     return rc;
 }
 
+int mvd_warp_variance_split_supported(int C, int h, int w, int V, int out_layout) {
+    return mvd::split_volume_supported(C, h, w, V, out_layout) ? 1 : 0;
+}
+
+int mvd_warp_variance_split_f32(const float* key_feat, const float* const* src_feat, const float* const* src_proj,
+                                const float* key_proj_inv, const float* depth_values, int B, int C, int D, int h, int w, int V,
+                                const float* split_absmax, void* split_out, int out_layout, void* workspace, size_t workspace_bytes,
+                                mvd_stream_t stream) {
+    MVD_REQUIRE(key_feat && src_feat && src_proj && key_proj_inv && depth_values && split_absmax && split_out,
+                "warp_variance_split: NULL argument");
+    MVD_REQUIRE(mvd::split_volume_supported(C, h, w, V, out_layout),
+                "warp_variance_split: needs C = 32, MVD_LAYOUT_NDHWC | MVD_FEAT_NHWC_BORDER and maps the tile kernel covers (h, w <= 65532, "
+                "h*w*128 < 2^31, V <= 32); got C=%d h=%d w=%d V=%d layout=0x%x", C, h, w, V, out_layout);
+    return mvd::run_warp(key_feat, src_feat, src_proj, key_proj_inv, depth_values, B, C, D, h, w, V, static_cast<float*>(split_out),
+                         out_layout, workspace, workspace_bytes, (hipStream_t)stream, false, nullptr, nullptr, split_absmax);
+}
+
 int mvd_absmax_f32(const float* x, long long n, float* absmax, mvd_stream_t stream) {
     MVD_REQUIRE(x && absmax && n >= 0, "absmax: NULL argument or negative count");
     return mvd::absmax_launch(x, n, absmax, (hipStream_t)stream);
diff --git a/robustmvd_amd/csrc/warp_variance_common.h b/robustmvd_amd/csrc/warp_variance_common.h
--- a/robustmvd_amd/csrc/warp_variance_common.h
+++ b/robustmvd_amd/csrc/warp_variance_common.h
@@ -65,7 +65,8 @@
 }
 
 bool warp_tile_supported(const WarpParams& p, bool f16);
-int launch_warp_tile(const WarpParams& p0, hipStream_t st, int tw, int win, int nch, int sets, bool f16, bool exact);
+int launch_warp_tile(const WarpParams& p0, hipStream_t st, int tw, int win, int nch, int sets, bool f16, bool exact,
+                     const float* split_absmax = nullptr);
 
 typedef void (*WarpKernel)(WarpParams);
 int launch_gather(const WarpParams& p0, int lpp, int dpb, WarpKernel kernel, hipStream_t st);
diff --git a/robustmvd_amd/csrc/warp_variance_tile.hip b/robustmvd_amd/csrc/warp_variance_tile.hip
--- a/robustmvd_amd/csrc/warp_variance_tile.hip
+++ b/robustmvd_amd/csrc/warp_variance_tile.hip
@@ -1,6 +1,7 @@
 #include "mvd_common.h"
 #include <type_traits>
 #include "warp_variance_common.h"
+#include "split_operand.h"
 
 namespace mvd {
 
@@ -69,8 +70,9 @@
     unsigned pad[2];
 };
 
-template <int TW, int WINPIX, bool F16, bool EXACT, int MINW, int SETS>
-__global__ void __launch_bounds__(256, MINW) warp_variance_tile_kernel(WarpParams p, int nch) {
+template <int TW, int WINPIX, bool F16, bool EXACT, int MINW, int SETS, bool SPLIT = false>
+__global__ void __launch_bounds__(256, MINW) warp_variance_tile_kernel(WarpParams p, int nch, const float* split_absmax) {
+    static_assert(!(SPLIT && F16), "the split volume is written from fp32 maps");
     constexpr int P = 8, NPX = 32;
     constexpr unsigned PIXB = F16 ? 64 : 128;
     constexpr unsigned QB = F16 ? 8 : 16;
@@ -371,6 +373,11 @@
 
     float amax = 0.f;
     const bool want_absmax = p.absmax != nullptr;
+    [[maybe_unused]] float xs = 0.f;
+    if constexpr (SPLIT) {
+        float xs_inv;
+        split_xscale(split_absmax, xs, xs_inv);
+    }
     auto store_chunk = [&](const Sums (&sm)[P], int c, bool drop) {
         int bx, by;
         const int t = opaque_tid();
@@ -394,6 +401,11 @@
             if constexpr (F16) {
                 const f16x2 lo = {(_Float16)r.x, (_Float16)r.y}, hi = {(_Float16)r.z, (_Float16)r.w};
                 store_b64(u32x2{as_u32(lo), as_u32(hi)}, orsrc, out_off);
+            } else if constexpr (SPLIT) {
+                unsigned h0, l0, h1, l1;
+                split2(xs, r.x, r.y, h0, l0, CONV0_LO_FACTOR);
+                split2(xs, r.z, r.w, h1, l1, CONV0_LO_FACTOR);
+                __builtin_amdgcn_raw_buffer_store_b128(u32x4{h0, h1, l0, l1}, orsrc, out_off, 0, 0);
             } else {
                 __builtin_amdgcn_raw_buffer_store_b128(u32x4{__float_as_uint(r.x), __float_as_uint(r.y), __float_as_uint(r.z), __float_as_uint(r.w)},
                                                        orsrc, out_off, 0, 0);
@@ -487,15 +499,15 @@
            (size_t)nch * V * sizeof(UnitRec);
 }
 
-template <int TW, int WINPIX, bool F16, bool EXACT, int MINW, int SETS>
-static int launch_tile_variant(const WarpParams& p, const dim3& grid, hipStream_t st, int nch) {
+template <int TW, int WINPIX, bool F16, bool EXACT, int MINW, int SETS, bool SPLIT = false>
+static int launch_tile_variant(const WarpParams& p, const dim3& grid, hipStream_t st, int nch, const float* split_absmax = nullptr) {
     const size_t lds = tile_lds_bytes(WINPIX, F16, p.V, nch);
-    auto* fn = warp_variance_tile_kernel<TW, WINPIX, F16, EXACT, MINW, SETS>;
+    auto* fn = warp_variance_tile_kernel<TW, WINPIX, F16, EXACT, MINW, SETS, SPLIT>;
     if (lds > 48 * 1024) {
         if (hipFuncSetAttribute(reinterpret_cast<const void*>(fn), hipFuncAttributeMaxDynamicSharedMemorySize, (int)lds) != hipSuccess)
             return launch_status("warp_variance_tile: hipFuncSetAttribute");
     }
-    hipLaunchKernelGGL(fn, grid, dim3(256), lds, st, p, nch);
+    hipLaunchKernelGGL(fn, grid, dim3(256), lds, st, p, nch, split_absmax);
     return MVD_OK;
 }
 
@@ -503,7 +515,7 @@
     return p.h + 3 < 65536 && p.w + 3 < 65536 && (long long)p.h * p.w * (f16 ? 64 : 128) < 0x7fffffffLL && p.V <= 32;
 }
 
-int launch_warp_tile(const WarpParams& p0, hipStream_t st, int tw, int win, int nch, int sets, bool f16, bool exact) {
+int launch_warp_tile(const WarpParams& p0, hipStream_t st, int tw, int win, int nch, int sets, bool f16, bool exact, const float* split_absmax) {
     WarpParams p = p0;
     const int th = 32 / tw;
     p.tiles_x = (p.w + tw - 1) / tw;
@@ -530,14 +542,20 @@
                  : (exact ? launch_tile_variant<TW_, WIN_, false, true, MW_, SETS_>(p, grid, st, nch)                 \
                           : launch_tile_variant<TW_, WIN_, false, false, MW_, SETS_>(p, grid, st, nch));              \
     }
+    if (split_absmax) {
+        if (tw == 8 && win == 104 && sets == 1 && !f16)
+            rc = exact ? launch_tile_variant<8, 104, false, true, 4, 1, true>(p, grid, st, nch, split_absmax)
+                       : launch_tile_variant<8, 104, false, false, 4, 1, true>(p, grid, st, nch, split_absmax);
+    } else {
     MVD_T(8, 104, 4, 1) MVD_T(8, 128, 4, 1)
 #ifdef MVD_EXPERIMENTS
     MVD_T(8, 128, 3, 2) MVD_T(8, 96, 4, 1) MVD_T(16, 128, 3, 2) MVD_T(16, 104, 4, 1) MVD_T(16, 96, 4, 1) MVD_T(32, 128, 3, 2) MVD_T(32, 104, 4, 1)
 #endif
+    }
 #undef MVD_T
     timing_end(st);
     if (rc == MVD_ERR_INVALID_ARG) {
-        set_error("warp_variance: tile variant tw=%d win=%d sets=%d is not compiled", tw, win, sets);
+        set_error("warp_variance: tile variant tw=%d win=%d sets=%d%s is not compiled", tw, win, sets, split_absmax ? " with the split store" : "");
         return rc;
     }
     if (rc) return rc;
diff --git a/robustmvd_amd/models.py b/robustmvd_amd/models.py
--- a/robustmvd_amd/models.py
+++ b/robustmvd_amd/models.py
@@ -156,7 +156,7 @@
 
 class MVSNet(nn.Module):
     def __init__(self, sample_in_inv_depth_space=False, num_sampling_steps=192, half_features=False, conv0_split=True,
-                 exact_grid=False, train_regulariser="vendor", sweep_backward="atomic"):
+                 exact_grid=False, train_regulariser="vendor", sweep_backward="atomic", presplit_handoff=True):
         super().__init__()
         if train_regulariser not in ("vendor", "engine"):
             raise ValueError(f"train_regulariser must be 'vendor' or 'engine', got {train_regulariser!r}")
@@ -167,6 +167,7 @@
         if sweep_backward == "gather":
             self.register_buffer("sweep_backward_fallbacks", torch.zeros(1, dtype=torch.int32), persistent=False)
         self.half_features = bool(half_features)
+        self.presplit_handoff = bool(presplit_handoff)
         if sample_in_inv_depth_space:
             raise NotImplementedError("sample_in_inv_depth_space=True is a dead branch in the reference "
                                       "(tensor[::-1] raises, mvsnet.py:50,56-63)")
@@ -241,10 +242,14 @@
         if self.half_features:
             var = ops.warp_variance_f16(feats[0], feats[1:], projs[1:], projs[0], depth_samples)
         else:
-            var = ops.warp_variance(feats[0], feats[1:], projs[1:], projs[0], depth_samples, channels_last=True, staged=True,
-                                    exact_grid=self.exact_grid)
+            handoff = None
             if split:
                 amax = a_feat * a_feat
+                _, hp, wp, C = feats[0].shape
+                if self.presplit_handoff and ops.warp_variance_split_supported(C, hp - 3, wp - 3, len(feats) - 1):
+                    handoff = amax
+            var = ops.warp_variance(feats[0], feats[1:], projs[1:], projs[0], depth_samples, channels_last=True, staged=True,
+                                    exact_grid=self.exact_grid, split_absmax=handoff)
         cost = self.cost_regularization.forward_channels_last(var, x_absmax=amax)
         del var
         depth, conf = ops.softmax_regress(cost, depth_samples)
diff --git a/robustmvd_amd/ops.py b/robustmvd_amd/ops.py
--- a/robustmvd_amd/ops.py
+++ b/robustmvd_amd/ops.py
@@ -157,9 +157,28 @@
     return fused, fmask
 
 
+class SplitVolume:
+    __slots__ = ("words", "absmax")
+
+    def __init__(self, words, absmax):
+        self.words, self.absmax = words, absmax
+
+    @property
+    def shape(self):
+        return self.words.shape
+
+    @property
+    def device(self):
+        return self.words.device
+
+
+def warp_variance_split_supported(C, h, w, V):
+    return bool(L.load().mvd_warp_variance_split_supported(C, h, w, V, L.LAYOUT_NDHWC | L.FEAT_NHWC_BORDER))
+
+
 @inference_only
 def warp_variance(key_feat, src_feats, src_projs, key_proj_inv, depth_values, channels_last=False, exact_grid=False,
-                  staged=False, return_absmax=False):
+                  staged=False, return_absmax=False, split_absmax=None):
     kf = L.as_f32(key_feat, "key_feat")
     if kf.dim() != 4:
         raise ValueError("key_feat must be (B,C,h,w)" + (" / (B,h+3,w+3,C) when staged" if staged else ""))
@@ -172,10 +191,17 @@
     V = len(srcs)
     projs, kpi, dv = _k3_calibration(src_projs, key_proj_inv, depth_values, V, B, C, dev)
     D = dv.shape[1]
-    out = torch.empty((B, D, h, w, C) if channels_last else (B, C, D, h, w), dtype=torch.float32, device=dev)
     wsb = L.load().mvd_warp_variance_workspace_bytes(B, C, h, w, 0 if staged else V)
     flags = (L.LAYOUT_NDHWC if channels_last else L.LAYOUT_NCDHW) | (L.GRID_EXACT if exact_grid else 0) | \
         (L.FEAT_NHWC_BORDER if staged else 0)
+    if split_absmax is not None:
+        if return_absmax or not (channels_last and staged):
+            raise ValueError("split_absmax: the split volume is written channels_last from staged maps, without return_absmax")
+        xam = L.as_f32(split_absmax, "split_absmax", (1,), dev)
+        words = torch.empty((B, D, h, w, C), dtype=torch.int32, device=dev)
+        call("mvd_warp_variance_split_f32", dev, kf, srcs, projs, kpi, dv, B, C, D, h, w, V, xam, words, flags, workspace(wsb, dev), wsb)
+        return SplitVolume(words, xam)
+    out = torch.empty((B, D, h, w, C) if channels_last else (B, C, D, h, w), dtype=torch.float32, device=dev)
     name, amax = "mvd_warp_variance_f32", []
     if return_absmax:
         name, amax = "mvd_warp_variance_absmax_f32", [torch.empty(1, dtype=torch.float32, device=dev)]
@@ -359,6 +385,25 @@
     if return_absmax:
         name, yam = "mvd_conv3d_bn_relu_absmax_f32_split", [torch.empty(1, dtype=torch.float32, device=dev)]
     call(name, dev, x, x_absmax, packed, scale, shift, y, *yam, B, D, h, w, cin, cout, int(bool(relu)))
+    return (y, yam[0]) if return_absmax else y
+
+
+@inference_only
+def conv3d_bn_relu_presplit(x, packed, scale, shift, relu=True, return_absmax=False):
+    if not isinstance(x, SplitVolume):
+        raise ValueError(f"x must be an ops.SplitVolume, got {type(x).__name__}")
+    B, D, h, w, cin = x.shape
+    dev = x.device
+    scale = L.as_f32(scale, "scale", device=dev)
+    cout = scale.numel()
+    if packed.numel() != L.load().mvd_conv3d_split_packed_weight_bytes(cin, cout):
+        raise ValueError(f"packed weights of {packed.numel()} bytes do not belong to a {cin} -> {cout} layer")
+    shift = L.as_f32(shift, "shift", (cout,), dev)
+    y = torch.empty((B, D, h, w, cout), dtype=torch.float32, device=dev)
+    name, yam = "mvd_conv3d_bn_relu_presplit", []
+    if return_absmax:
+        name, yam = "mvd_conv3d_bn_relu_absmax_presplit", [torch.empty(1, dtype=torch.float32, device=dev)]
+    call(name, dev, x.words, x.absmax, packed, scale, shift, y, *yam, B, D, h, w, cin, cout, int(bool(relu)))
     return (y, yam[0]) if return_absmax else y
 
 
```

Result: no change. 349.4 depth-maps/sec (median of 4 runs) (+0.8%).
